# hammershock/SFM-Python

Hardware: AMD Instinct MI355X
Metric: BA iterations/sec (higher is better)
Workload: dtype f64

## Files before the change

sfm-python_amd/csrc/ba_kernels.hpp:

```cpp
#pragma once

#include <hip/hip_runtime.h>
#include <stdint.h>

#include "tr2d.hpp"

namespace sfmba {

constexpr int kCamTab = 17;
constexpr int kCamRow = 18;
#ifndef SFMBA_REC_LAYOUT
#define SFMBA_REC_LAYOUT 0
#endif
constexpr int kRecLayout = SFMBA_REC_LAYOUT;
constexpr int kRec = kRecLayout == 0 ? 6 : (kRecLayout == 1 ? 8 : 16);
constexpr int kVinvRow = kRecLayout == 0 ? 6 : (kRecLayout == 1 ? 8 : 16);
constexpr int kVinvInRec = kRecLayout == 2 ? 8 : -1;
constexpr int kRhsRec = 16;
constexpr int kSweepThreads = 1024;
constexpr int kWavesPerSweepBlock = kSweepThreads / 64;

struct KMat { double k[9]; };

constexpr int kJPlanes = 6;
// ... 68 lines not shown
        for (int q = 0; q < NQ; ++q) {
            double s = 0.0;
            for (int k = 0; k < nw; ++k) s += red[k * NQ + q];
            v[q] = s;
        }
    }
}

__device__ __forceinline__ double block_sum_all(double v, double* slots) {
    const int nw = (blockDim.x + 63) >> 6;
    v = wave_sum(v);
    if ((threadIdx.x & 63) == 0) slots[threadIdx.x >> 6] = v;
    __syncthreads();
    double s = 0.0;
    for (int k = 0; k < nw; ++k) s += slots[k];
    return s;
}

constexpr int kNQ = 9;

constexpr int kFinishCols = 10;
struct FinishJob { int row0[2], nrows[2], slot[2][kFinishCols]; };

__device__ __forceinline__ void finish_task(const double* __restrict__ part, const FinishJob& job, int y, int k,
                                            int nq, int first_sum, double* __restrict__ out) {
    const int lane = threadIdx.x & 63;
    const double* __restrict__ rows = part + (size_t)job.row0[y] * nq;
    const int nparts = job.nrows[y];
    double s = 0.0;
    if (k < first_sum) {
        for (int b = lane; b < nparts; b += 64) s = fmax(s, rows[(size_t)b * nq + k]);
        s = wave_max(s);
    } else {
        for (int b = lane; b < nparts; b += 64) s += rows[(size_t)b * nq + k];
        s = wave_sum(s);
    }
    const int dst = job.slot[y][k];
    if (lane == 0 && dst >= 0) out[dst] = s;
}

struct Piggyback {
    const double* __restrict__ part;
    double* __restrict__ out;
    FinishJob job;
    int ny, nq, first_sum;
};
__device__ __forceinline__ void finish_in_block(const Piggyback& pb) {
    const int w = threadIdx.x >> 6, nw = blockDim.x >> 6;
    for (int t = w; t < pb.ny * pb.nq; t += nw)
        finish_task(pb.part, pb.job, t / pb.nq, t % pb.nq, pb.nq, pb.first_sum, pb.out);
}

template <int NV>
__device__ __forceinline__ void seg_reduce_serial(double (&v)[NV], int key, int lane) {
    constexpr int kRowShl = 0x100;
    const int col = lane & 15, row = lane >> 4;
    const int n1 = dpp_int<kRowShl + 1>(key), n2 = dpp_int<kRowShl + 2>(key);
    const int n4 = dpp_int<kRowShl + 4>(key), n8 = dpp_int<kRowShl + 8>(key);
    const int f48 = __builtin_amdgcn_readlane(key, 48), f32 = __builtin_amdgcn_readlane(key, 32);
    const int f16 = __builtin_amdgcn_readlane(key, 16);
    const double m1 = ((col + 1 < 16) & (n1 == key)) ? 1.0 : 0.0, m2 = ((col + 2 < 16) & (n2 == key)) ? 1.0 : 0.0;
    const double m4 = ((col + 4 < 16) & (n4 == key)) ? 1.0 : 0.0, m8 = ((col + 8 < 16) & (n8 == key)) ? 1.0 : 0.0;
    const double r2 = ((row == 2) & (key == f48)) ? 1.0 : 0.0, r1 = ((row == 1) & (key == f32)) ? 1.0 : 0.0;
    const double r0 = ((row == 0) & (key == f16)) ? 1.0 : 0.0;
#pragma unroll
    for (int n = 0; n < NV; ++n) {
        double x = v[n];
        x = fma(dpp_double<kRowShl + 1>(x), m1, x);
        x = fma(dpp_double<kRowShl + 2>(x), m2, x);
        x = fma(dpp_double<kRowShl + 4>(x), m4, x);
        x = fma(dpp_double<kRowShl + 8>(x), m8, x);
        x = fma(readlane_double(x, 48), r2, x);
        x = fma(readlane_double(x, 32), r1, x);
        x = fma(readlane_double(x, 16), r0, x);
        v[n] = x;
        __builtin_amdgcn_sched_barrier(0);
    }
}

__device__ __forceinline__ int lane_below(int key, int lane) {
    int prev = dpp_int<0x111>(key);
    const int k15 = __builtin_amdgcn_readlane(key, 15), k31 = __builtin_amdgcn_readlane(key, 31);
    const int k47 = __builtin_amdgcn_readlane(key, 47);
    return lane == 16 ? k15 : (lane == 32 ? k31 : (lane == 48 ? k47 : prev));
}

__device__ __forceinline__ size_t jaddr_f32(int i, int m) {
    return ((size_t)(i >> 6) * 3 + m) * 64 + (i & 63);
}
__device__ __forceinline__ double2 load_pair(const double* __restrict__ base, int f32, int i) {
    if (f32) {
        const float2 v = reinterpret_cast<const float2*>(base)[i];
        return make_double2((double)v.x, (double)v.y);
    }
    return reinterpret_cast<const double2*>(base)[i];
}
__device__ __forceinline__ void store_pair(double* __restrict__ base, int f32, int i, double a, double b) {
    if (f32) reinterpret_cast<float2*>(base)[i] = make_float2((float)a, (float)b);
    else reinterpret_cast<double2*>(base)[i] = make_double2(a, b);
}

constexpr int kCamRT = 12, kCamWbc = 5;
__host__ __device__ constexpr size_t cam_rt_offset(int C) { return (size_t)C * kCamRow; }
__host__ __device__ constexpr size_t cam_wbc_offset(int C) { return cam_rt_offset(C) + (size_t)C * kCamRT; }
__host__ __device__ constexpr size_t cam_table_doubles(int C) { return cam_wbc_offset(C) + (size_t)C * kCamWbc; }
__device__ __forceinline__ void cam_row_values(const double* __restrict__ prm, double* __restrict__ t) {
    const double wx = prm[0], wy = prm[1], wz = prm[2];
    const double th2 = wx * wx + wy * wy + wz * wz;
    const double th = sqrt(th2);
    double a, b, cc;
    if (th < 1e-4) {
        a = 1.0 - th2 / 6.0 + th2 * th2 / 120.0;
        b = 0.5 - th2 / 24.0 + th2 * th2 / 720.0;
    } else {
        a = sin(th) / th;
        const double h = 0.5 * th;
        const double s = sin(h) / h;
        b = 0.5 * s * s;
    }
    if (th < 0.3) {
        cc = 1.0 / 6.0 - th2 / 120.0 + th2 * th2 / 5040.0 - th2 * th2 * th2 / 362880.0 +
             th2 * th2 * th2 * th2 / 39916800.0 - th2 * th2 * th2 * th2 * th2 / 6227020800.0;
    } else {
        cc = (th - sin(th)) / (th2 * th);
    }
    t[0] = 1.0 + b * (wx * wx - th2); t[1] = -a * wz + b * wx * wy;     t[2] = a * wy + b * wx * wz;
    t[3] = a * wz + b * wx * wy;      t[4] = 1.0 + b * (wy * wy - th2); t[5] = -a * wx + b * wy * wz;
    t[6] = -a * wy + b * wx * wz;     t[7] = a * wx + b * wy * wz;      t[8] = 1.0 + b * (wz * wz - th2);
    t[9] = prm[3]; t[10] = prm[4]; t[11] = prm[5];
    t[12] = wx; t[13] = wy; t[14] = wz;
    t[15] = b; t[16] = cc;
}
__device__ __forceinline__ void cam_table_row(const double* __restrict__ prm, double* __restrict__ tab, int C, int c) {
    double* __restrict__ t = tab + (size_t)c * kCamRow;
    t[kCamTab] = 0.0;
    cam_row_values(prm, t);
    double* __restrict__ rt = tab + cam_rt_offset(C) + (size_t)c * kCamRT;
#pragma unroll
    for (int k = 0; k < kCamRT; ++k) rt[k] = t[k];
    double* __restrict__ wbc = tab + cam_wbc_offset(C);
#pragma unroll
    for (int k = 0; k < kCamWbc; ++k) wbc[(size_t)k * C + c] = t[12 + k];
}

__global__ void k_cam_table(const double* __restrict__ xc, int C, double* __restrict__ tab) {
    const int c = blockIdx.x * blockDim.x + threadIdx.x;
    if (c >= C) return;
    double prm[6];
#pragma unroll
    for (int k = 0; k < 6; ++k) prm[k] = xc[6 * (size_t)c + k];
    cam_table_row(prm, tab, C, c);
}

__global__ void k_tr_step(double* __restrict__ sc, double Delta, const PcgCtrl* __restrict__ ctrl,
                          Piggyback pb) {
    if (pb.part != nullptr) {
        finish_in_block(pb);
        __syncthreads();
    }
    if (threadIdx.x != 0 || blockIdx.x != 0) return;
    if (ctrl != nullptr && ctrl->done == 0) { sc[30] = 1.0; return; }
    auto q = [&](int point_slot, int k) { return sc[point_slot] + sc[16 + k]; };
    const TrModel m = tr_build_model(sc[1], sc[2], sc[3], q(8, 1), q(4, 5), q(5, 6), q(11, 4), q(6, 7), q(7, 8));
    const TrStep st = tr_solve_step(m, Delta);
    sc[25] = st.c1; sc[26] = st.c2; sc[27] = st.predicted; sc[28] = st.step_h_norm; sc[29] = st.step_norm;
    sc[30] = 0.0; sc[31] = Delta;
}

__global__ __launch_bounds__(256) void k_step_table(const double* __restrict__ x,
                                                    const double* __restrict__ sg,
                                                    const double* __restrict__ p, double c1, double c2,
                                                    const double* __restrict__ coef,
                                                    int C, int64_t n, int bc, double* __restrict__ x_new,
                                                    double* __restrict__ tab, double* __restrict__ rec_new,
                                                    const double* __restrict__ skip) {
    if (skip != nullptr && *skip != 0.0) return;
    if (coef != nullptr) { c1 = coef[0]; c2 = coef[1]; }
    if ((int)blockIdx.x < bc) {
        const int c = blockIdx.x * blockDim.x + threadIdx.x;
        if (c >= C) return;
        double prm[6];
#pragma unroll
        for (int k = 0; k < 6; ++k) {
            const size_t e = 6 * (size_t)c + k;
            prm[k] = x[e] + c1 * sg[e] + c2 * p[e];
            x_new[e] = prm[k];
        }
        cam_table_row(prm, tab, C, c);
        return;
    }
    const int64_t n6 = 6 * (int64_t)C;
    const int nb = gridDim.x - bc;
    for (int64_t e = n6 + (blockIdx.x - bc) * (int64_t)blockDim.x + threadIdx.x; e < n; e += (int64_t)nb * blockDim.x) {
        const double v = x[e] + c1 * sg[e] + c2 * p[e];
        x_new[e] = v;
        const int q = (int)(e - n6), pt = q / 3;
        rec_new[(size_t)kRec * pt + (q - 3 * pt)] = v;
    }
}

__global__ void k_fill_rec(const double* __restrict__ pts, int P, double* __restrict__ rec) {
    const int q = blockIdx.x * blockDim.x + threadIdx.x;
    if (q >= 3 * P) return;
    const int p = q / 3;
    rec[(size_t)kRec * p + (q - 3 * p)] = pts[q];
}

template <bool JAC>
__device__ __forceinline__ void observe(const double* __restrict__ t, double X, double Y, double Z,
                                        double u, double v, const KMat& K, double& rx, double& ry,
                                        double* __restrict__ jc, double* __restrict__ jp) {
    const double vx = X - t[9], vy = Y - t[10], vz = Z - t[11];
    const double qx = t[0] * vx + t[1] * vy + t[2] * vz;
    const double qy = t[3] * vx + t[4] * vy + t[5] * vz;
    const double qz = t[6] * vx + t[7] * vy + t[8] * vz;
    const double px = K.k[0] * qx + K.k[1] * qy + K.k[2] * qz;
    const double py = K.k[3] * qx + K.k[4] * qy + K.k[5] * qz;
    const double pz = K.k[6] * qx + K.k[7] * qy + K.k[8] * qz;
    const double iz = 1.0 / pz;
    const double u0 = px * iz, u1 = py * iz;
    rx = u0 - u;
    ry = u1 - v;
    if (JAC) {
        const double wx = t[12], wy = t[13], wz = t[14], b = t[15], c = t[16];
#pragma unroll
        for (int k = 0; k < 2; ++k) {
            const double pk = k == 0 ? u0 : u1;
            const double a0 = (K.k[3 * k + 0] - pk * K.k[6]) * iz;
            const double a1 = (K.k[3 * k + 1] - pk * K.k[7]) * iz;
            const double a2 = (K.k[3 * k + 2] - pk * K.k[8]) * iz;
            const double j0 = a0 * t[0] + a1 * t[3] + a2 * t[6];
            const double j1 = a0 * t[1] + a1 * t[4] + a2 * t[7];
            const double j2 = a0 * t[2] + a1 * t[5] + a2 * t[8];
            jp[3 * k + 0] = j0; jp[3 * k + 1] = j1; jp[3 * k + 2] = j2;
            const double m0 = j1 * vz - j2 * vy, m1 = j2 * vx - j0 * vz, m2 = j0 * vy - j1 * vx;
            const double s0 = m1 * wz - m2 * wy, s1 = m2 * wx - m0 * wz, s2 = m0 * wy - m1 * wx;
            const double t0 = s1 * wz - s2 * wy, t1 = s2 * wx - s0 * wz, t2 = s0 * wy - s1 * wx;
            jc[6 * k + 0] = -(m0 - b * s0 + c * t0);
            jc[6 * k + 1] = -(m1 - b * s1 + c * t1);
            jc[6 * k + 2] = -(m2 - b * s2 + c * t2);
            jc[6 * k + 3] = -j0; jc[6 * k + 4] = -j1; jc[6 * k + 5] = -j2;
        }
    }
}

__device__ __forceinline__ void st16(double* __restrict__ p, double a, double b) {
    *reinterpret_cast<double2*>(p) = make_double2(a, b);
}

constexpr int kRowPieces = kCamRow / 2;
constexpr size_t kRowSlabDoubles = 64 * (size_t)kCamRow;
__device__ __forceinline__ void rows_request(const double* __restrict__ table, int cam, int lane, double* slab) {
#pragma unroll
    for (int k = 0; k < kRowPieces; ++k) {
        const int q = k * 64 + lane;
        const int row = q / kRowPieces, piece = q - kRowPieces * row;
        const int cr = __shfl(cam, row);
        __builtin_amdgcn_global_load_lds(table + (size_t)cr * kCamRow + 2 * piece,
                                         (__attribute__((address_space(3))) void*)(slab + 2 * 64 * k), 16, 0, 0);
        __builtin_amdgcn_sched_barrier(0);
    }
}
__device__ __forceinline__ void rows_wait() { asm volatile("s_waitcnt vmcnt(0)" ::: "memory"); }
__device__ __forceinline__ void rows_read_done() { asm volatile("s_waitcnt lgkmcnt(0)" ::: "memory"); }

constexpr int kEdgeRow = 10;
struct PointBlocksOut {
    double* __restrict__ V;
    double* __restrict__ gp;
    double* __restrict__ edge;
};

template <bool LDS_TAB, bool JAC, bool STORE_R, bool F32, bool BLOCKS = false, bool STORE_J = true>
__global__ __launch_bounds__(kSweepThreads) void k_resjac(
    const double* __restrict__ camtab, const double* __restrict__ pts, const int* __restrict__ cam_idx,
    const int* __restrict__ pt_idx, const double* __restrict__ uv, double* __restrict__ r,
    double* __restrict__ J, int N, int64_t ld, int C, KMat K,
    double* __restrict__ cost_part, const double* __restrict__ skip, PointBlocksOut pb) {
    extern __shared__ __align__(16) double smem[];
    __shared__ double red[kWavesPerSweepBlock];
    if (skip != nullptr && *skip != 0.0) return;
    const int stride = gridDim.x * blockDim.x;
    const int lane = threadIdx.x & 63;
    static_assert(JAC || !BLOCKS, "the point blocks are sums of Jacobian entries");
    constexpr bool blocks = BLOCKS;
    int i = blockIdx.x * blockDim.x + threadIdx.x;
    int c0 = 0, p0 = 0, c1 = 0, p1 = 0;
    double2 uv0 = make_double2(0.0, 0.0);
    double X0 = 0.0, Y0 = 0.0, Z0 = 0.0;
    if (i < N) { c0 = cam_idx[i]; p0 = pt_idx[i]; uv0 = load_pair(uv, F32, i); }
    if (i + stride < N) { c1 = cam_idx[i + stride]; p1 = pt_idx[i + stride]; }
    if (i < N) { const double* __restrict__ Xp = pts + 3 * (size_t)p0; X0 = Xp[0]; Y0 = Xp[1]; Z0 = Xp[2]; }
    if (LDS_TAB) {
        const int n2 = (C * kCamRow) >> 1;
        const double2* __restrict__ src = reinterpret_cast<const double2*>(camtab);
        double2* __restrict__ dst = reinterpret_cast<double2*>(smem);
        for (int k = threadIdx.x; k < n2; k += blockDim.x) dst[k] = src[k];
        __syncthreads();
    }
    double* const slab = smem + (size_t)(threadIdx.x >> 6) * kRowSlabDoubles;
    if (!LDS_TAB && i - lane < N) rows_request(camtab, c0, lane, slab);
    double acc = 0.0;
    while (i - lane < N) {
        const bool on = i < N;
        const int in = i + stride, in2 = in + stride;
        double tl[kCamRow];
        if (!LDS_TAB) rows_wait();
        {
            const double2* __restrict__ trow = reinterpret_cast<const double2*>(LDS_TAB ? smem + (size_t)c0 * kCamRow
                                                                                         : slab + (size_t)lane * kCamRow);
#pragma unroll
            for (int k = 0; k < kCamRow / 2; ++k) { const double2 q = trow[k]; tl[2 * k] = q.x; tl[2 * k + 1] = q.y; }
        }
        if (!LDS_TAB) {
            rows_read_done();
            if (in - lane < N) rows_request(camtab, c1, lane, slab);
        }
        int c2 = 0, p2 = 0;
        double2 uv1 = make_double2(0.0, 0.0);
        double X1 = 0.0, Y1 = 0.0, Z1 = 0.0;
        if (in2 < N) { c2 = cam_idx[in2]; p2 = pt_idx[in2]; }
        if (in < N) {
            uv1 = load_pair(uv, F32, in);
            const double* __restrict__ Xp = pts + 3 * (size_t)p1;
            X1 = Xp[0]; Y1 = Xp[1]; Z1 = Xp[2];
        }
        const int ib = i - lane;
        int pprev = -1, pnext = -2;
        if (blocks) {
            if (ib > 0) pprev = pt_idx[ib - 1];
            if (ib + 64 < N) pnext = pt_idx[ib + 64];
        }
        double jc[12], jp[6], rx, ry;
        observe<JAC>(tl, X0, Y0, Z0, uv0.x, uv0.y, K, rx, ry, jc, jp);
        if (on) {
            acc += rx * rx + ry * ry;
            if (STORE_R) {
                if (F32) store_pair(r, 1, i, rx, ry); else st16(r + 2 * (size_t)i, rx, ry);
            }
            if (JAC && STORE_J) {
                if (F32) {
                    float4* __restrict__ Jf = reinterpret_cast<float4*>(J);
                    Jf[jaddr_f32(i, 0)] = make_float4((float)jc[0], (float)jc[1], (float)jc[2], (float)jc[6]);
                    Jf[jaddr_f32(i, 1)] = make_float4((float)jc[7], (float)jc[8], (float)jp[0], (float)jp[1]);
                    Jf[jaddr_f32(i, 2)] = make_float4((float)jp[2], (float)jp[3], (float)jp[4], (float)jp[5]);
                } else {
                    st16(J + jaddr(ld, i, 0), jc[0], jc[1]);
                    st16(J + jaddr(ld, i, 1), jc[2], jc[6]);
                    st16(J + jaddr(ld, i, 2), jc[7], jc[8]);
#pragma unroll
                    for (int m = 0; m < 3; ++m) st16(J + jaddr(ld, i, 3 + m), jp[2 * m], jp[2 * m + 1]);
                }
            }
        }
        if (blocks) {
            double v[9];
            v[0] = jp[0] * jp[0] + jp[3] * jp[3]; v[1] = jp[0] * jp[1] + jp[3] * jp[4];
            v[2] = jp[0] * jp[2] + jp[3] * jp[5]; v[3] = jp[1] * jp[1] + jp[4] * jp[4];
// ... 377 lines not shown
                                  const double* __restrict__ uv, int f32, int N, int* __restrict__ cm_pt,
                                  double* __restrict__ cm_uv) {
    const int k = blockIdx.x * blockDim.x + threadIdx.x;
    if (k >= N) return;
    const int i = perm[k];
    cm_pt[k] = pt_idx[i];
    if (f32) reinterpret_cast<float2*>(cm_uv)[k] = reinterpret_cast<const float2*>(uv)[i];
    else reinterpret_cast<double2*>(cm_uv)[k] = reinterpret_cast<const double2*>(uv)[i];
}

__global__ __launch_bounds__(256) void k_unpack_obs(const unsigned short* __restrict__ ci16, const short2* __restrict__ uv16,
                                                    int from, int to, int f32, int* __restrict__ cam_idx, double* __restrict__ uv) {
    const int k = from + blockIdx.x * blockDim.x + threadIdx.x;
    if (k >= to) return;
    cam_idx[k] = (int)ci16[k];
    const short2 q = uv16[k];
    if (f32) reinterpret_cast<float2*>(uv)[k] = make_float2((float)q.x, (float)q.y);
    else reinterpret_cast<double2*>(uv)[k] = make_double2((double)q.x, (double)q.y);
}
__global__ __launch_bounds__(256) void k_expand_pt_idx(const int* __restrict__ pt_ptr, int P, int N, int ld, int* __restrict__ pt_idx) {
    const int p = blockIdx.x * blockDim.x + threadIdx.x;
    if (p < P) {
        const int b = pt_ptr[p], e = pt_ptr[p + 1];
        for (int k = b; k < e; ++k) pt_idx[k] = p;
    } else if (p == P) {
        for (int k = N; k < ld; ++k) pt_idx[k] = 0;
    }
}

constexpr int kSortSlices = 512;
__global__ __launch_bounds__(64) void k_cam_hist(const int* __restrict__ cam_idx, const unsigned char* __restrict__ fixed,
                                                 int N, int C, int per, int* __restrict__ hist) {
    extern __shared__ int cnt[];
    for (int c = threadIdx.x; c < C; c += 64) cnt[c] = 0;
    __syncthreads();
    const int b0 = blockIdx.x * per, b1 = min(N, b0 + per);
    for (int k0 = b0 + (int)threadIdx.x; k0 < b1; k0 += 64 * 8) {
        int c[8];
#pragma unroll
        for (int u = 0; u < 8; ++u) { const int k = k0 + 64 * u; c[u] = k < b1 ? cam_idx[k] : -1; }
#pragma unroll
        for (int u = 0; u < 8; ++u)
            if (c[u] >= 0 && (fixed == nullptr || fixed[c[u]] == 0)) atomicAdd(&cnt[c[u]], 1);
    }
    __syncthreads();
    for (int c = threadIdx.x; c < C; c += 64) hist[(size_t)blockIdx.x * C + c] = cnt[c];
}
__global__ __launch_bounds__(256) void k_cam_offsets(const int* __restrict__ hist, const int* __restrict__ cam_ptr, int B, int C,
                                                     int* __restrict__ off) {
    const int c = blockIdx.x * blockDim.x + threadIdx.x;
    if (c >= C) return;
    int run = cam_ptr[c];
    for (int b0 = 0; b0 < B; b0 += 16) {
        int n[16];
#pragma unroll
        for (int u = 0; u < 16; ++u) n[u] = b0 + u < B ? hist[(size_t)(b0 + u) * C + c] : 0;
#pragma unroll
        for (int u = 0; u < 16; ++u) {
            if (b0 + u < B) off[(size_t)(b0 + u) * C + c] = run;
            run += n[u];
        }
    }
}
__global__ __launch_bounds__(64) void k_cam_scatter(const int* __restrict__ cam_idx, const unsigned char* __restrict__ fixed,
                                                    const int* __restrict__ pt_idx, const double* __restrict__ uv, int f32,
                                                    int N, int C, int per, int key_bits, const int* __restrict__ off,
                                                    int* __restrict__ cm_pt, double* __restrict__ cm_uv) {
    extern __shared__ int cur[];
    for (int c = threadIdx.x; c < C; c += 64) cur[c] = off[(size_t)blockIdx.x * C + c];
    __syncthreads();
    const int lane = threadIdx.x;
    const unsigned long long lt = lane == 0 ? 0ull : (~0ull >> (64 - lane));
    const int b0 = blockIdx.x * per, b1 = min(N, b0 + per);
    auto fetch = [&](int k, int& c, int& p, double2& q) {
        c = -1; p = 0; q = make_double2(0.0, 0.0);
        if (k < b1) {
            c = cam_idx[k];
            p = pt_idx[k];
            if (f32) { const float2 t = reinterpret_cast<const float2*>(uv)[k]; q = make_double2((double)t.x, (double)t.y); }
            else q = reinterpret_cast<const double2*>(uv)[k];
        }
    };
    int cn, pn;
    double2 qn;
    fetch(b0 + lane, cn, pn, qn);
    for (int k0 = b0; k0 < b1; k0 += 64) {
        int c = cn;
        const int p = pn;
        const double2 q = qn;
        fetch(k0 + 64 + lane, cn, pn, qn);
        if (c >= 0 && fixed != nullptr && fixed[c] != 0) c = -1;
        const bool act = c >= 0;
        unsigned long long eq = __ballot(act);
        for (int bit = 0; bit < key_bits; ++bit) {
            const unsigned long long m = __ballot(act && ((c >> bit) & 1));
            eq &= ((c >> bit) & 1) ? m : ~m;
        }
        if (act) {
            const int dst = cur[c] + __popcll(eq & lt);
            cm_pt[dst] = p;
            if (f32) reinterpret_cast<float2*>(cm_uv)[dst] = make_float2((float)q.x, (float)q.y);
            else reinterpret_cast<double2*>(cm_uv)[dst] = q;
            if ((eq >> lane) == 1ull) cur[c] += __popcll(eq);
        }
        __builtin_amdgcn_wave_barrier();
    }
}
__global__ __launch_bounds__(256) void k_xcd_chunks(const int* __restrict__ cam_ptr, const int* __restrict__ cm_pt, int C, int P,
                                                    int4* __restrict__ chunks) {
    const int e = blockIdx.x * blockDim.x + threadIdx.x;
    const int groups = (C + 3) / 4;
    if (e >= groups * 32) return;
    const int j = e & 3, k = (e >> 2) & 7, g = e >> 5;
    const int c = 4 * g + j;
    if (c >= C) { chunks[e] = make_int4(-1, 0, 0, 8); return; }
    const int b = cam_ptr[c], en = cam_ptr[c + 1];
    auto bound = [&](int kk) {
        if (kk <= 0) return b;
        if (kk >= 8) return en;
        const int p_hi = (int)(((long long)P * kk) / 8);
        int lo = b, hi = en;
        while (lo < hi) { const int mid = (lo + hi) >> 1; if (cm_pt[mid] < p_hi) lo = mid + 1; else hi = mid; }
        return lo;
    };
    chunks[e] = make_int4(c, bound(k), bound(k + 1), 8);
}

struct StepTable {
    const int2* __restrict__ wsteps;
    const int2* __restrict__ steps;
    int n_waves;
};

__device__ __forceinline__ void write_partials(double (&q)[kNQ], double* __restrict__ part) {
    __shared__ double red[4 * kNQ];
    __shared__ double mred[4];
    const double m = wave_max(q[0]);
    q[0] = 0.0;
    if ((threadIdx.x & 63) == 0) mred[threadIdx.x >> 6] = m;
    block_sum<kNQ>(q, red);
    if (threadIdx.x == 0) {
        double mm = 0.0;
        for (int k = 0; k < (int)(blockDim.x >> 6); ++k) mm = fmax(mm, mred[k]);
        part[(size_t)blockIdx.x * kNQ + 0] = mm;
        for (int k = 1; k < kNQ; ++k) part[(size_t)blockIdx.x * kNQ + k] = q[k];
    }
}

template <int kScalePts>
__global__ __launch_bounds__(256) void k_update_scale(const double* __restrict__ Ugc,
                                                      const double* __restrict__ V,
                                                      const double* __restrict__ gp,
                                                      const double* __restrict__ x, int C, int P,
                                                      int first, int bc, double* __restrict__ si,
                                                      double* __restrict__ g, double* __restrict__ sg,
                                                      double* __restrict__ part) {
    const int n6 = 6 * C;
    double q[kNQ];
#pragma unroll
    for (int k = 0; k < kNQ; ++k) q[k] = 0.0;
    auto element = [&](double d, double ge, double s_old, double xe, double& s, double& sge) {
        s = sqrt(d);
        if (first) { if (s == 0.0) s = 1.0; } else { s = fmax(s, s_old); }
        sge = ge / (s * s);
        q[0] = fmax(q[0], fabs(ge));
        q[1] += (ge / s) * (ge / s);
        q[2] += (xe * s) * (xe * s);
        q[3] += xe * xe;
        q[4] += sge * sge;
    };
    if ((int)blockIdx.x < bc) {
        const int diagU[6] = {0, 6, 11, 15, 18, 20};
        for (int e = blockIdx.x * blockDim.x + threadIdx.x; e < n6; e += bc * blockDim.x) {
            const int c = e / 6, k = e - 6 * c;
            const double d = Ugc[(size_t)c * 27 + diagU[k]], ge = Ugc[(size_t)c * 27 + 21 + k];
            double s, sge;
            element(d, ge, first ? 0.0 : si[e], x[e], s, sge);
            si[e] = s; g[e] = ge; sg[e] = sge;
        }
    } else {
        const int nb = (int)gridDim.x - bc, b = (int)blockIdx.x - bc;
        const double* __restrict__ xp = x + n6;
        double* __restrict__ sip = si + n6;
        double* __restrict__ gpo = g + n6;
        double* __restrict__ sgp = sg + n6;
        for (int p0 = (b * kScalePts) * (int)blockDim.x + (int)threadIdx.x; p0 < P; p0 += nb * kScalePts * (int)blockDim.x) {
            double d[kScalePts][3], ge[kScalePts][3], so[kScalePts][3], xe[kScalePts][3];
#pragma unroll
            for (int u = 0; u < kScalePts; ++u) {
                const int p = p0 + u * (int)blockDim.x;
                const size_t pp = (size_t)(p < P ? p : 0);
                d[u][0] = V[pp * 6 + 0]; d[u][1] = V[pp * 6 + 3]; d[u][2] = V[pp * 6 + 5];
#pragma unroll
                for (int k = 0; k < 3; ++k) {
                    ge[u][k] = gp[pp * 3 + k];
                    xe[u][k] = xp[pp * 3 + k];
                    so[u][k] = first ? 0.0 : sip[pp * 3 + k];
                }
            }
#pragma unroll
            for (int u = 0; u < kScalePts; ++u) {
                const int p = p0 + u * (int)blockDim.x;
                if (p >= P) continue;
#pragma unroll
                for (int k = 0; k < 3; ++k) {
                    double s, sge;
                    element(d[u][k], ge[u][k], so[u][k], xe[u][k], s, sge);
                    sip[(size_t)p * 3 + k] = s; gpo[(size_t)p * 3 + k] = ge[u][k]; sgp[(size_t)p * 3 + k] = sge;
                }
            }
        }
    }
    write_partials(q, part);
}


__global__ void k_post(Mailbox mb) { post_mailbox(mb); }

__global__ void k_finish(const double* __restrict__ part, FinishJob job, int nq, int first_sum,
                         double* __restrict__ out, const double* __restrict__ skip, Mailbox mb) {
    if (skip != nullptr && *skip != 0.0) {
        if (mb.host != nullptr && blockIdx.x == 0 && threadIdx.x < 64) post_mailbox(mb);
        return;
    }
    const int k = threadIdx.x >> 6;
    if (k < nq) finish_task(part, job, (int)blockIdx.x, k, nq, first_sum, out);
    if (mb.host != nullptr) {
        __syncthreads();
        if (threadIdx.x < 64) post_mailbox(mb);
    }
}

struct Recompute {
    const double* __restrict__ camtab;
    const double* __restrict__ pts;
    KMat K;
};
__device__ __forceinline__ void stage_cam_table(const double* __restrict__ camtab, int C, double* __restrict__ smem) {
    const int n2 = (C * kCamRow) >> 1;
    const double2* __restrict__ src = reinterpret_cast<const double2*>(camtab);
    double2* __restrict__ dst = reinterpret_cast<double2*>(smem);
    for (int k = threadIdx.x; k < n2; k += blockDim.x) dst[k] = src[k];
    __syncthreads();
}
__device__ __forceinline__ void recompute_blocks(const Recompute& rc, const double* __restrict__ tab_lds, int c, int p,
                                                 double* jc, double* jp) {
    double tl[kCamRow];
    const double2* __restrict__ trow = reinterpret_cast<const double2*>(tab_lds + (size_t)c * kCamRow);
#pragma unroll
    for (int k = 0; k < kCamRow / 2; ++k) { const double2 q = trow[k]; tl[2 * k] = q.x; tl[2 * k + 1] = q.y; }
    const double* __restrict__ Xp = rc.pts + 3 * (size_t)p;
    double rx, ry;
    observe<true>(tl, Xp[0], Xp[1], Xp[2], 0.0, 0.0, rc.K, rx, ry, jc, jp);
}

template <bool LDS_VEC, bool JFREE = false>
__global__ __launch_bounds__(kSweepThreads) void k_jdot(ObsArrays o, const double* __restrict__ sgc,
                                                        const double* __restrict__ sgp, int N, int C,
                                                        double* __restrict__ t1,
                                                        double* __restrict__ part, Piggyback pb, Recompute rc) {
    static_assert(!(LDS_VEC && JFREE), "J-free: the LDS holds the camera table, the vector comes from L2");
    extern __shared__ __align__(16) double smem[];
    __shared__ double red[kWavesPerSweepBlock];
    const int nwork = pb.part != nullptr ? (int)gridDim.x - 1 : (int)gridDim.x;
    if ((int)blockIdx.x == nwork) { finish_in_block(pb); return; }
    if (LDS_VEC) {
        for (int i = threadIdx.x; i < 6 * C; i += blockDim.x) smem[i] = sgc[i];
        __syncthreads();
    }
    if (JFREE) stage_cam_table(rc.camtab, C, smem);
    const double* __restrict__ vc = LDS_VEC ? smem : sgc;
    double acc = 0.0;
    for (int i = blockIdx.x * blockDim.x + threadIdx.x; i < N; i += nwork * blockDim.x) {
        double jc[12], jp[6];
        if (JFREE) recompute_blocks(rc, smem, o.cam_idx[i], o.pt_idx[i], jc, jp);
        else load_blocks(o, i, jc, jp);
        const double2* a2 = reinterpret_cast<const double2*>(vc + 6 * o.cam_idx[i]);
        const double2 a01 = a2[0], a23 = a2[1], a45 = a2[2];
        const double a[6] = {a01.x, a01.y, a23.x, a23.y, a45.x, a45.y};
        const double* b = sgp + 3 * (size_t)o.pt_idx[i];
        double t0 = 0.0, t1v = 0.0;
#pragma unroll
        for (int k = 0; k < 6; ++k) { t0 += jc[k] * a[k]; t1v += jc[6 + k] * a[k]; }
#pragma unroll
        for (int k = 0; k < 3; ++k) { t0 += jp[k] * b[k]; t1v += jp[3 + k] * b[k]; }
        store_pair(t1, o.f32, i, t0, t1v);
        acc += t0 * t0 + t1v * t1v;
    }
    acc = wave_sum(acc);
    if ((threadIdx.x & 63) == 0) red[threadIdx.x >> 6] = acc;
    __syncthreads();
    if (threadIdx.x == 0) {
        double s = 0.0;
        for (int k = 0; k < (int)(blockDim.x >> 6); ++k) s += red[k];
        part[blockIdx.x] = s;
    }
}

__device__ __forceinline__ void chol3_inverse(const double* a , double* inv ) {
    const double l00 = sqrt(a[0]);
    const double l10 = a[1] / l00, l20 = a[2] / l00;
    const double l11 = sqrt(a[3] - l10 * l10);
    const double l21 = (a[4] - l20 * l10) / l11;
    const double l22 = sqrt(a[5] - l20 * l20 - l21 * l21);
    const double m00 = 1.0 / l00, m11 = 1.0 / l11, m22 = 1.0 / l22;
    const double m10 = -l10 * m00 * m11;
    const double m21 = -l21 * m11 * m22;
    const double m20 = -(l20 * m00 + l21 * m10) * m22;
    inv[0] = m00 * m00 + m10 * m10 + m20 * m20;
    inv[1] = m10 * m11 + m20 * m21;
    inv[2] = m20 * m22;
    inv[3] = m11 * m11 + m21 * m21;
    inv[4] = m21 * m22;
    inv[5] = m22 * m22;
}

__device__ __forceinline__ double reg_from_a11(double a11, double G11, double Delta, double reg_min) {
    const double a = 0.5 * G11, b = -a11;
    double reg = reg_min;
    if (a11 > 0.0) {
        const double to_tr = Delta / sqrt(a11);
        double best = 0.0;
        const double y_ub = to_tr * (a * to_tr + b);
        if (y_ub < best) best = y_ub;
        if (a != 0.0) {
            const double ext = -0.5 * b / a;
            if (ext > 0.0 && ext < to_tr) { const double y = ext * (a * ext + b); if (y < best) best = y; }
        }
        reg = fmax(-best / (Delta * Delta), reg_min);
    }
    return reg;
}
__device__ __forceinline__ double reg_from_scalars(const double* __restrict__ sc, double G11, double Delta,
                                                   double reg_min) {
    return reg_from_a11(sc[8] + sc[16 + 1], G11, Delta, reg_min);
}

__device__ __forceinline__ void point_prep_one(const double* __restrict__ V, const double* __restrict__ gp,
                                               const double* __restrict__ sip, const double* __restrict__ dp_extra,
                                               int p, double reg, double* __restrict__ Vinv,
                                               double* __restrict__ e, const double* __restrict__ pts = nullptr,
                                               double* __restrict__ rhsrec = nullptr) {
    double a[6], inv[6];
#pragma unroll
    for (int k = 0; k < 6; ++k) a[k] = V[(size_t)p * 6 + k];
    if (dp_extra) {
        a[0] += dp_extra[3 * (size_t)p]; a[3] += dp_extra[3 * (size_t)p + 1]; a[5] += dp_extra[3 * (size_t)p + 2];
    } else {
        const double s0 = sip[3 * (size_t)p], s1 = sip[3 * (size_t)p + 1], s2 = sip[3 * (size_t)p + 2];
        a[0] += reg * s0 * s0; a[3] += reg * s1 * s1; a[5] += reg * s2 * s2;
// ... 24 lines not shown
    float* __restrict__ rt32;
    float* __restrict__ rec32;
    double* __restrict__ rtd;
    Origin o;
};
__device__ __forceinline__ void mixed_prep_camera(const MixedPrep& mx, int C, int c) {
    const double* __restrict__ rt = mx.camtab + cam_rt_offset(C) + (size_t)kCamRT * c;
    float4* __restrict__ out = reinterpret_cast<float4*>(mx.rt32 + (size_t)kRt32 * c);
    out[0] = make_float4((float)rt[0], (float)rt[1], (float)rt[2], (float)rt[3]);
    out[1] = make_float4((float)rt[4], (float)rt[5], (float)rt[6], (float)rt[7]);
    out[2] = make_float4((float)rt[8], (float)(rt[9] - mx.o.x), (float)(rt[10] - mx.o.y), (float)(rt[11] - mx.o.z));
    double* __restrict__ d = mx.rtd + (size_t)kRt32 * c;
    const float4 a = out[0], b = out[1], e = out[2];
    d[0] = a.x; d[1] = a.y; d[2] = a.z; d[3] = a.w; d[4] = b.x; d[5] = b.y; d[6] = b.z; d[7] = b.w;
    d[8] = e.x; d[9] = e.y; d[10] = e.z; d[11] = e.w;
}
__device__ __forceinline__ void mixed_prep_point(const MixedPrep& mx, const double* __restrict__ pts, int p) {
    float4* __restrict__ out = reinterpret_cast<float4*>(mx.rec32 + (size_t)kRec32 * p);
    out[0] = make_float4((float)(pts[3 * (size_t)p] - mx.o.x), (float)(pts[3 * (size_t)p + 1] - mx.o.y),
                         (float)(pts[3 * (size_t)p + 2] - mx.o.z), 0.f);
}
__global__ void k_mixed_prep(MixedPrep mx, const double* __restrict__ pts, int C, int P, int bc) {
    if ((int)blockIdx.x < bc) {
        const int c = blockIdx.x * blockDim.x + threadIdx.x;
        if (c < C) mixed_prep_camera(mx, C, c);
        return;
    }
    const int p = (blockIdx.x - bc) * blockDim.x + threadIdx.x;
    if (p < P) mixed_prep_point(mx, pts, p);
}

__global__ void k_point_prep(const double* __restrict__ V, const double* __restrict__ gp,
                             const double* __restrict__ sip, const double* __restrict__ dp_extra,
                             int P, double reg, double* __restrict__ Vinv, double* __restrict__ e,
                             const double* __restrict__ pts, double* __restrict__ rhsrec) {
    const int p = blockIdx.x * blockDim.x + threadIdx.x;
    if (p >= P) return;
    point_prep_one(V, gp, sip, dp_extra, p, reg, Vinv, e, pts, rhsrec);
}

__device__ __forceinline__ void spd6_inverse(const double (&A)[6][6], double (&out)[21]) {
    double Lm[6][6];
#pragma unroll
    for (int j = 0; j < 6; ++j) {
        double sj = A[j][j];
#pragma unroll
        for (int k = 0; k < j; ++k) sj -= Lm[j][k] * Lm[j][k];
        const double ljj = sqrt(sj);
        Lm[j][j] = ljj;
        const double inv = 1.0 / ljj;
#pragma unroll
        for (int i = j + 1; i < 6; ++i) {
            double t = A[i][j];
#pragma unroll
            for (int k = 0; k < j; ++k) t -= Lm[i][k] * Lm[j][k];
            Lm[i][j] = t * inv;
        }
    }
    double M[6][6];
#pragma unroll
    for (int j = 0; j < 6; ++j) {
        M[j][j] = 1.0 / Lm[j][j];
#pragma unroll
        for (int i = j + 1; i < 6; ++i) {
            double t = 0.0;
#pragma unroll
            for (int k = j; k < i; ++k) t -= Lm[i][k] * M[k][j];
            M[i][j] = t / Lm[i][i];
        }
    }
    int n = 0;
#pragma unroll
    for (int a = 0; a < 6; ++a)
#pragma unroll
        for (int b = a; b < 6; ++b) {
            double t = 0.0;
#pragma unroll
            for (int k = b; k < 6; ++k) t += M[k][a] * M[k][b];
            out[n++] = t;
        }
}

__device__ __forceinline__ void cam_prep_regs(const double* __restrict__ Ugc, const double* __restrict__ sic,
                                              const double* __restrict__ dc_extra, int C, int c, double reg,
                                              double* __restrict__ Dc, double* __restrict__ Minv,
                                              const double* __restrict__ sd, double (&out)[21]) {
    double A[6][6];
    {
        int n = 0;
#pragma unroll
        for (int a = 0; a < 6; ++a)
#pragma unroll
            for (int b = a; b < 6; ++b) {
                A[a][b] = Ugc[(size_t)c * 27 + n] - (sd ? sd[(size_t)n * C + c] : 0.0);
                A[b][a] = A[a][b];
                ++n;
            }
    }
#pragma unroll
    for (int a = 0; a < 6; ++a) {
        double d;
        if (sd) d = Dc[(size_t)a * C + c];
        else {
            d = dc_extra ? dc_extra[6 * (size_t)c + a] : reg * sic[6 * (size_t)c + a] * sic[6 * (size_t)c + a];
            Dc[(size_t)a * C + c] = d;
        }
        A[a][a] += d;
    }
    spd6_inverse(A, out);
#pragma unroll
    for (int n = 0; n < 21; ++n) Minv[(size_t)n * C + c] = out[n];
}
__device__ __forceinline__ void cam_prep_one(const double* __restrict__ Ugc, const double* __restrict__ sic,
                                             const double* __restrict__ dc_extra, int C, int c, double reg,
                                             double* __restrict__ Dc, double* __restrict__ Minv,
                                             const double* __restrict__ sd = nullptr) {
    double out[21];
    cam_prep_regs(Ugc, sic, dc_extra, C, c, reg, Dc, Minv, sd, out);
}

__global__ void k_cam_prep(const double* __restrict__ Ugc, const double* __restrict__ sic,
                           const double* __restrict__ dc_extra, int C, double reg,
                           double* __restrict__ Dc, double* __restrict__ Minv) {
    const int c = blockIdx.x * blockDim.x + threadIdx.x;
    if (c >= C) return;
    cam_prep_one(Ugc, sic, dc_extra, C, c, reg, Dc, Minv);
}

__global__ __launch_bounds__(64) void k_cam_prep_schur(const double* __restrict__ Ugc, const double* __restrict__ sd, int C,
                                                       double* __restrict__ Dc, double* __restrict__ Minv) {
    const int c = blockIdx.x * blockDim.x + threadIdx.x;
    if (c >= C) return;
    cam_prep_one(Ugc, nullptr, nullptr, C, c, 0.0, Dc, Minv, sd);
}

__global__ __launch_bounds__(64) void k_prep(double* __restrict__ sc, double Delta, double reg_min,
                                             const double* __restrict__ Ugc, const double* __restrict__ V,
                                             const double* __restrict__ gp, const double* __restrict__ si,
                                             int C, int P, int bc, double* __restrict__ Dc,
                                             double* __restrict__ Minv,
                                             double* __restrict__ Vinv, double* __restrict__ e,
                                             const double* __restrict__ jd_part, int jd_n, double eta_min, double eta_max,
                                             const double* __restrict__ pts, double* __restrict__ rhsrec, MixedPrep mx) {
    double G11;
    if (jd_part != nullptr) {
        double s = 0.0;
        for (int b = threadIdx.x; b < jd_n; b += 64) s += jd_part[b];
        G11 = wave_sum(s);
        G11 = __shfl(G11, 0);
        if (blockIdx.x == 0 && threadIdx.x == 0) sc[1] = G11;
    } else {
        G11 = sc[1];
    }
    const double reg = reg_from_scalars(sc, G11, Delta, reg_min);
    if (blockIdx.x == 0 && threadIdx.x == 0) {
        sc[13] = reg;
        const double a11 = sc[8] + sc[16 + 1], prev = sc[14];
        double eta = eta_max;
        if (prev > 0.0 && a11 >= 0.0) eta = fmin(eta_max, fmax(eta_min, sqrt(a11 / prev)));
        sc[15] = eta;
        sc[14] = a11;
    }
    if ((int)blockIdx.x < bc) {
        const int c = blockIdx.x * blockDim.x + threadIdx.x;
        if (c >= C) return;
        if (mx.rt32 != nullptr) mixed_prep_camera(mx, C, c);
        if (Minv != nullptr) { cam_prep_one(Ugc, si, nullptr, C, c, reg, Dc, Minv); return; }
#pragma unroll
        for (int a = 0; a < 6; ++a) Dc[(size_t)a * C + c] = reg * si[6 * (size_t)c + a] * si[6 * (size_t)c + a];
        return;
    }
    const int p = (blockIdx.x - bc) * blockDim.x + threadIdx.x;
    if (p >= P) return;
    if (mx.rt32 != nullptr) mixed_prep_point(mx, pts, p);
    point_prep_one(V, gp, si + 6 * (size_t)C, nullptr, p, reg, Vinv, e, pts, rhsrec);
}

__device__ __forceinline__ double minv_row(const double* m, const double* r, int k) {
    double z = 0.0;
#pragma unroll
    for (int j = 0; j < 6; ++j) {
        const int a = k < j ? k : j, b = k < j ? j : k;
        z += m[a * 6 - a * (a - 1) / 2 + (b - a)] * r[j];
    }
    return z;
}

struct PcgFused {
    const double* __restrict__ Dc;
    const double* __restrict__ Minv;
    const double* __restrict__ Ugc;
    double* __restrict__ vecs;
    PcgCtrl* __restrict__ ctrl2;
    double tol;
    int max_iters;
    const double* __restrict__ tol_dev;
    double* __restrict__ part;
};
constexpr int kPcgM = kPcgUcm;

__device__ __forceinline__ double pcg_local_step(const double* __restrict__ part, int C, const PcgCtrl& ci, PcgCtrl& co) {
    __shared__ double red4[16][4];
    const int cam = threadIdx.x;
    double q4[4] = {0.0, 0.0, 0.0, 0.0};
    if (cam < C) {
#pragma unroll
        for (int k = 0; k < 4; ++k) q4[k] = part[(size_t)k * C + cam];
    }
#pragma unroll
    for (int k = 0; k < 4; ++k) q4[k] = wave_sum(q4[k]);
    if ((threadIdx.x & 63) == 0) {
#pragma unroll
        for (int k = 0; k < 4; ++k) red4[threadIdx.x >> 6][k] = q4[k];
    }
    __syncthreads();
    double tot[4] = {0.0, 0.0, 0.0, 0.0};
    for (int w = 0; w < (int)(blockDim.x >> 6); ++w) {
#pragma unroll
        for (int k = 0; k < 4; ++k) tot[k] += red4[w][k];
    }
    const double delta = tot[0], su = tot[1], sm = tot[2], gamma = tot[3];
    const double beta = ci.iters == 0 ? 0.0 : ci.rz / ci.rz_prev;
    const double den = delta - (ci.iters == 0 ? 0.0 : beta * gamma / ci.alpha_prev);
    const double alpha = gamma / den;
    co = ci;
    if (!(den > 0.0) || !isfinite(alpha)) { co.done = 3; return 0.0; }
    const double rz = gamma - 2.0 * alpha * su + alpha * alpha * sm;
    int done = 0;
    if (!(rz > ci.tol2 * ci.rz0)) done = 1;
    else if (ci.iters + 1 >= ci.max_iters) done = 2;
    co.rz_prev = gamma; co.alpha_prev = alpha; co.rz = rz; co.iters = ci.iters + 1; co.done = done;
    return alpha;
}

__device__ __forceinline__ bool pcg_fused_update(const PcgFused& pf, const double* __restrict__ acc, int C, int L,
                                                 double (&uu)[6]) {
    __shared__ double red_a[16];
    __shared__ double red_b[16];
    const int n6 = 6 * C;
    PcgCtrl* __restrict__ cout = pf.ctrl2 + ((L + 1) & 1);
    const bool writer = blockIdx.x == 0 && threadIdx.x == 0;
    const int cam = threadIdx.x;
    const bool has = cam < C;
    const int slice = (C + (int)gridDim.x - 1) / (int)gridDim.x;
    const bool own = has && cam >= (int)blockIdx.x * slice && cam < ((int)blockIdx.x + 1) * slice;
    const int set = L == 0 ? 0 : (L - 1) & 1;
    const double* __restrict__ vold = pf.vecs + (size_t)set * kPcgVecs * n6;
    double* __restrict__ vnew = pf.vecs + (size_t)(L == 0 ? 0 : set ^ 1) * kPcgVecs * n6;
#pragma unroll
    for (int k = 0; k < 6; ++k) uu[k] = 0.0;
    double m[21];
    PcgCtrl ci;
    if (L != 0) {
        ci = pf.ctrl2[L & 1];
        if (ci.done != 0) {
            if (writer) *cout = ci;
            return false;
        }
    }
    if (pf.part != nullptr && L != 0) {
        double ue[6] = {0.0, 0.0, 0.0, 0.0, 0.0, 0.0}, me[6] = {0.0, 0.0, 0.0, 0.0, 0.0, 0.0};
        if (has) {
#pragma unroll
            for (int k = 0; k < 6; ++k) {
                const size_t e = (size_t)k * C + cam;
                ue[k] = vold[kPcgU * n6 + e];
                me[k] = pf.vecs[kPcgM * n6 + e];
            }
        }
        PcgCtrl co;
        const double alpha = pcg_local_step(pf.part, C, ci, co);
        if (writer) *cout = co;
        if (co.done == 3) return false;
        const int done = co.done;
        if (has) {
#pragma unroll
            for (int k = 0; k < 6; ++k) uu[k] = ue[k] - alpha * me[k];
            if (own) {
#pragma unroll
                for (int k = 0; k < 6; ++k) {
                    const size_t e = (size_t)k * C + cam;
                    vnew[kPcgU * n6 + e] = uu[k];
                    if (done != 0) {
                        const double xk = pf.vecs[kPcgX * n6 + e] + alpha * pf.vecs[kPcgP * n6 + e];
                        pf.vecs[kPcgX * n6 + e] = xk;
                        pf.vecs[(size_t)kPcgVecs * n6 + kPcgX * n6 + e] = xk;
                    }
                }
            }
        }
        return done == 0;
    }
    if (has) {
#pragma unroll
        for (int n = 0; n < 21; ++n) m[n] = pf.Minv[(size_t)n * C + cam];
    }
    if (L == 0) {
        double rr[6];
        double t = 0.0;
        if (has) {
#pragma unroll
            for (int k = 0; k < 6; ++k) rr[k] = -pf.Ugc[(size_t)cam * 27 + 21 + k] - acc[(size_t)k * C + cam];
#pragma unroll
            for (int k = 0; k < 6; ++k) {
                uu[k] = minv_row(m, rr, k);
                t += uu[k] * rr[k];
            }
// ... 1980 lines not shown
```

sfm-python_amd/csrc/sfmba.hip:

```cpp
#include "../../include/sfmba.h"

#include <hip/hip_runtime.h>
#include <hip/hip_ext.h>
#include <rccl/rccl.h>
#include <dlfcn.h>

#include <algorithm>
#include <atomic>
#include <chrono>
#include <cmath>
#include <cstdarg>
#include <cstdio>
#include <cstdlib>
#include <cstring>
#include <condition_variable>
#include <functional>
#include <mutex>
#include <numeric>
#include <string>
#include <thread>
#include <vector>

#include "ba_kernels.hpp"
#include "tr2d.hpp"
// ... 54 lines not shown
        if (p && keep) memcpy(q, p, std::min(keep, bytes));
        if (p) (void)hipHostFree(p);
        p = q; bytes = cap;
        return hipSuccess;
    }
    template <class T> T* as() const { return static_cast<T*>(p); }
};

class HostPool {
public:
    static constexpr int kMax = 16;
    ~HostPool() {
        { std::lock_guard<std::mutex> lk(m_); stop_ = true; ++gen_; }
        cv_.notify_all();
        for (auto& t : th_) t.join();
    }
    int parts_for(int64_t n) const {
        const int hw = (int)std::thread::hardware_concurrency();
        return (int)std::max<int64_t>(1, std::min<int64_t>(std::min(kMax, hw > 0 ? hw : 1), n / 65536));
    }
    template <class Fn>
    void run(int parts, Fn fn) {
        if (parts <= 1) { fn(0); return; }
        while ((int)th_.size() < parts - 1) {
            const int id = (int)th_.size() + 1;
            th_.emplace_back([this, id] { worker(id); });
        }
        std::function<void(int)> f = fn;
        {
            std::lock_guard<std::mutex> lk(m_);
            job_ = &f; job_parts_ = parts; pending_ = parts - 1; ++gen_;
        }
        cv_.notify_all();
        fn(0);
        std::unique_lock<std::mutex> lk(m_);
        done_.wait(lk, [this] { return pending_ == 0; });
        job_ = nullptr;
    }
private:
    void worker(int id) {
        unsigned long long seen = 0;
        for (;;) {
            std::function<void(int)>* f = nullptr;
            {
                std::unique_lock<std::mutex> lk(m_);
                cv_.wait(lk, [&] { return gen_ != seen; });
                seen = gen_;
                if (stop_) return;
                if (id >= job_parts_ || job_ == nullptr) continue;
                f = job_;
            }
            (*f)(id);
            {
                std::lock_guard<std::mutex> lk(m_);
                if (--pending_ == 0) done_.notify_one();
            }
        }
    }
    std::vector<std::thread> th_;
    std::mutex m_;
    std::condition_variable cv_, done_;
    std::function<void(int)>* job_ = nullptr;
    int job_parts_ = 0, pending_ = 0;
    unsigned long long gen_ = 0;
    bool stop_ = false;
};

struct RcclApi {
    void* lib = nullptr;
    ncclResult_t (*GetUniqueId)(ncclUniqueId*) = nullptr;
    ncclResult_t (*CommInitRank)(ncclComm_t*, int, ncclUniqueId, int) = nullptr;
    ncclResult_t (*AllReduce)(const void*, void*, size_t, ncclDataType_t, ncclRedOp_t, ncclComm_t, hipStream_t) = nullptr;
    ncclResult_t (*CommDestroy)(ncclComm_t) = nullptr;
    const char* (*GetErrorString)(ncclResult_t) = nullptr;
};
RcclApi* rccl_api() {
    static RcclApi api;
    static bool tried = false;
    if (!tried) {
        tried = true;
        void* lib = dlopen("librccl.so.1", RTLD_NOW | RTLD_GLOBAL);
        if (!lib) lib = dlopen("librccl.so", RTLD_NOW | RTLD_GLOBAL);
        if (!lib) lib = dlopen("/opt/rocm/lib/librccl.so.1", RTLD_NOW | RTLD_GLOBAL);
        if (lib) {
            api.GetUniqueId = (decltype(api.GetUniqueId))dlsym(lib, "ncclGetUniqueId");
            api.CommInitRank = (decltype(api.CommInitRank))dlsym(lib, "ncclCommInitRank");
            api.AllReduce = (decltype(api.AllReduce))dlsym(lib, "ncclAllReduce");
            api.CommDestroy = (decltype(api.CommDestroy))dlsym(lib, "ncclCommDestroy");
            api.GetErrorString = (decltype(api.GetErrorString))dlsym(lib, "ncclGetErrorString");
            if (api.GetUniqueId && api.CommInitRank && api.AllReduce && api.CommDestroy && api.GetErrorString)
                api.lib = lib;
        }
    }
    return api.lib ? &api : nullptr;
}

double now_s() {
    return std::chrono::duration<double>(std::chrono::steady_clock::now().time_since_epoch()).count();
}

}

struct sfmba_handle {
    int device = 0;
    hipStream_t stream = nullptr;
    bool own_stream = false;
    std::string err;
    int n_cu = 256;

    bool have_problem = false;
    int64_t C = 0, P = 0, N = 0, ld = 0, n = 0;
    int64_t N_total = 0;
    KMat K{};
    bool permuted = false;
    std::vector<int64_t> order;
    int n_ranges = 0;
    bool f32 = false;
    bool f32_next = false;
    std::vector<int64_t> fixed_next;
    int64_t n_fixed = 0;
    bool lds_tab = true, lds_vec = true;
    bool sweep_rc = false;
    bool sweep_rc_g = false;
    DevBuf rctab;
    bool jfree = false;
    bool mixed = false;
    bool mixed_b = false;
    DevBuf rt32, rec32, rctab32, rtd;
    Origin origin{0.0, 0.0, 0.0};
    bool dense = false;
    DevView cov_ptr, cov_pt, blk_ab;
    DevBuf Sblk;
    DevBuf tables;
    int n_blk = 0;
    struct Debug {
        int pcg_fused = -1;
        int tab_lds = -1, vec_lds = -1;
        int sweep_rc = -1;
        int dense = -1;
        int precond = -1;
        int pcg_local = -1;
        int xcd_chunks = -1;
        int rhsrec = -1;
        int cost_rider = -1;
        int packed_upload = -1;
        int jfree = -1;
        int cm_device = -1;
        int pcg_inline = -1;
        int xcd_cam = -1;
        int pcg_skip_last = -1;
        int pcg_mixed_b = -1;
        int pcg_mixed = -1;
        int pcg_split = -1;
        int cam_chunk = 0;
        int pcg_guess_bias = 0;
        int trace_pcg = 0, trace_stalls = 0, trace_timing = 0;
        int wait_deadline_s = 120;
        int p2p_delay_ms = 0;
        int p2p_timeout_ms = 0;
    } dbg;

    DevBuf cam_idx, pt_idx, pt_ptr, uv;
    DevView ranges, wsteps, steps;
    int n_steps = 0;
    DevBuf cm_perm, cm_pt, cm_uv, cam_partial;
    DevBuf sort_hist, fixed_dev;
    DevView cam_ptr_dev;
    DevView cam_chunks, cam_chunk_ptr;
    int n_chunks = 0;
    DevView cam_chunks_b, cam_chunk_ptr_b;
    int n_chunks_b = 0;
    bool xcd_b = false;
    std::vector<int4> host_chunks_b;
    std::vector<int> host_chunk_ptr_b;
    bool cam_multi = false;
    DevBuf xa, xb, tabA, tabB, r, J, t1;
    DevBuf rhsrec;
    DevBuf V, Vinv, gp, e, recA, recB;
    DevBuf edge;
    DevBuf g, si, sg, p;
    DevBuf Dc, Minv, vecs, vtmp, vcm;
    DevBuf part, ctrl;
    DevBuf arena_own;
    double* arena = nullptr;
    int64_t arena_doubles = 0;
    sfmba_allreduce_fn ar_fn = nullptr;
    void* ar_ctx = nullptr;
    sfmba_print_fn print_fn = nullptr;
    void* print_ctx = nullptr;
    ncclComm_t comm = nullptr;
    int64_t n_collectives = 0, n_launches = 0;
    struct P2p {
        bool ready = false;
        int rank = 0, world = 0;
        int64_t stride = 0;
        void* own = nullptr;
        void* opened[kP2pMaxRanks] = {};
        double* data[kP2pMaxRanks] = {};
        unsigned long long* flags[kP2pMaxRanks] = {};
        double* camdata[kP2pMaxRanks] = {};
        unsigned* words = nullptr;
        int64_t calls = 0;
        bool first_in_solve = true;
        int shared_device = 1;
        bool any_multi = false;
    } p2p;
    double* h_scal = nullptr;
    struct Stage { PinnedBuf uv, ci, pi, perm, ptr, uvf, tables, ci16, uv16; } stage;
    DevBuf ci16_dev, uv16_dev;
    struct Prev { bool valid = false; bool f32 = false; bool packed = false; int64_t N = 0, P = 0; } prev;
    std::vector<int2> host_ranges, host_wsteps, host_steps;
    std::vector<int4> host_chunks;
    std::vector<int> host_chunk_ptr;
    HostPool pool;
    int64_t obs_reused = 0, obs_uploaded = 0;
    double* mbox = nullptr;
    double* mbox_dev = nullptr;
    unsigned long long mbox_seq = 0;
    Mailbox post{};
    double* h_x = nullptr;
    size_t h_x_doubles = 0;
    hipStream_t copy_stream = nullptr;
    hipEvent_t ev_written = nullptr, ev_copied[2] = {nullptr, nullptr};
    PinnedBuf mirror[2];
    unsigned long long mirror_tag[2] = {0, 0}, copy_count = 0, x_tag = 0;
    bool mirror_on = false;
    const double* skip = nullptr;
    double pcg_tol = 0.0; int pcg_cap = 0;
    bool pcg_fused = false;
    bool pcg_local = false;
    bool pcg_local2 = false;
    bool pcg_b_owed = false;
    bool pcg_a_owed = false;
    bool pcg_inline = false;
    bool pcg_split = false;
    DevBuf pcg_part;
    int pcg_hint = 0;
    std::vector<int> pcg_hist;
    int64_t hist_C = 0, hist_P = 0, hist_N = 0;
    unsigned long long hist_sig = 0;
    unsigned long long problem_gen = 0;
    bool use_rhsrec = false;
    bool solved = false;
    bool transport_dropped = false;
    std::vector<const void*> lds_ready;
    int last_pcg_iters = 0;

    double* x = nullptr;
    double* x_new = nullptr;
    double* tab = nullptr;
    double* tab_new = nullptr;
    double* rec = nullptr;
    double* rec_new = nullptr;

    double* acc() const { return arena; }
    double* sd() const { return arena + 6 * C; }
    double* Ugc() const { return arena + 27 * C; }
    double* scal() const { return arena + 54 * C; }
    int pcg_L = 0;
    int red_bc = 1, red_grid = 2;
    int scale_pts = 1;
    double* partB() const { return part.as<double>() + (size_t)kPartRows * kNQ; }
    bool pending_scale_sums = false;
};

namespace {

int fail(sfmba_handle* h, int code, const char* fmt, ...) {
    char buf[512];
    va_list ap;
    va_start(ap, fmt);
    vsnprintf(buf, sizeof buf, fmt, ap);
    va_end(ap);
    if (h) h->err = buf;
    return code;
}

#define HIPCHK(h, call)                                                                         \
    do {                                                                                        \
        hipError_t e_ = (call);                                                                 \
        if (e_ != hipSuccess)                                                                   \
            return fail(h, e_ == hipErrorOutOfMemory ? -4 : -3, "%s failed: %s (%s:%d)", #call,  \
                        hipGetErrorString(e_), __FILE__, __LINE__);                             \
    } while (0)

#define LAUNCHED(h)                            \
    do {                                       \
        ++(h)->n_launches;                     \
        HIPCHK(h, hipGetLastError());          \
    } while (0)

#define CHK(expr)                  \
    do {                           \
        int rc_ = (expr);          \
        if (rc_ != 0) return rc_;  \
    } while (0)

int enter(sfmba_handle* h) {
    if (!h) return -1;
    h->err.clear();
    HIPCHK(h, hipSetDevice(h->device));
    return 0;
}

void p2p_release(sfmba_handle* h);
void p2p_close_peers(sfmba_handle* h);
bool multi_rank(const sfmba_handle* h) { return h->p2p.ready || h->comm != nullptr || h->ar_fn != nullptr; }
const unsigned* p2p_error_word(const sfmba_handle* h) { return h->p2p.ready ? h->p2p.words + 1 : nullptr; }

constexpr long long kP2pFirstTicks = 6000000000ll, kP2pSteadyTicks = 3000000000ll;
constexpr size_t kP2pFlagBytes = sizeof(unsigned long long) * 2 * kP2pMaxRanks * kP2pFlagStride;

void p2p_fill_args(sfmba_handle* h, P2pArgs& a) {
    auto& p = h->p2p;
    for (int q = 0; q < p.world; ++q) { a.data[q] = p.data[q]; a.flags[q] = p.flags[q]; }
    a.rank = p.rank; a.world = p.world; a.stride = p.stride;
    a.seq = reinterpret_cast<unsigned long long*>(p.words + 2);
    a.ticket = p.words; a.error = p.words + 1;
    a.timeout = p.first_in_solve ? kP2pFirstTicks : kP2pSteadyTicks;
    if (h->dbg.p2p_timeout_ms > 0) a.timeout = 100000ll * h->dbg.p2p_timeout_ms;
    p.first_in_solve = false;
}

constexpr int64_t kSharedDeviceCams = 128;
bool p2p_inline_ok(const sfmba_handle* h) {
    const auto& p = h->p2p;
    return p.ready && !p.any_multi && !(p.shared_device > 1 && h->C * (p.shared_device - 1) > kSharedDeviceCams);
}
bool xcd_cam(const sfmba_handle* h) { return h->xcd_b && h->dbg.xcd_cam != 0; }
bool cam_inline(const sfmba_handle* h) { return p2p_inline_ok(h) && !h->cam_multi && !xcd_cam(h) && h->dbg.pcg_inline != 0; }

CamExchange cam_exchange(sfmba_handle* h) {
    CamExchange cx{};
    auto& p = h->p2p;
    for (int q = 0; q < p.world; ++q) cx.data[q] = p.camdata[q];
    cx.rank = p.rank; cx.world = p.world; cx.C = (int)h->C; cx.error = p.words + 1;
    cx.timeout = p.first_in_solve ? kP2pFirstTicks : kP2pSteadyTicks;
    if (h->dbg.p2p_timeout_ms > 0) cx.timeout = 100000ll * h->dbg.p2p_timeout_ms;
    p.first_in_solve = false;
    return cx;
}

int p2p_allreduce(sfmba_handle* h, double* ptr, int64_t count, int op, const int* cancel,
                  unsigned long long max_mask = 0, const Piggyback* rider = nullptr, const Mailbox* post = nullptr,
                  const double* skip = nullptr) {
    auto& p = h->p2p;
    P2pArgs a{};
    p2p_fill_args(h, a);
    a.cancel = cancel;
    a.max_mask = max_mask;
    if (rider) a.rider = *rider;
    if (post) a.post = *post;
    a.skip = skip;
    if ((rider || post) && count > 512) return fail(h, -1, "rider / post need a single-workgroup collective");
    const int grid = (int)std::min<int64_t>(kP2pMaxBlocks, std::max<int64_t>(1, (count + 511) / 512));
    hipLaunchKernelGGL(k_p2p_allreduce, dim3(grid), dim3(256), 0, h->stream, ptr, (int)count, op, a);
    LAUNCHED(h);
    ++p.calls;
    return 0;
}

int exchange(sfmba_handle* h, double* ptr, int64_t count, int op, const int* cancel = nullptr) {
    if (h->p2p.ready && count <= h->p2p.stride) {
        CHK(p2p_allreduce(h, ptr, count, op, cancel));
        ++h->n_collectives;
        return 0;
    }
    if (h->comm) {
        RcclApi* api = rccl_api();
        const ncclResult_t rc = api->AllReduce(ptr, ptr, (size_t)count, ncclDouble, op == 0 ? ncclSum : ncclMax,
                                               h->comm, h->stream);
        if (rc != ncclSuccess) return fail(h, -5, "ncclAllReduce failed: %s", api->GetErrorString(rc));
        ++h->n_collectives;
        return 0;
    }
    if (!h->ar_fn) return 0;
    if (h->ar_fn(h->ar_ctx, ptr, count, op) != 0) return fail(h, -5, "all-reduce callback failed");
    ++h->n_collectives;
    return 0;
}

template <class Kern>
int set_lds(sfmba_handle* h, Kern k, size_t bytes) {
    if (bytes <= 64 * 1024) return 0;
    const void* fn = reinterpret_cast<const void*>(k);
    if (std::find(h->lds_ready.begin(), h->lds_ready.end(), fn) != h->lds_ready.end()) return 0;
    HIPCHK(h, hipFuncSetAttribute(fn, hipFuncAttributeMaxDynamicSharedMemorySize, (int)kLdsDynMax));
    h->lds_ready.push_back(fn);
    return 0;
}

double* vinv_ptr(const sfmba_handle* h) { return kVinvInRec < 0 ? h->Vinv.as<double>() : h->rec + kVinvInRec; }

MixedPrep mixed_prep(const sfmba_handle* h, const double* tab) {
    if (!h->mixed) return MixedPrep{nullptr, nullptr, nullptr, nullptr, Origin{0.0, 0.0, 0.0}};
    return MixedPrep{tab, h->rt32.as<float>(), h->rec32.as<float>(), h->rtd.as<double>(), h->origin};
}
int launch_mixed_prep(sfmba_handle* h, const double* x, const double* tab) {
    if (!h->mixed) return 0;
    const int bc = (int)((h->C + 255) / 256), bp = (int)((h->P + 255) / 256);
    hipLaunchKernelGGL(k_mixed_prep, dim3(bc + bp), dim3(256), 0, h->stream, mixed_prep(h, tab), x + 6 * h->C, (int)h->C, (int)h->P, bc);
    LAUNCHED(h);
    return 0;
}

ObsArrays obs_arrays(const sfmba_handle* h) {
    return ObsArrays{h->cam_idx.as<int>(), h->pt_idx.as<int>(), h->pt_ptr.as<int>(),
                     h->J.as<double>(), h->ld, h->f32 ? 1 : 0};
}

StepTable step_table(const sfmba_handle* h) {
    return StepTable{h->wsteps.as<int2>(), h->steps.as<int2>(), h->n_ranges};
}

int grid_1d(int64_t n, int block, int cap) {
    int64_t g = (n + block - 1) / block;
    if (g < 1) g = 1;
    if (g > cap) g = cap;
    return (int)g;
}

void report_stall(const sfmba_handle* h, const char* where, double seconds) {
    if (h->dbg.trace_stalls && seconds > 2e-3) fprintf(stderr, "sfmba: waited %.2f ms in %s\n", 1e3 * seconds, where);
}

int wait_stream(sfmba_handle* h) {
    const double t0 = now_s();
    for (;;) {
        const hipError_t e = hipStreamQuery(h->stream);
        if (e == hipSuccess) { report_stall(h, "wait_stream", now_s() - t0); return 0; }
        if (e != hipErrorNotReady) return fail(h, -3, "hipStreamQuery failed: %s", hipGetErrorString(e));
        if (now_s() - t0 > 0.05) break;
    }
    HIPCHK(h, hipStreamSynchronize(h->stream));
    report_stall(h, "wait_stream (blocking)", now_s() - t0);
    return 0;
}

int p2p_timed_out(sfmba_handle* h, unsigned code);
int mailbox_arrived(sfmba_handle* h, const char* where, double t0) {
    report_stall(h, where, now_s() - t0);
    if (h->mbox[kMboxErr] != 0.0)
        return p2p_timed_out(h, (unsigned)h->mbox[kMboxErr]);
    return 0;
}

int p2p_timed_out(sfmba_handle* h, unsigned code) {
    if ((code & 0x80000000u) == 0u) return fail(h, -5, "a direct all-reduce timed out waiting for a peer rank");
    static const char* const kinds[8] = {"?", "?", "Schur product (pass B)", "camera blocks (K3)", "reduced right-hand side", "?", "?", "?"};
    return fail(h, -5, "a direct all-reduce timed out waiting for a peer rank: the per-camera exchange of the %s, value %u of "
                       "camera %u", kinds[(code >> 28) & 7u], (code >> 23) & 31u, code & 0x7FFFFFu);
}

int wait_mailbox(sfmba_handle* h, unsigned long long seq) {
    unsigned long long* word = reinterpret_cast<unsigned long long*>(h->mbox + kMboxSeq);
    const double t0 = now_s();
    double t_check = t0 + 5e-3;
    for (int spin = 0;; ++spin) {
        if (__atomic_load_n(word, __ATOMIC_ACQUIRE) == seq) return mailbox_arrived(h, "wait_mailbox", t0);
        __builtin_ia32_pause();
        if ((spin & 15) != 15) continue;
        const double t = now_s();
        if (t < t_check) continue;
        const hipError_t e = hipStreamQuery(h->stream);
        if (e == hipSuccess) {
            if (__atomic_load_n(word, __ATOMIC_ACQUIRE) == seq) return mailbox_arrived(h, "wait_mailbox (stream idle)", t0);
            return fail(h, -3, "hand-off mailbox was not written");
        }
        if (e != hipErrorNotReady) return fail(h, -3, "hipStreamQuery failed: %s", hipGetErrorString(e));
        if (t - t0 > h->dbg.wait_deadline_s)
            return fail(h, -3, "hand-off not posted within %d s: the device queue is stuck", h->dbg.wait_deadline_s);
        t_check = t + 1e-3;
    }
}


int launch_cam_table(sfmba_handle* h, const double* x, double* tab, double* rec) {
    hipLaunchKernelGGL(k_cam_table, dim3((h->C + 255) / 256), dim3(256), 0, h->stream, x, (int)h->C, tab);
    LAUNCHED(h);
    hipLaunchKernelGGL(k_fill_rec, dim3((unsigned)((3 * h->P + 255) / 256)), dim3(256), 0, h->stream, x + 6 * h->C, (int)h->P, rec);
    LAUNCHED(h);
    return 0;
}

PointBlocksOut point_blocks_out(sfmba_handle* h) {
    return PointBlocksOut{h->V.as<double>(), h->gp.as<double>(), h->edge.as<double>()};
}

template <bool LDS, bool JAC, bool STORE_R, bool F32, bool BLOCKS>
int launch_resjac_b(sfmba_handle* h, const double* x, const double* tab, int grid, size_t lds,
                    hipEvent_t ev0, hipEvent_t ev1) {
    const double* pts = x + 6 * h->C;
    const PointBlocksOut pb = BLOCKS ? point_blocks_out(h) : PointBlocksOut{nullptr, nullptr, nullptr};
    auto kern = k_resjac<LDS, JAC, STORE_R, F32, BLOCKS>;
    if constexpr (JAC && BLOCKS && LDS && STORE_R) {
        if (h->jfree) kern = k_resjac<LDS, JAC, STORE_R, F32, BLOCKS, false>;
    }
    CHK(set_lds(h, kern, lds));
    if (ev0) {
        hipExtLaunchKernelGGL(kern, dim3(grid), dim3(kSweepThreads), (uint32_t)lds, h->stream, ev0, ev1, 0u, tab, pts,
                              (const int*)h->cam_idx.as<int>(), (const int*)h->pt_idx.as<int>(),
                              (const double*)h->uv.as<double>(), h->r.as<double>(), h->J.as<double>(),
                              (int)h->N, h->ld, (int)h->C, h->K, h->part.as<double>(), h->skip, pb);
    } else {
        hipLaunchKernelGGL(kern, dim3(grid), dim3(kSweepThreads), lds, h->stream, tab, pts,
                           h->cam_idx.as<int>(), h->pt_idx.as<int>(), h->uv.as<double>(),
                           h->r.as<double>(), h->J.as<double>(), (int)h->N,
                           h->ld, (int)h->C, h->K, h->part.as<double>(), h->skip, pb);
    }
    LAUNCHED(h);
    return 0;
}
template <bool LDS, bool JAC, bool STORE_R, bool F32>
int launch_resjac_v(sfmba_handle* h, const double* x, const double* tab, int grid, size_t lds,
                    hipEvent_t ev0, hipEvent_t ev1, bool blocks) {
    if constexpr (JAC) {
        if (blocks) return launch_resjac_b<LDS, JAC, STORE_R, F32, true>(h, x, tab, grid, lds, ev0, ev1);
    }
    return launch_resjac_b<LDS, JAC, STORE_R, F32, false>(h, x, tab, grid, lds, ev0, ev1);
}

template <bool JAC, bool STORE_R>
int launch_resjac(sfmba_handle* h, const double* x, const double* tab, int* nparts,
                  hipEvent_t ev0 = nullptr, hipEvent_t ev1 = nullptr, bool blocks = JAC) {
    const int grid = grid_1d(h->N, kSweepThreads, h->n_cu);
    *nparts = grid;
    const size_t lds = (size_t)h->C * kCamRow * sizeof(double);
    if (h->lds_tab)
        return h->f32 ? launch_resjac_v<true, JAC, STORE_R, true>(h, x, tab, grid, lds, ev0, ev1, blocks)
                      : launch_resjac_v<true, JAC, STORE_R, false>(h, x, tab, grid, lds, ev0, ev1, blocks);
    const size_t slabs = sizeof(double) * kRowSlabDoubles * kWavesPerSweepBlock;
    return h->f32 ? launch_resjac_v<false, JAC, STORE_R, true>(h, x, tab, grid, slabs, ev0, ev1, blocks)
                  : launch_resjac_v<false, JAC, STORE_R, false>(h, x, tab, grid, slabs, ev0, ev1, blocks);
}

int launch_finish(sfmba_handle* h, const double* part, int nparts, int nq, int slot) {
    FinishJob job{};
    job.row0[0] = 0; job.nrows[0] = nparts;
    for (int k = 0; k < kFinishCols; ++k) { job.slot[0][k] = slot + k; job.slot[1][k] = -1; }
    hipLaunchKernelGGL(k_finish, dim3(1), dim3(64 * nq), 0, h->stream, part, job, nq, 0, h->scal(), h->skip,
                       h->post);
    LAUNCHED(h);
    return 0;
}

FinishJob slices_job(const sfmba_handle* h, int q_lo, int q_hi) {
    FinishJob job{};
    job.row0[0] = 0;         job.nrows[0] = h->red_bc;
    job.row0[1] = h->red_bc; job.nrows[1] = h->red_grid - h->red_bc;
    for (int k = 0; k < kFinishCols; ++k) { job.slot[0][k] = -1; job.slot[1][k] = -1; }
    for (int k = 0; k < kNQ; ++k) {
        job.slot[0][k] = kCamSlot + k;
        job.slot[1][k] = (k >= q_lo && k <= q_hi) ? kPointSlot[k] : -1;
    }
    return job;
}
Piggyback slices_rider(sfmba_handle* h, int q_lo, int q_hi) {
    return Piggyback{h->part.as<double>(), h->scal(), slices_job(h, q_lo, q_hi), 2, kNQ, 1};
}

int launch_finish_slices(sfmba_handle* h, int q_lo, int q_hi) {
    const FinishJob job = slices_job(h, q_lo, q_hi);
    hipLaunchKernelGGL(k_finish, dim3(2), dim3(64 * kNQ), 0, h->stream, h->part.as<double>(), job, kNQ, 1, h->scal(),
                       (const double*)nullptr, Mailbox{});
    LAUNCHED(h);
    return 0;
}

CamMajor cam_major(const sfmba_handle* h) {
    return CamMajor{h->cam_chunks.as<int4>(), h->cm_pt.as<int>(), h->cm_uv.as<double>()};
}

int launch_cam_combine(sfmba_handle* h, int ncols, double* out, int cs, int ks, const double* skip, const int* done,
                       bool table_b = false) {
    if (!(table_b ? h->xcd_b : h->cam_multi)) return 0;
    hipLaunchKernelGGL(k_cam_combine, dim3((int)((h->C * ncols + 255) / 256)), dim3(256), 0, h->stream,
                       (table_b ? h->cam_chunk_ptr_b : h->cam_chunk_ptr).as<int>(), h->cam_partial.as<double>(), (int)h->C, ncols,
                       out, cs, ks, skip, done);
    LAUNCHED(h);
    return 0;
}

template <bool F32>
int launch_normal_blocks_v(sfmba_handle* h, const double* x, const double* tab, const double* rec, int cost_parts,
                           const Mailbox& mb) {
    (void)x;
    const int tiles = (int)((h->N + 63) / 64);
    const int riders = (tiles + kCamThreads - 1) / kCamThreads;
    CamExchange cx{};
    if (cam_inline(h)) { cx = cam_exchange(h); ++h->p2p.calls; ++h->n_collectives; }
    Piggyback fin{};
    if (cost_parts > 0) {
        fin = Piggyback{h->part.as<double>(), h->scal(), FinishJob{}, 1, 1, 0};
        fin.job.row0[0] = 0; fin.job.nrows[0] = cost_parts;
        for (int k = 0; k < kFinishCols; ++k) { fin.job.slot[0][k] = k; fin.job.slot[1][k] = -1; }
    }
    if (xcd_cam(h)) {
        const CamMajor cmb{h->cam_chunks_b.as<int4>(), h->cm_pt.as<int>(), h->cm_uv.as<double>()};
        const int wgrid = h->n_chunks_b / kWaveChunkCams;
        hipLaunchKernelGGL((k_cam_blocks_w<F32>), dim3(wgrid + riders + (cost_parts > 0 ? 1 : 0)), dim3(kCamThreads), 0, h->stream,
                           cmb, tab, rec, h->K, h->cam_partial.as<double>(), h->skip, wgrid,
                           (const int*)h->pt_idx.as<int>(), (int)h->N, point_blocks_out(h), fin, mb);
        LAUNCHED(h);
        hipLaunchKernelGGL(k_cam_combine_w<27>, dim3((unsigned)((27 * h->C + 255) / 256)), dim3(256), 0, h->stream,
                           (const double*)h->cam_partial.as<double>(), (int)h->C, h->Ugc(), 27, 1, (const int*)nullptr,
                           (const double*)h->skip);
        LAUNCHED(h);
        return exchange(h, h->Ugc(), 27 * h->C, 0);
    }
    hipLaunchKernelGGL((k_cam_blocks<F32>), dim3(h->n_chunks + riders + (cost_parts > 0 ? 1 : 0)), dim3(kCamThreads), 0, h->stream,
                       cam_major(h), tab, rec, h->K, h->Ugc(), h->cam_partial.as<double>(), h->skip, (int)h->n_chunks,
                       (const int*)h->pt_idx.as<int>(), (int)h->N, point_blocks_out(h), fin, mb, cx);
    LAUNCHED(h);
    CHK(launch_cam_combine(h, 27, h->Ugc(), 27, 1, h->skip, nullptr));
    if (cx.world > 1 || cam_inline(h)) return 0;
    return exchange(h, h->Ugc(), 27 * h->C, 0);
}
int launch_normal_blocks(sfmba_handle* h, const double* x, const double* tab, const double* rec, int cost_parts = 0,
                         const Mailbox& mb = Mailbox{}) {
    return h->f32 ? launch_normal_blocks_v<true>(h, x, tab, rec, cost_parts, mb)
                  : launch_normal_blocks_v<false>(h, x, tab, rec, cost_parts, mb);
}

int launch_point_sweep(sfmba_handle* h, const double* vin, const PcgCtrl* ctrl2, int L) {
    const int grid = (h->n_ranges + kWavesPerSweepBlock - 1) / kWavesPerSweepBlock;
    if (h->mixed && h->sweep_rc) {
        const size_t lds = sizeof(float) * kRc32Row * (size_t)h->C;
        auto kern = h->mixed_b ? k_point_sweep_rc32<false, false, false> : k_point_sweep_rc32<false, false, true>;
        CHK(set_lds(h, kern, lds));
        hipLaunchKernelGGL(kern, dim3(grid), dim3(kSweepThreads), lds, h->stream, step_table(h), (const int*)h->cam_idx.as<int>(),
// ... 79 lines not shown
        auto kern_rc = k_point_sweep_rc<true>;
        CHK(set_lds(h, kern_rc, lds_rc));
        hipLaunchKernelGGL(kern_rc, dim3(grid), dim3(kSweepThreads), lds_rc, h->stream, step_table(h),
                           (const int*)h->cam_idx.as<int>(), (const int*)h->pt_idx.as<int>(), (const double*)h->tab,
                           (const double*)(h->x + 6 * h->C), h->K, (const double*)h->vecs.as<double>(),
                           (const double*)vinv_ptr(h), h->rec, (const double*)h->acc(), (int)h->C,
                           (const PcgCtrl*)h->ctrl.as<PcgCtrl>(), L, pf, (const double*)nullptr);
        LAUNCHED(h);
        return 0;
    }
    const size_t lds = sizeof(double) * 6 * (size_t)h->C;
    auto kern = k_point_sweep<true, true>;
    CHK(set_lds(h, kern, lds));
    hipLaunchKernelGGL(kern, dim3(grid), dim3(kSweepThreads), lds, h->stream, step_table(h), obs_arrays(h),
                       (const double*)h->vecs.as<double>(), vinv_ptr(h), h->rec,
                       (const double*)h->acc(), (int)h->C, (const PcgCtrl*)h->ctrl.as<PcgCtrl>(), L, pf);
    LAUNCHED(h);
    return 0;
}

template <int MODE>
int launch_cam_schur(sfmba_handle* h, const double* vin, const PcgCtrl* ctrl_done, int set, bool local = false,
                     bool inline_exchange = false) {
    const PcgLocal pl{h->Dc.as<double>(), h->Minv.as<double>(), h->vecs.as<double>(),
                      local ? h->pcg_part.as<double>() : (double*)nullptr};
    CamExchange cx{};
    if (MODE == 0 && inline_exchange) { cx = cam_exchange(h); ++h->p2p.calls; ++h->n_collectives; }
    const bool tb = MODE == 0 && h->xcd_b;
    const CamMajor cm = tb ? CamMajor{h->cam_chunks_b.as<int4>(), h->cm_pt.as<int>(), h->cm_uv.as<double>()} : cam_major(h);
    const int grid = tb ? h->n_chunks_b : h->n_chunks;
    const MixedB mxb{h->rtd.as<double>()};
    if (tb) {
        const bool round = h->f32 && !h->sweep_rc && !h->sweep_rc_g;
        if (round) return fail(h, -1, "XCD-aware chunks need the recomputing form of pass A");
        const int wgrid = h->n_chunks_b / kWaveChunkCams;
        if (h->mixed_b)
            hipLaunchKernelGGL((k_cam_schur_w<true>), dim3(wgrid), dim3(kCamThreads), 0, h->stream, cm, (const double*)h->tab,
                               reinterpret_cast<const double*>(h->rec32.as<float>()), h->K, vin, (int)h->C,
                               h->cam_partial.as<double>(), ctrl_done, set, mxb);
        else
            hipLaunchKernelGGL((k_cam_schur_w<false>), dim3(wgrid), dim3(kCamThreads), 0, h->stream, cm, (const double*)h->tab,
                               (const double*)h->rec, h->K, vin, (int)h->C, h->cam_partial.as<double>(), ctrl_done, set, mxb);
        LAUNCHED(h);
        hipLaunchKernelGGL(k_cam_combine_w<6>, dim3((unsigned)((6 * h->C + 255) / 256)), dim3(256), 0, h->stream,
                           (const double*)h->cam_partial.as<double>(), (int)h->C, h->acc(), 1, (int)h->C,
                           ctrl_done ? &ctrl_done->done : (const int*)nullptr, (const double*)nullptr);
        LAUNCHED(h);
        return 0;
    }
    if (h->f32 && !h->sweep_rc && !h->sweep_rc_g)
        hipLaunchKernelGGL((k_cam_schur<MODE, true>), dim3(grid), dim3(kCamThreads), 0, h->stream, cm,
                           (const double*)h->tab, (const double*)h->rec, h->K, vin, (int)h->C, h->acc(),
                           h->cam_partial.as<double>(), ctrl_done, set, pl, mxb, cx);
    else if (MODE == 0 && h->mixed_b)
        hipLaunchKernelGGL((k_cam_schur<0, false, true>), dim3(grid), dim3(kCamThreads), 0, h->stream, cm,
                           (const double*)h->tab, reinterpret_cast<const double*>(h->rec32.as<float>()), h->K, vin, (int)h->C,
                           h->acc(), h->cam_partial.as<double>(), ctrl_done, set, pl, mxb, cx);
    else
        hipLaunchKernelGGL((k_cam_schur<MODE, false>), dim3(grid), dim3(kCamThreads), 0, h->stream, cm,
                           (const double*)h->tab, (const double*)h->rec, h->K, vin, (int)h->C, h->acc(),
                           h->cam_partial.as<double>(), ctrl_done, set, pl, mxb, cx);
    LAUNCHED(h);
    return launch_cam_combine(h, 6, h->acc(), 1, (int)h->C, nullptr, ctrl_done ? &ctrl_done->done : nullptr, tb);
}

bool pcg_split_mode(const sfmba_handle* h) {
    if (h->dbg.pcg_local == 0 || h->dbg.precond == 0) return false;
    if (!(h->pcg_fused || h->sweep_rc_g)) return false;
    return (multi_rank(h) || h->cam_multi || h->xcd_b) ? h->dbg.pcg_split != 0 : h->dbg.pcg_split == 1;
}

int launch_rhs_and_preconditioner(sfmba_handle* h) {
    const int64_t C = h->C;
    if (h->dbg.precond == 0) {
        CHK(launch_cam_schur<1>(h, nullptr, nullptr, 0));
        return exchange(h, h->acc(), 6 * C, 0);
    }
    CamExchange cx{};
    if (cam_inline(h)) { cx = cam_exchange(h); ++h->p2p.calls; ++h->n_collectives; }
    if (xcd_cam(h)) {
        const CamMajor cmb{h->cam_chunks_b.as<int4>(), h->cm_pt.as<int>(), h->cm_uv.as<double>()};
        const int wgrid = h->n_chunks_b / kWaveChunkCams;
        const double* rr = h->use_rhsrec ? (const double*)h->rhsrec.as<double>() : (const double*)nullptr;
        if (h->f32 && !h->sweep_rc && !h->sweep_rc_g)
            hipLaunchKernelGGL((k_cam_rhs_diag_w<true>), dim3(wgrid), dim3(kCamThreads), 0, h->stream, cmb, (const double*)h->tab,
                               (const double*)h->rec, (const double*)vinv_ptr(h), h->K, h->cam_partial.as<double>(), rr);
        else
            hipLaunchKernelGGL((k_cam_rhs_diag_w<false>), dim3(wgrid), dim3(kCamThreads), 0, h->stream, cmb, (const double*)h->tab,
                               (const double*)h->rec, (const double*)vinv_ptr(h), h->K, h->cam_partial.as<double>(), rr);
        LAUNCHED(h);
        hipLaunchKernelGGL(k_cam_combine_w<27>, dim3((unsigned)((27 * C + 255) / 256)), dim3(256), 0, h->stream,
                           (const double*)h->cam_partial.as<double>(), (int)C, h->acc(), 1, (int)C, (const int*)nullptr,
                           (const double*)nullptr);
        LAUNCHED(h);
        CHK(exchange(h, h->acc(), 27 * C, 0));
        hipLaunchKernelGGL(k_cam_prep_schur, dim3((unsigned)((C + 63) / 64)), dim3(64), 0, h->stream, (const double*)h->Ugc(),
                           (const double*)h->sd(), (int)C, h->Dc.as<double>(), h->Minv.as<double>());
        LAUNCHED(h);
        return 0;
    }
    const bool own_inverse = !h->cam_multi && (!multi_rank(h) || cam_inline(h));
    const RhsPrecond mp = own_inverse ? RhsPrecond{h->Ugc(), h->Dc.as<double>(), h->Minv.as<double>()} : RhsPrecond{nullptr, nullptr, nullptr};
    if (h->f32 && !h->sweep_rc && !h->sweep_rc_g)
        hipLaunchKernelGGL((k_cam_rhs_diag<true>), dim3(h->n_chunks), dim3(kRhsThreads), 0, h->stream, cam_major(h),
                           (const double*)h->tab, (const double*)h->rec, (const double*)vinv_ptr(h), h->K, (int)C,
                           h->acc(), h->cam_partial.as<double>(), mp, h->use_rhsrec ? (const double*)h->rhsrec.as<double>() : (const double*)nullptr, cx);
    else
        hipLaunchKernelGGL((k_cam_rhs_diag<false>), dim3(h->n_chunks), dim3(kRhsThreads), 0, h->stream, cam_major(h),
                           (const double*)h->tab, (const double*)h->rec, (const double*)vinv_ptr(h), h->K, (int)C,
                           h->acc(), h->cam_partial.as<double>(), mp, h->use_rhsrec ? (const double*)h->rhsrec.as<double>() : (const double*)nullptr, cx);
    LAUNCHED(h);
    if (own_inverse) return 0;
    CHK(launch_cam_combine(h, 27, h->acc(), 1, (int)C, nullptr, nullptr));
    CHK(exchange(h, h->acc(), 27 * C, 0));
    hipLaunchKernelGGL(k_cam_prep_schur, dim3((unsigned)((C + 63) / 64)), dim3(64), 0, h->stream, (const double*)h->Ugc(),
                       (const double*)h->sd(), (int)C, h->Dc.as<double>(), h->Minv.as<double>());
    LAUNCHED(h);
    return 0;
}

constexpr double kDenseTolFactor = 0.1;
int launch_dense_solve(sfmba_handle* h, double tol, int max_iters, bool rhs) {
    hipLaunchKernelGGL(k_schur_blocks, dim3(h->n_blk), dim3(kCamThreads), 0, h->stream, (const int*)h->cov_ptr.as<int>(),
                       (const int*)h->cov_pt.as<int>(), (const int2*)h->blk_ab.as<int2>(), (const double*)h->tab,
                       (const double*)h->rec, (const double*)vinv_ptr(h), h->K, (int)h->C,
                       h->Sblk.as<double>(), rhs ? h->acc() : (double*)nullptr);
    LAUNCHED(h);
    const int n = 6 * (int)h->C;
    const size_t lds = sizeof(double) * ((size_t)n * (size_t)(n | 1) + 2 * kDenseMaxN + ((21 * kDenseMaxN / 6 + 1) & ~1) +
                                         4 * (kDenseThreads / 64));
    CHK(set_lds(h, k_dense_pcg, lds));
    hipLaunchKernelGGL(k_dense_pcg, dim3(1), dim3(kDenseThreads), lds, h->stream, (const double*)h->Sblk.as<double>(),
                       (const double*)h->Ugc(), (const double*)h->Dc.as<double>(),
                       (const double*)h->acc(), (int)h->C, tol, max_iters, h->vecs.as<double>(), h->ctrl.as<PcgCtrl>());
    LAUNCHED(h);
    h->pcg_L = 0;
    return 0;
}

int schur_product_standalone(sfmba_handle* h, const double* v_planes) {
    const double* va = v_planes;
    if (!h->lds_vec && !h->sweep_rc && !h->sweep_rc_g) {
        hipLaunchKernelGGL(k_transpose, dim3((unsigned)((6 * h->C + 255) / 256)), dim3(256), 0, h->stream, v_planes,
                           6, (int)h->C, h->vcm.as<double>(), (const PcgCtrl*)nullptr, 0);
        LAUNCHED(h);
        va = h->vcm.as<double>();
    }
    CHK(launch_point_sweep(h, va, nullptr, 0));
    return launch_cam_schur<0>(h, v_planes, nullptr, 0);
}

int launch_jdot(sfmba_handle* h, int* nparts) {
    const int grid = grid_1d(h->N, kSweepThreads, h->n_cu);
    const double* sgc = h->sg.as<double>();
    const double* sgp = sgc + 6 * h->C;
    Piggyback pb{};
    if (h->pending_scale_sums) pb = slices_rider(h, 0, 4);
    const int launch_grid = grid + (pb.part != nullptr ? 1 : 0);
    const Recompute rc{h->tab, h->x + 6 * h->C, h->K};
    if (h->jfree) {
        const size_t lds = sizeof(double) * kCamRow * (size_t)h->C;
        auto kern = k_jdot<false, true>;
        CHK(set_lds(h, kern, lds));
        hipLaunchKernelGGL(kern, dim3(launch_grid), dim3(kSweepThreads), lds, h->stream, obs_arrays(h), sgc, sgp,
                           (int)h->N, (int)h->C, h->t1.as<double>(), h->partB(), pb, rc);
    } else if (h->lds_vec) {
        const size_t lds = sizeof(double) * 6 * h->C;
        auto kern = k_jdot<true>;
        CHK(set_lds(h, kern, lds));
        hipLaunchKernelGGL(kern, dim3(launch_grid), dim3(kSweepThreads), lds, h->stream, obs_arrays(h), sgc, sgp,
                           (int)h->N, (int)h->C, h->t1.as<double>(), h->partB(), pb, rc);
    } else {
        hipLaunchKernelGGL(k_jdot<false>, dim3(launch_grid), dim3(kSweepThreads), 0, h->stream, obs_arrays(h),
                           sgc, sgp, (int)h->N, (int)h->C, h->t1.as<double>(), h->partB(), pb, rc);
    }
    LAUNCHED(h);
    h->pending_scale_sums = false;
    *nparts = grid;
    return 0;
}

int launch_backsub(sfmba_handle* h, int* nparts) {
    const int grid = (h->n_ranges + kWavesPerSweepBlock - 1) / kWavesPerSweepBlock;
    double* dc = h->p.as<double>();
    double* dp = dc + 6 * h->C;
    const PcgCtrl* ctrl2 = h->ctrl.as<PcgCtrl>();
    const Recompute rc{h->tab, h->x + 6 * h->C, h->K};
    if (h->jfree) {
        hipLaunchKernelGGL(k_transpose, dim3((6 * h->C + 255) / 256), dim3(256), 0, h->stream,
                           (const double*)h->vecs.as<double>(), 6, (int)h->C, dc, ctrl2, h->pcg_L);
        LAUNCHED(h);
        const size_t lds = sizeof(double) * kCamRow * (size_t)h->C;
        auto kern = k_backsub<false, true>;
        CHK(set_lds(h, kern, lds));
        hipLaunchKernelGGL(kern, dim3(grid), dim3(kSweepThreads), lds, h->stream, h->ranges.as<int2>(), h->n_ranges, obs_arrays(h),
                           h->vecs.as<double>(), dc, vinv_ptr(h), h->gp.as<double>(), h->t1.as<double>(), dp, h->partB(),
                           (int)h->C, (const PcgCtrl*)nullptr, 0, h->g.as<double>(), h->si.as<double>(), h->sg.as<double>(), rc, FinalUpdate{});
    } else if (h->lds_vec) {
        const size_t lds = sizeof(double) * 6 * h->C;
        auto kern = k_backsub<true>;
        CHK(set_lds(h, kern, lds));
        hipLaunchKernelGGL(kern, dim3(grid), dim3(kSweepThreads), lds, h->stream, h->ranges.as<int2>(),
                           h->n_ranges, obs_arrays(h), h->vecs.as<double>(), dc, vinv_ptr(h),
                           h->gp.as<double>(), h->t1.as<double>(), dp, h->partB(), (int)h->C,
                           ctrl2, h->pcg_L, h->g.as<double>(), h->si.as<double>(), h->sg.as<double>(), rc,
                           h->pcg_a_owed ? FinalUpdate{h->pcg_part.as<double>(), h->vecs.as<double>(), h->ctrl.as<PcgCtrl>(), h->pcg_L - 1}
                                         : FinalUpdate{});
    } else {
        hipLaunchKernelGGL(k_transpose, dim3((6 * h->C + 255) / 256), dim3(256), 0, h->stream,
                           (const double*)h->vecs.as<double>(), 6, (int)h->C, dc, ctrl2, h->pcg_L);
        LAUNCHED(h);
        hipLaunchKernelGGL(k_backsub<false>, dim3(grid), dim3(kSweepThreads), 0, h->stream,
                           h->ranges.as<int2>(), h->n_ranges, obs_arrays(h), h->vecs.as<double>(), dc,
                           vinv_ptr(h), h->gp.as<double>(), h->t1.as<double>(), dp,
                           h->partB(), (int)h->C, (const PcgCtrl*)nullptr, 0, h->g.as<double>(),
                           h->si.as<double>(), h->sg.as<double>(), rc, FinalUpdate{});
    }
    LAUNCHED(h);
    *nparts = grid;
    return 0;
}

int launch_update_scale(sfmba_handle* h, int first, bool defer = false) {
    if (h->scale_pts == 2)
        hipLaunchKernelGGL(k_update_scale<2>, dim3(h->red_grid), dim3(256), 0, h->stream, h->Ugc(), h->V.as<double>(),
                           h->gp.as<double>(), h->x, (int)h->C, (int)h->P, first, h->red_bc, h->si.as<double>(),
                           h->g.as<double>(), h->sg.as<double>(), h->part.as<double>());
    else
        hipLaunchKernelGGL(k_update_scale<1>, dim3(h->red_grid), dim3(256), 0, h->stream, h->Ugc(), h->V.as<double>(),
                           h->gp.as<double>(), h->x, (int)h->C, (int)h->P, first, h->red_bc, h->si.as<double>(),
                           h->g.as<double>(), h->sg.as<double>(), h->part.as<double>());
    LAUNCHED(h);
    if (defer) { h->pending_scale_sums = true; return 0; }
    return launch_finish_slices(h, 0, 4);
}

Piggyback backsub_rider(sfmba_handle* h, int nparts) {
    Piggyback pb{h->partB(), h->scal(), FinishJob{}, 1, kBacksubCols, 0};
    pb.job.row0[0] = 0; pb.job.nrows[0] = nparts;
    for (int k = 0; k < kFinishCols; ++k) { pb.job.slot[0][k] = -1; pb.job.slot[1][k] = -1; }
    for (int k = 0; k < 6; ++k) pb.job.slot[0][k] = 2 + k;
    for (int k = 0; k < 4; ++k) pb.job.slot[0][6 + k] = kCamSlot + 5 + k;
    return pb;
}
int launch_finish_backsub(sfmba_handle* h, int nparts) {
    const Piggyback pb = backsub_rider(h, nparts);
    hipLaunchKernelGGL(k_finish, dim3(1), dim3(64 * kBacksubCols), 0, h->stream, pb.part, pb.job, kBacksubCols, 0,
                       h->scal(), (const double*)nullptr, Mailbox{});
    LAUNCHED(h);
    return 0;
}

int flush_scale_sums(sfmba_handle* h) {
    if (!h->pending_scale_sums) return 0;
    h->pending_scale_sums = false;
    return launch_finish_slices(h, 0, 4);
}
int exchange_linearise(sfmba_handle* h) {
    CHK(exchange(h, h->scal() + 8, 4, 0));
    CHK(exchange(h, h->scal() + kMaxSlot, 1, 1));
    return 0;
}
int exchange_tail(sfmba_handle* h) {
    return exchange(h, h->scal() + 2, 6, 0);
}

int fetch_scalars(sfmba_handle* h) {
    const Mailbox mb{h->mbox_dev, h->scal(), nullptr, ++h->mbox_seq, p2p_error_word(h)};
    hipLaunchKernelGGL(k_post, dim3(1), dim3(64), 0, h->stream, mb);
    LAUNCHED(h);
    CHK(wait_mailbox(h, h->mbox_seq));
    memcpy(h->h_scal, h->mbox, sizeof(double) * kScalSlots);
    return 0;
}

double qsum(const sfmba_handle* h, int q) { return h->h_scal[kPointSlot[q]] + h->h_scal[kCamSlot + q]; }

int ensure_h_x(sfmba_handle* h) {
    const size_t need = (size_t)std::max<int64_t>(h->n, 2 * h->N);
    if (h->h_x && h->h_x_doubles >= need) return 0;
    if (h->h_x) { (void)hipHostFree(h->h_x); h->h_x = nullptr; h->h_x_doubles = 0; }
    HIPCHK(h, hipHostMalloc((void**)&h->h_x, sizeof(double) * need, hipHostMallocDefault));
    h->h_x_doubles = need;
    return 0;
}

template <class Fn>
void staging_copy(sfmba_handle* h, void* dst, const void* src, size_t bytes, Fn chunk_done) {
    const int parts = (int)std::min<size_t>(4, bytes >> 19);
    if (parts <= 1) { memcpy(dst, src, bytes); chunk_done(0, (size_t)0, bytes); return; }
    const size_t per = ((bytes + parts - 1) / parts + 63) & ~(size_t)63;
    std::atomic<int> done[8];
    for (auto& d : done) d.store(0, std::memory_order_relaxed);
    h->pool.run(parts, [&](int t) {
        const size_t b = std::min(bytes, (size_t)t * per), e = std::min(bytes, b + per);
        if (e > b) memcpy(static_cast<char*>(dst) + b, static_cast<const char*>(src) + b, e - b);
        if (t != 0) { done[t].store(1, std::memory_order_release); return; }
        chunk_done(0, b, e - b);
        for (int k = 1; k < parts; ++k) {
            while (done[k].load(std::memory_order_acquire) == 0) { }
            const size_t bk = std::min(bytes, (size_t)k * per), ek = std::min(bytes, bk + per);
            chunk_done(k, bk, ek - bk);
        }
    });
}
void staging_copy(sfmba_handle* h, void* dst, const void* src, size_t bytes) {
    staging_copy(h, dst, src, bytes, [](int, size_t, size_t) {});
}

int upload_x(sfmba_handle* h, const double* x_host) {
    CHK(ensure_h_x(h));
    if (h->mixed) {
        const double* pts = x_host + 6 * h->C;
        const int64_t stride = std::max<int64_t>(1, h->P / 1024);
        double sx = 0.0, sy = 0.0, sz = 0.0;
        int64_t cnt = 0;
        for (int64_t q = 0; q < h->P; q += stride, ++cnt) { sx += pts[3 * q]; sy += pts[3 * q + 1]; sz += pts[3 * q + 2]; }
        h->origin = Origin{sx / (double)cnt, sy / (double)cnt, sz / (double)cnt};
        if (!std::isfinite(h->origin.x + h->origin.y + h->origin.z)) h->origin = Origin{0.0, 0.0, 0.0};
    }
    HIPCHK(h, hipStreamSynchronize(h->stream));
    const double t0 = now_s();
    hipError_t err = hipSuccess;
    staging_copy(h, h->h_x, x_host, sizeof(double) * h->n, [&](int, size_t off, size_t bytes) {
        if (bytes == 0 || err != hipSuccess) return;
        err = hipMemcpyAsync(reinterpret_cast<char*>(h->x) + off, reinterpret_cast<const char*>(h->h_x) + off, bytes,
                             hipMemcpyHostToDevice, h->stream);
    });
    HIPCHK(h, err);
    if (h->dbg.trace_timing) fprintf(stderr, "sfmba: upload_x  staging copy + enqueue %.1f us\n", 1e6 * (now_s() - t0));
    return 0;
}

int download_residuals(sfmba_handle* h, double* r_out) {
    CHK(ensure_h_x(h));
    HIPCHK(h, hipStreamSynchronize(h->stream));
    const size_t bytes = (h->f32 ? sizeof(float) : sizeof(double)) * 2 * (size_t)h->N;
    HIPCHK(h, hipMemcpyAsync(h->h_x, h->r.p, bytes, hipMemcpyDeviceToHost, h->stream));
    CHK(wait_stream(h));
    if (!h->f32 && !h->permuted) { memcpy(r_out, h->h_x, bytes); return 0; }
    const float* sf = reinterpret_cast<const float*>(h->h_x);
    for (int64_t k = 0; k < h->N; ++k) {
        const int64_t d = h->permuted ? h->order[k] : k;
        r_out[2 * d] = h->f32 ? (double)sf[2 * k] : h->h_x[2 * k];
        r_out[2 * d + 1] = h->f32 ? (double)sf[2 * k + 1] : h->h_x[2 * k + 1];
    }
    return 0;
}

int check_ready(sfmba_handle* h, const void* x) {
    if (!h->have_problem) return fail(h, -1, "sfmba_set_problem has not been called");
    if (h->transport_dropped)
        return fail(h, -1, "sfmba_set_problem removed this handle's multi-rank transport (direct link / RCCL communicator / "
                           "callback): set it up again for the new problem, or call sfmba_set_exchange(h, NULL, 0, NULL, NULL, 0) "
                           "to solve the shard on its own");
    if (!x) return fail(h, -1, "x is NULL");
    return 0;
}

int pcg_max_iters(const sfmba_handle* h, const sfmba_options& opt) {
    return opt.pcg_max_iter > 0 ? opt.pcg_max_iter : (int)std::max<int64_t>(20, 2 * 6 * h->C);
}

int pcg_start(sfmba_handle* h, const sfmba_options& opt) {
    h->pcg_L = 0;
    h->pcg_b_owed = false;
    h->pcg_a_owed = false;
    h->pcg_inline = p2p_inline_ok(h) && !h->cam_multi && !h->xcd_b && h->dbg.pcg_inline != 0 && h->dbg.pcg_local != 0 &&
                    h->dbg.precond != 0 && h->dbg.pcg_split != 1 && (h->pcg_fused || h->sweep_rc_g);
    h->pcg_split = !h->pcg_inline && pcg_split_mode(h);
    const bool own_cameras = (!multi_rank(h) && !h->cam_multi && !h->xcd_b) || h->pcg_split || h->pcg_inline;
    h->pcg_local = h->pcg_fused && h->dbg.pcg_local != 0 && own_cameras;
    h->pcg_local2 = !h->pcg_fused && h->sweep_rc_g && h->dbg.pcg_local != 0 && own_cameras;
    if (h->pcg_fused) {
        h->pcg_tol = opt.pcg_tol;
        h->pcg_cap = pcg_max_iters(h, opt);
        return 0;
    }
    if (h->pcg_local2)
        hipLaunchKernelGGL(k_pcg_init_local, dim3((unsigned)((h->C + 63) / 64)), dim3(64), 0, h->stream, (const double*)h->Ugc(),
                           (const double*)h->acc(), (const double*)h->Minv.as<double>(), (int)h->C, h->vecs.as<double>(),
                           (const double*)(h->scal() + kEtaSlot), pcg_max_iters(h, opt), h->ctrl.as<PcgCtrl>());
    else
        hipLaunchKernelGGL(k_pcg_init, dim3(1), dim3(1024), 0, h->stream, h->Ugc(), (const double*)h->acc(),
                           h->Minv.as<double>(), (int)h->C, h->vecs.as<double>(), (const double*)(h->scal() + kEtaSlot),
                           pcg_max_iters(h, opt), h->ctrl.as<PcgCtrl>());
    LAUNCHED(h);
    return 0;
}

int launch_reduce_and_tail(sfmba_handle* h, const PcgCtrl* cd, int set) {
    const int C = (int)h->C;
    const PcgLocal pl{h->Dc.as<double>(), h->Minv.as<double>(), h->vecs.as<double>(), h->pcg_part.as<double>()};
    const int grid = std::max((C + kP2pPcgThreads - 1) / kP2pPcgThreads, std::min(kP2pMaxBlocks, (C + 63) / 64));
    if (h->p2p.ready && 6 * h->C <= h->p2p.stride && grid <= kP2pMaxBlocks) {
        P2pArgs a{};
        p2p_fill_args(h, a);
        hipLaunchKernelGGL(k_p2p_pcg, dim3(grid), dim3(kP2pPcgThreads), 0, h->stream, h->acc(), (const double*)h->vecs.as<double>(),
                           C, cd, set, pl, a);
        LAUNCHED(h);
        ++h->p2p.calls;
        ++h->n_collectives;
        return 0;
    }
    CHK(exchange(h, h->acc(), 6 * h->C, 0, &cd->done));
    hipLaunchKernelGGL(k_pcg_tail, dim3((unsigned)((C + 63) / 64)), dim3(64), 0, h->stream, (const double*)h->acc(),
                       (const double*)h->vecs.as<double>(), C, cd, set, pl);
    LAUNCHED(h);
    return 0;
}

int pcg_pass_b(sfmba_handle* h, int L) {
    const PcgCtrl* cd = h->ctrl.as<PcgCtrl>() + ((L + 1) & 1);
    CHK(launch_cam_schur<0>(h, h->vecs.as<double>(), cd, L & 1, h->pcg_local && !h->pcg_split, h->pcg_inline));
    if (h->pcg_split) CHK(launch_reduce_and_tail(h, cd, L & 1));
    else if (!h->pcg_inline) CHK(exchange(h, h->acc(), 6 * h->C, 0, &cd->done));
    return 0;
}

int pcg_enqueue(sfmba_handle* h, int count, bool speculative = false) {
    PcgCtrl* ctrl2 = h->ctrl.as<PcgCtrl>();
    if (h->pcg_a_owed) {
        h->pcg_a_owed = false;
        h->pcg_b_owed = true;
        CHK(launch_pcg_fused(h, h->pcg_L - 1));
    }
    if (h->pcg_b_owed) {
        h->pcg_b_owed = false;
        CHK(pcg_pass_b(h, h->pcg_L - 1));
    }
    for (int k = 0; k < count; ++k) {
        const int L = h->pcg_L;
        if (h->pcg_fused) {
            const bool last = speculative && k == count - 1 && (!multi_rank(h) || h->pcg_inline) && h->dbg.pcg_skip_last != 0;
            if (last && L > 0 && h->pcg_local && h->lds_vec && !h->jfree && h->dbg.pcg_skip_last != 2) {
                h->pcg_L = L + 1;
                h->pcg_a_owed = true;
                break;
            }
            CHK(launch_pcg_fused(h, L));
            h->pcg_L = L + 1;
            if (last) { h->pcg_b_owed = true; break; }
            CHK(pcg_pass_b(h, L));
            continue;
        }
        const PcgCtrl* cd = ctrl2 + (L & 1);
        CHK(launch_point_sweep(h, h->vecs.as<double>(), ctrl2, L));
        CHK(launch_cam_schur<0>(h, h->vecs.as<double>(), cd, -1, h->pcg_local2 && !h->pcg_split, h->pcg_inline));
        if (h->pcg_local2 && h->pcg_split) CHK(launch_reduce_and_tail(h, cd, -1));
        if (h->pcg_local2) {
            hipLaunchKernelGGL(k_pcg_update_local, dim3((unsigned)((h->C + 1023) / 1024)), dim3(1024), 0, h->stream,
                               h->vecs.as<double>(), (const double*)h->pcg_part.as<double>(), ctrl2, L, (int)h->C);
            LAUNCHED(h);
            h->pcg_L = L + 1;
            continue;
        }
        CHK(exchange(h, h->acc(), 6 * h->C, 0, &cd->done));
        hipLaunchKernelGGL(k_pcg_update, dim3(kPcgUpdateBlocks), dim3(1024), 0, h->stream, (const double*)h->acc(),
                           h->Dc.as<double>(), h->Minv.as<double>(), (int)h->C, h->vecs.as<double>(), ctrl2, L);
        LAUNCHED(h);
        h->pcg_L = L + 1;
    }
    return 0;
}

int pcg_read(sfmba_handle* h, PcgCtrl* hc) {
    static_assert(sizeof(PcgCtrl) <= 24 * sizeof(double), "PcgCtrl fits the pinned tail");
    HIPCHK(h, hipMemcpyAsync(h->h_scal + 40, h->ctrl.as<PcgCtrl>() + (h->pcg_L & 1), sizeof *hc,
                             hipMemcpyDeviceToHost, h->stream));
    CHK(wait_stream(h));
    memcpy(hc, h->h_scal + 40, sizeof *hc);
    return 0;
}

int pcg_finish_polling(sfmba_handle* h, const sfmba_options& opt, PcgCtrl* hc) {
    const int every = std::max(1, opt.pcg_check_every);
    const int cap = pcg_max_iters(h, opt) + every + 1;
    int launched = 0;
    for (;;) {
        CHK(pcg_enqueue(h, every));
        launched += every;
        CHK(pcg_read(h, hc));
        if (hc->done != 0 || launched > cap) return 0;
    }
}

void append_center(std::string& line, const char* s) {
    const int w = 15, len = (int)strlen(s);
    const int left = (w - len) / 2 > 0 ? (w - len) / 2 : 0;
    const int right = w - len - left > 0 ? w - len - left : 0;
    line.append((size_t)left, ' ').append(s).append((size_t)right, ' ');
}
void emit_line(sfmba_handle* h, const std::string& line) {
    if (h->print_fn) { h->print_fn(h->print_ctx, line.c_str()); return; }
    fputs(line.c_str(), stdout);
    fputc('\n', stdout);
    fflush(stdout);
}

void print_header(sfmba_handle* h) {
    const char* cols[6] = {"Iteration", "Total nfev", "Cost", "Cost reduction", "Step norm", "Optimality"};
    std::string line;
    for (auto c : cols) append_center(line, c);
    emit_line(h, line);
}
void print_iter(sfmba_handle* h, int64_t it, int64_t nfev, double cost, bool have, double red, double step, double opt) {
    char b[64];
    std::string line;
    snprintf(b, sizeof b, "%lld", (long long)it); append_center(line, b);
    snprintf(b, sizeof b, "%lld", (long long)nfev); append_center(line, b);
    snprintf(b, sizeof b, "%.4e", cost); append_center(line, b);
    if (have) { snprintf(b, sizeof b, "%.2e", red); append_center(line, b); snprintf(b, sizeof b, "%.2e", step); append_center(line, b); }
    else { append_center(line, ""); append_center(line, ""); }
    snprintf(b, sizeof b, "%.2e", opt); append_center(line, b);
    emit_line(h, line);
}

}


extern "C" {

void sfmba_default_options(sfmba_options* o) {
    if (!o) return;
    memset(o, 0, sizeof *o);
    o->ftol = 1e-8; o->xtol = 1e-8; o->gtol = 1e-8;
    o->max_nfev = 0; o->verbose = 0; o->max_iter = 0;
    o->pcg_tol = 1e-2; o->pcg_max_iter = 0; o->pcg_check_every = 2;
    o->reg_min = 1e-6; o->profile = 0; o->reserved = 0; o->pcg_tol_max = 0.1;
}

int sfmba_create(sfmba_handle** out, int device_id) {
    if (!out) return -1;
    *out = nullptr;
    int ndev = 0;
    hipError_t e = hipGetDeviceCount(&ndev);
    if (e != hipSuccess || ndev <= 0) return -3;
    if (device_id < 0 || device_id >= ndev) return -1;
    auto* h = new sfmba_handle();
    h->device = device_id;
    if (hipSetDevice(device_id) != hipSuccess) { delete h; return -3; }
    hipDeviceProp_t prop;
    if (hipGetDeviceProperties(&prop, device_id) == hipSuccess) h->n_cu = prop.multiProcessorCount;
    if (hipStreamCreateWithFlags(&h->stream, hipStreamNonBlocking) != hipSuccess) { delete h; return -3; }
    h->own_stream = true;
    if (hipHostMalloc((void**)&h->h_scal, sizeof(double) * 64, hipHostMallocDefault) != hipSuccess ||
        hipHostMalloc((void**)&h->mbox, sizeof(double) * 64, hipHostMallocCoherent | hipHostMallocMapped) != hipSuccess ||
        hipHostGetDevicePointer((void**)&h->mbox_dev, h->mbox, 0) != hipSuccess) {
        (void)hipStreamDestroy(h->stream); delete h; return -4;
    }
    memset(h->mbox, 0, sizeof(double) * 64);
    {
        int prio_low = 0, prio_high = 0;
        if (hipDeviceGetStreamPriorityRange(&prio_low, &prio_high) != hipSuccess) prio_low = 0;
        if (hipStreamCreateWithPriority(&h->copy_stream, hipStreamNonBlocking, prio_low) != hipSuccess) h->copy_stream = nullptr;
    }
    if (h->copy_stream &&
        (hipEventCreateWithFlags(&h->ev_written, hipEventDisableTiming) != hipSuccess ||
         hipEventCreateWithFlags(&h->ev_copied[0], hipEventDisableTiming) != hipSuccess ||
         hipEventCreateWithFlags(&h->ev_copied[1], hipEventDisableTiming) != hipSuccess)) {
        (void)hipStreamDestroy(h->copy_stream);
        h->copy_stream = nullptr;
    }
    *out = h;
    return 0;
}

void sfmba_destroy(sfmba_handle* h) {
    if (!h) return;
    (void)hipSetDevice(h->device);
    if (h->stream) (void)hipStreamSynchronize(h->stream);
    if (h->comm) { if (RcclApi* api = rccl_api()) (void)api->CommDestroy(h->comm); h->comm = nullptr; }
    p2p_release(h);
    if (h->copy_stream) { (void)hipStreamSynchronize(h->copy_stream); (void)hipStreamDestroy(h->copy_stream); }
    if (h->ev_written) (void)hipEventDestroy(h->ev_written);
    for (auto& ev : h->ev_copied) if (ev) (void)hipEventDestroy(ev);
    if (h->own_stream && h->stream) (void)hipStreamDestroy(h->stream);
    if (h->h_scal) (void)hipHostFree(h->h_scal);
    if (h->mbox) (void)hipHostFree(h->mbox);
    if (h->h_x) (void)hipHostFree(h->h_x);
    delete h;
}

const char* sfmba_last_error(const sfmba_handle* h) { return h ? h->err.c_str() : "null handle"; }

int sfmba_set_stream(sfmba_handle* h, void* hip_stream) {
    CHK(enter(h));
    if (h->stream) HIPCHK(h, hipStreamSynchronize(h->stream));
    if (h->own_stream && h->stream) (void)hipStreamDestroy(h->stream);
    h->stream = static_cast<hipStream_t>(hip_stream);
    h->own_stream = false;
    return 0;
}

int sfmba_set_print(sfmba_handle* h, sfmba_print_fn fn, void* ctx) {
    CHK(enter(h));
    h->print_fn = fn;
    h->print_ctx = ctx;
    return 0;
}

int sfmba_debug_option(sfmba_handle* h, const char* name, int64_t value) {
    CHK(enter(h));
    if (!name) return fail(h, -1, "option name is NULL");
    const std::string n(name);
    const int v = (int)value;
    if (n == "pcg_fused") h->dbg.pcg_fused = v;
    else if (n == "sweep_rc") h->dbg.sweep_rc = v;
    else if (n == "dense") h->dbg.dense = v;
    else if (n == "precond") h->dbg.precond = v;
    else if (n == "pcg_local") h->dbg.pcg_local = v;
    else if (n == "pcg_split") h->dbg.pcg_split = v;
    else if (n == "pcg_mixed") h->dbg.pcg_mixed = v;
    else if (n == "pcg_inline") h->dbg.pcg_inline = v;
    else if (n == "pcg_skip_last") h->dbg.pcg_skip_last = v;
    else if (n == "xcd_cam") h->dbg.xcd_cam = v;
    else if (n == "cm_device") h->dbg.cm_device = v;
    else if (n == "jfree") h->dbg.jfree = v;
    else if (n == "packed_upload") h->dbg.packed_upload = v;
    else if (n == "pcg_mixed_b") h->dbg.pcg_mixed_b = v;
    else if (n == "cost_rider") h->dbg.cost_rider = v;
    else if (n == "rhsrec") h->dbg.rhsrec = v;
    else if (n == "xcd_chunks") h->dbg.xcd_chunks = v;
    else if (n == "tab_lds") h->dbg.tab_lds = v;
    else if (n == "vec_lds") h->dbg.vec_lds = v;
    else if (n == "cam_chunk") h->dbg.cam_chunk = v;
    else if (n == "pcg_guess_bias") h->dbg.pcg_guess_bias = v;
    else if (n == "trace_pcg") h->dbg.trace_pcg = v;
    else if (n == "trace_stalls") h->dbg.trace_stalls = v;
    else if (n == "trace_timing") h->dbg.trace_timing = v;
    else if (n == "wait_deadline_s") h->dbg.wait_deadline_s = v;
    else if (n == "p2p_delay_ms") h->dbg.p2p_delay_ms = v;
    else if (n == "p2p_timeout_ms") h->dbg.p2p_timeout_ms = v;
    else return fail(h, -1, "unknown debug option '%s'", name);
    return 0;
}

int sfmba_set_precision(sfmba_handle* h, int32_t storage_bits) {
    CHK(enter(h));
    if (storage_bits != 64 && storage_bits != 32) return fail(h, -1, "storage_bits must be 64 or 32");
    h->f32_next = storage_bits == 32;
    return 0;
}

int sfmba_set_fixed_cameras(sfmba_handle* h, const int64_t* camera_indices, int64_t n_fixed) {
    CHK(enter(h));
    if (n_fixed < 0 || (n_fixed > 0 && !camera_indices)) return fail(h, -1, "bad fixed-camera list");
    h->fixed_next.assign(camera_indices, camera_indices + n_fixed);
    return 0;
}

int64_t sfmba_exchange_doubles(int64_t n_cameras) { return 54 * n_cameras + kScalSlots; }

int sfmba_set_exchange(sfmba_handle* h, void* arena, int64_t arena_doubles, sfmba_allreduce_fn fn,
                       void* ctx, int64_t n_obs_total) {
    CHK(enter(h));
    if (!h->have_problem) return fail(h, -1, "call sfmba_set_problem before sfmba_set_exchange");
    h->transport_dropped = false;
    if (!fn) {
        h->ar_fn = nullptr; h->ar_ctx = nullptr;
        h->arena = h->arena_own.as<double>();
        h->N_total = h->N;
        return 0;
    }
    if (!arena || arena_doubles < sfmba_exchange_doubles(h->C))
        return fail(h, -1, "exchange arena too small: need %lld doubles", (long long)sfmba_exchange_doubles(h->C));
    if (n_obs_total < h->N) return fail(h, -1, "n_obs_total is smaller than the local shard");
    h->arena = static_cast<double*>(arena);
    h->arena_doubles = arena_doubles;
    h->ar_fn = fn; h->ar_ctx = ctx;
    h->N_total = n_obs_total;
    return 0;
}

int sfmba_comm_get_unique_id(void* id128_out) {
    RcclApi* api = rccl_api();
    if (!api || !id128_out) return -5;
    ncclUniqueId id;
    if (api->GetUniqueId(&id) != ncclSuccess) return -5;
    static_assert(sizeof(ncclUniqueId) == 128, "ncclUniqueId is 128 bytes");
    memcpy(id128_out, &id, sizeof id);
    return 0;
}

int sfmba_comm_init(sfmba_handle* h, const void* id128, int32_t rank, int32_t world, int64_t n_obs_total) {
    CHK(enter(h));
    if (!h->have_problem) return fail(h, -1, "call sfmba_set_problem before sfmba_comm_init");
    if (!id128 || world < 1 || rank < 0 || rank >= world) return fail(h, -1, "bad communicator arguments");
    if (n_obs_total < h->N) return fail(h, -1, "n_obs_total is smaller than the local shard");
    RcclApi* api = rccl_api();
    if (!api) return fail(h, -5, "librccl.so.1 could not be loaded: %s", dlerror());
    if (h->comm) { (void)api->CommDestroy(h->comm); h->comm = nullptr; }
    ncclUniqueId id;
    memcpy(&id, id128, sizeof id);
    const ncclResult_t rc = api->CommInitRank(&h->comm, world, id, rank);
    if (rc != ncclSuccess) { h->comm = nullptr; return fail(h, -5, "ncclCommInitRank failed: %s", api->GetErrorString(rc)); }
    h->ar_fn = nullptr; h->ar_ctx = nullptr;
    h->arena = h->arena_own.as<double>();
    h->N_total = n_obs_total;
    h->transport_dropped = false;
    return 0;
}

int sfmba_comm_destroy(sfmba_handle* h) {
    CHK(enter(h));
    h->transport_dropped = false;
    if (h->comm) {
        if (h->stream) HIPCHK(h, hipStreamSynchronize(h->stream));
        if (RcclApi* api = rccl_api()) (void)api->CommDestroy(h->comm);
        h->comm = nullptr;
    }
    h->N_total = h->N;
    return 0;
}

namespace {
void p2p_close_peers(sfmba_handle* h) {
    auto& p = h->p2p;
    if (h->stream) (void)hipStreamSynchronize(h->stream);
    for (int q = 0; q < kP2pMaxRanks; ++q) {
        if (p.opened[q]) (void)hipIpcCloseMemHandle(p.opened[q]);
        p.opened[q] = nullptr; p.data[q] = nullptr; p.flags[q] = nullptr; p.camdata[q] = nullptr;
    }
    p.ready = false;
}
void p2p_release(sfmba_handle* h) {
    auto& p = h->p2p;
    p2p_close_peers(h);
    if (p.own) (void)hipFree(p.own);
    if (p.words) (void)hipFree(p.words);
    p.own = nullptr; p.words = nullptr; p.ready = false; p.world = 0; p.stride = 0;
    p.shared_device = 1; p.any_multi = false;
}
}

int sfmba_p2p_export(sfmba_handle* h, int32_t world, void* handle64_out) {
    CHK(enter(h));
    if (!h->have_problem) return fail(h, -1, "call sfmba_set_problem before sfmba_p2p_export");
    if (!handle64_out || world < 1 || world > kP2pMaxRanks) return fail(h, -1, "bad arguments (1 <= world <= %d)", kP2pMaxRanks);
    p2p_release(h);
    auto& p = h->p2p;
    p.world = world;
    p.stride = (27 * h->C + 15) / 16 * 16;
    const size_t bytes = kP2pFlagBytes + sizeof(double) * 2 * (size_t)world * (size_t)p.stride +
                         sizeof(double) * cam_slots_total(world, (int)h->C);
    if (hipExtMallocWithFlags(&p.own, bytes, hipDeviceMallocUncached) != hipSuccess) {
        p.own = nullptr; (void)hipGetLastError();
        return fail(h, -5, "hipExtMallocWithFlags(uncached, %zu bytes) failed", bytes);
    }
    HIPCHK(h, hipMalloc((void**)&p.words, 4 * sizeof(unsigned)));
    HIPCHK(h, hipMemset(p.own, 0, bytes));
    {
        const size_t cam_off = kP2pFlagBytes + sizeof(double) * 2 * (size_t)world * (size_t)p.stride;
        HIPCHK(h, hipMemsetD32((hipDeviceptr_t)(static_cast<char*>(p.own) + cam_off), (int)0xFFF8A5A5u, (bytes - cam_off) / 4));
    }
    HIPCHK(h, hipMemset(p.words, 0, 4 * sizeof(unsigned)));
    HIPCHK(h, hipDeviceSynchronize());
    hipIpcMemHandle_t mh;
    if (hipIpcGetMemHandle(&mh, p.own) != hipSuccess) {
        (void)hipGetLastError(); p2p_release(h);
        return fail(h, -5, "hipIpcGetMemHandle failed");
    }
    static_assert(sizeof mh == 64, "hipIpcMemHandle_t is 64 bytes");
    memcpy(handle64_out, &mh, sizeof mh);
    return 0;
}

int sfmba_p2p_attach(sfmba_handle* h, const void* handles, int32_t rank, int32_t world) {
    CHK(enter(h));
    auto& p = h->p2p;
    if (!p.own || world != p.world) return fail(h, -1, "sfmba_p2p_export(world) must precede sfmba_p2p_attach");
    if (!handles || rank < 0 || rank >= world) return fail(h, -1, "bad arguments");
    p.rank = rank;
    for (int q = 0; q < world; ++q) {
// ... 323 lines not shown
        if (h->dbg.cam_chunk > 0) chunk_len = h->dbg.cam_chunk;
        h->cam_multi = false;
        for (int64_t c = 0; c < C; ++c) {
            chunk_ptr[c] = (int)chunks.size();
            const int b = cam_ptr[c], e = cam_ptr[c + 1];
            const int nch = std::max<int>(1, (int)((e - b + chunk_len - 1) / chunk_len));
            if (nch > 1) h->cam_multi = true;
            for (int j = 0; j < nch; ++j)
                chunks.push_back(make_int4((int)c, (int)std::min<int64_t>(e, b + j * chunk_len),
                                           (int)std::min<int64_t>(e, b + (j + 1) * chunk_len), nch));
        }
        chunk_ptr[C] = (int)chunks.size();
        h->n_chunks = (int)chunks.size();
        std::vector<int4>& chunks_b = h->host_chunks_b;
        std::vector<int>& chunk_ptr_b = h->host_chunk_ptr_b;
        chunks_b.clear();
        chunk_ptr_b.clear();
        h->xcd_b = h->dbg.xcd_chunks == 1 || (h->dbg.xcd_chunks != 0 && P >= 250000);
        if (h->xcd_b) {
            constexpr int kX = kWaveChunkRanges, kG = kWaveChunkCams;
            static_assert(kX == 8, "one range per XCD");
            const int64_t groups = (C + kG - 1) / kG;
            chunks_b.assign((size_t)(groups * kX * kG), make_int4(-1, 0, 0, kX));
            for (int64_t c = 0; c < C && !cm_device; ++c) {
                const int b = cam_ptr[c], e = cam_ptr[c + 1];
                int prev = b;
                for (int k = 0; k < kX; ++k) {
                    int bound = e;
                    if (k + 1 < kX) {
                        const int64_t p_hi = P * (int64_t)(k + 1) / kX;
                        int lo = prev, hi = e;
                        while (lo < hi) { const int mid = (lo + hi) >> 1; if (pi[perm[mid]] < p_hi) lo = mid + 1; else hi = mid; }
                        bound = lo;
                    }
                    chunks_b[(size_t)(((c / kG) * kX + k) * kG + c % kG)] = make_int4((int)c, prev, bound, kX);
                    prev = bound;
                }
            }
        }
        h->n_chunks_b = (int)chunks_b.size();
    }
    h->dense = 6 * C <= kDenseMaxN && h->dbg.dense != 0;
    std::vector<int> cov_ptr, cov_pt;
    std::vector<int2> blk_ab;
    if (h->dense) {
        const int nblk = (int)(C * (C + 1) / 2);
        cov_ptr.assign((size_t)nblk + 1, 0);
        const int pp = P >= 32768 ? 4 : 1;
        std::vector<int> cnt((size_t)pp * (size_t)nblk, 0);
        const int64_t pper = (P + pp - 1) / pp;
        auto each_pair = [&](int t, auto&& visit) {
            const int64_t p0 = std::min<int64_t>(P, t * pper), p1 = std::min<int64_t>(P, p0 + pper);
            for (int64_t p = p0; p < p1; ++p)
                for (int i = ptr[p]; i < ptr[p + 1]; ++i)
                    for (int j = i; j < ptr[p + 1]; ++j) {
                        const int a = std::min(ci[i], ci[j]), b = std::max(ci[i], ci[j]);
                        if (fixed[(size_t)a] || fixed[(size_t)b]) continue;
                        visit((int)p, dense_block_index(a, b, (int)C), i == j, a == b);
                    }
        };
        h->pool.run(pp, [&](int t) {
            int* ct = cnt.data() + (size_t)t * (size_t)nblk;
            each_pair(t, [&](int, int blk, bool self, bool same_cam) { ct[blk] += (self || !same_cam) ? 1 : 2; });
        });
        int64_t total = 0;
        for (int blk = 0; blk < nblk; ++blk) {
            cov_ptr[(size_t)blk] = (int)std::min<int64_t>(total, INT32_MAX);
            for (int t = 0; t < pp; ++t) { int& v = cnt[(size_t)t * (size_t)nblk + blk]; const int n_e = v; v = (int)std::min<int64_t>(total, INT32_MAX); total += n_e; }
        }
        cov_ptr[(size_t)nblk] = (int)std::min<int64_t>(total, INT32_MAX);
        if (total > ((int64_t)1 << 26)) h->dense = false;
        else {
            cov_pt.resize((size_t)std::max<int64_t>(1, total));
            h->pool.run(pp, [&](int t) {
                int* fill = cnt.data() + (size_t)t * (size_t)nblk;
                each_pair(t, [&](int p, int blk, bool self, bool same_cam) {
                    int& f = fill[blk];
                    cov_pt[(size_t)f++] = self ? ~p : p;
                    if (!self && same_cam) cov_pt[(size_t)f++] = p;
                });
            });
            blk_ab.resize((size_t)nblk);
            for (int a = 0; a < (int)C; ++a)
                for (int b = a; b < (int)C; ++b) blk_ab[(size_t)dense_block_index(a, b, (int)C)] = make_int2(a, b);
            h->n_blk = nblk;
        }
    }
    tp2 = now_s();
    h->lds_tab = (size_t)C * kCamRow * sizeof(double) <= kLdsDynMax;
    h->lds_vec = (size_t)C * 6 * sizeof(double) <= kLdsDynMax;
    if (h->dbg.tab_lds == 0) h->lds_tab = false;
    if (h->dbg.vec_lds == 0) h->lds_vec = false;
    h->sweep_rc = C <= kRcMaxCams && (size_t)C * kRcRow * sizeof(double) <= kLdsDynMax && h->dbg.sweep_rc != 0 &&
                  h->dbg.sweep_rc != 2;
    h->sweep_rc_g = !h->sweep_rc && h->dbg.sweep_rc != 0;
    h->pcg_fused = (h->lds_vec || h->sweep_rc) && C <= kSweepThreads;
    if (h->dbg.pcg_fused == 0) h->pcg_fused = false;
    h->mixed = (h->sweep_rc || h->sweep_rc_g) && (h->dbg.pcg_mixed == 1 || (h->dbg.pcg_mixed != 0 && f32));
    h->mixed_b = h->mixed && h->dbg.pcg_mixed_b != 0;
    h->jfree = h->dbg.jfree == 1 && h->lds_tab;

    const size_t esz = f32 ? sizeof(float) : sizeof(double);
    const size_t keep = (size_t)fdiff;
    HIPCHK(h, h->cam_idx.ensure_keep(sizeof(int) * ldz, sizeof(int) * keep));
    HIPCHK(h, h->pt_idx.ensure_keep(sizeof(int) * ldz, sizeof(int) * keep));
    HIPCHK(h, h->uv.ensure_keep(esz * 2 * ldz, esz * 2 * keep));
    const int64_t p_keep = keep == 0 ? 0 : std::min<int64_t>(std::min<int64_t>(prev.P, P), (int64_t)pi[fdiff - 1] + 1);
    HIPCHK(h, h->pt_ptr.ensure_keep(sizeof(int) * ((size_t)P + 1), sizeof(int) * (size_t)p_keep));
    struct Piece { const void* src; size_t bytes; DevView* view; size_t off; };
    Piece pieces[11] = {
        {cam_ptr.data(), sizeof(int) * cam_ptr.size(), &h->cam_ptr_dev, 0},
        {ranges.data(), sizeof(int2) * ranges.size(), &h->ranges, 0}, {wsteps.data(), sizeof(int2) * wsteps.size(), &h->wsteps, 0},
        {steps.data(), sizeof(int2) * steps.size(), &h->steps, 0}, {chunks.data(), sizeof(int4) * chunks.size(), &h->cam_chunks, 0},
        {chunk_ptr.data(), sizeof(int) * chunk_ptr.size(), &h->cam_chunk_ptr, 0},
        {cov_ptr.data(), h->dense ? sizeof(int) * cov_ptr.size() : 0, &h->cov_ptr, 0},
        {cov_pt.data(), h->dense ? sizeof(int) * cov_pt.size() : 0, &h->cov_pt, 0},
        {blk_ab.data(), h->dense ? sizeof(int2) * blk_ab.size() : 0, &h->blk_ab, 0},
        {h->host_chunks_b.data(), sizeof(int4) * h->host_chunks_b.size(), &h->cam_chunks_b, 0},
        {h->host_chunk_ptr_b.data(), sizeof(int) * h->host_chunk_ptr_b.size(), &h->cam_chunk_ptr_b, 0}};
    size_t tables_bytes = 0;
    for (auto& pc : pieces) { pc.off = tables_bytes; tables_bytes += (pc.bytes + 255) / 256 * 256; }
    HIPCHK(h, h->tables.ensure(tables_bytes + 256));
    HIPCHK(h, sg.tables.ensure(tables_bytes + 256, 0));
    for (auto& pc : pieces) {
        if (pc.bytes) memcpy(sg.tables.as<char>() + pc.off, pc.src, pc.bytes);
        pc.view->p = h->tables.as<char>() + pc.off;
    }
    HIPCHK(h, h->xa.ensure(sizeof(double) * h->n));
    HIPCHK(h, h->xb.ensure(sizeof(double) * h->n));
    HIPCHK(h, h->tabA.ensure(sizeof(double) * cam_table_doubles((int)C)));
    HIPCHK(h, h->tabB.ensure(sizeof(double) * cam_table_doubles((int)C)));
    HIPCHK(h, h->r.ensure(esz * 2 * ldz));
    HIPCHK(h, h->J.ensure(esz * 12 * ldz));
    HIPCHK(h, h->cm_perm.ensure(sizeof(int) * ldz));
    HIPCHK(h, h->cm_pt.ensure(sizeof(int) * ldz));
    HIPCHK(h, h->cm_uv.ensure(esz * 2 * ldz));
    HIPCHK(h, h->cam_partial.ensure(sizeof(double) * std::max<size_t>(27 * chunks.size(), 27 * h->host_chunks_b.size())));
    HIPCHK(h, h->recA.ensure(sizeof(double) * kRec * P));
    HIPCHK(h, h->recB.ensure(sizeof(double) * kRec * P));
    h->use_rhsrec = h->dbg.rhsrec == 1 || (h->dbg.rhsrec != 0 && P >= 250000);
    if (h->use_rhsrec) HIPCHK(h, h->rhsrec.ensure(sizeof(double) * kRhsRec * P));
    if (h->dense) {
        HIPCHK(h, h->Sblk.ensure(sizeof(double) * 36 * blk_ab.size()));
    }
    HIPCHK(h, h->t1.ensure(esz * 2 * ldz));
    HIPCHK(h, h->V.ensure(sizeof(double) * 6 * P));
    HIPCHK(h, h->Vinv.ensure(sizeof(double) * (kVinvInRec < 0 ? kVinvRow * P : 8)));
    HIPCHK(h, h->gp.ensure(sizeof(double) * 3 * P + 16));
    HIPCHK(h, h->edge.ensure(sizeof(double) * 2 * kEdgeRow * (size_t)((N + 63) / 64)));
    HIPCHK(h, h->e.ensure(sizeof(double) * 3 * P));
    HIPCHK(h, h->g.ensure(sizeof(double) * h->n));
    HIPCHK(h, h->si.ensure(sizeof(double) * h->n));
    HIPCHK(h, h->sg.ensure(sizeof(double) * h->n));
    HIPCHK(h, h->p.ensure(sizeof(double) * h->n + 16));
    HIPCHK(h, h->Dc.ensure(sizeof(double) * 6 * C));
    HIPCHK(h, h->Minv.ensure(sizeof(double) * 21 * C));
    HIPCHK(h, h->vecs.ensure(sizeof(double) * 2 * kPcgVecs * 6 * C));
    HIPCHK(h, h->vtmp.ensure(sizeof(double) * 6 * C));
    HIPCHK(h, h->vcm.ensure(sizeof(double) * 6 * C));
    if (h->sweep_rc_g) HIPCHK(h, h->rctab.ensure(sizeof(double) * kRcRow * (size_t)C));
    if (h->mixed) {
        HIPCHK(h, h->rt32.ensure(sizeof(float) * kRt32 * (size_t)C));
        HIPCHK(h, h->rtd.ensure(sizeof(double) * kRt32 * (size_t)C));
        HIPCHK(h, h->rec32.ensure(sizeof(float) * kRec32 * (size_t)P));
        if (h->sweep_rc_g) HIPCHK(h, h->rctab32.ensure(sizeof(float) * kRc32Row * (size_t)C));
    }
    h->scale_pts = P >= 65536 ? 2 : 1;
    h->red_bc = grid_1d(6 * C, 256, 32);
    h->red_grid = h->red_bc + grid_1d(P, 256 * h->scale_pts, 992);
    HIPCHK(h, h->part.ensure(sizeof(double) * (size_t)(2 * kPartRows * kNQ)));
    HIPCHK(h, h->ctrl.ensure(2 * sizeof(PcgCtrl)));
    HIPCHK(h, h->pcg_part.ensure(sizeof(double) * 4 * C));
    HIPCHK(h, h->arena_own.ensure(sizeof(double) * (size_t)sfmba_exchange_doubles(C)));
    h->arena = h->arena_own.as<double>();
    h->ar_fn = nullptr; h->ar_ctx = nullptr;
    h->x = h->xa.as<double>(); h->x_new = h->xb.as<double>();
    h->tab = h->tabA.as<double>(); h->tab_new = h->tabB.as<double>();
    h->rec = h->recA.as<double>(); h->rec_new = h->recB.as<double>();

    auto up = [&](void* dst, const void* src, size_t elem, size_t from, size_t to) -> hipError_t {
        if (to <= from) return hipSuccess;
        return hipMemcpyAsync(static_cast<char*>(dst) + elem * from, static_cast<const char*>(src) + elem * from,
                              elem * (to - from), hipMemcpyHostToDevice, h->stream);
    };
    if (packed) {
        HIPCHK(h, h->ci16_dev.ensure(sizeof(unsigned short) * ldz));
        HIPCHK(h, h->uv16_dev.ensure(sizeof(short) * 2 * ldz));
        HIPCHK(h, up(h->ci16_dev.p, ci16, sizeof(unsigned short), keep, ldz));
        HIPCHK(h, up(h->uv16_dev.p, uv16, 2 * sizeof(short), keep, ldz));
    } else {
        HIPCHK(h, up(h->cam_idx.p, ci, sizeof(int), keep, ldz));
        HIPCHK(h, up(h->pt_idx.p, pi, sizeof(int), keep, ldz));
        HIPCHK(h, up(h->uv.p, f32 ? (const void*)uvf : (const void*)uvs, 2 * esz, keep, ldz));
    }
    HIPCHK(h, up(h->pt_ptr.p, ptr, sizeof(int), (size_t)p_keep, (size_t)P + 1));
    if (packed) {
        if (keep < ldz) {
            hipLaunchKernelGGL(k_unpack_obs, dim3((unsigned)((ldz - keep + 255) / 256)), dim3(256), 0, h->stream,
                               (const unsigned short*)h->ci16_dev.as<unsigned short>(), (const short2*)h->uv16_dev.as<short2>(),
                               (int)keep, (int)ldz, f32 ? 1 : 0, h->cam_idx.as<int>(), h->uv.as<double>());
            LAUNCHED(h);
            hipLaunchKernelGGL(k_expand_pt_idx, dim3((unsigned)((P + 1 + 255) / 256)), dim3(256), 0, h->stream,
                               (const int*)h->pt_ptr.as<int>(), (int)P, (int)N, (int)ld, h->pt_idx.as<int>());
            LAUNCHED(h);
        }
    }
    h->obs_reused = fdiff;
    h->obs_uploaded = ld - fdiff;
    if (!(fdiff == N && n_cmp == N && prev.N == N && prev.P == P && h->C == C)) ++h->problem_gen;
    HIPCHK(h, hipMemcpyAsync(h->tables.p, sg.tables.p, tables_bytes, hipMemcpyHostToDevice, h->stream));
    {
        ZeroJob z{};
        auto put = [&](int k, void* ptr_, size_t bytes) { z.p[k] = ptr_; z.n16[k] = (int64_t)(bytes / 16); };
        put(0, h->arena, sizeof(double) * (size_t)sfmba_exchange_doubles(C));
        put(1, h->V.p, sizeof(double) * 6 * P);
        put(2, h->gp.p, (sizeof(double) * 3 * P + 15) / 16 * 16);
        put(3, h->p.p, (sizeof(double) * h->n + 15) / 16 * 16);
        put(4, h->r.p, esz * 2 * ldz);
        put(5, h->recA.p, sizeof(double) * kRec * P);
        put(6, h->recB.p, sizeof(double) * kRec * P);
        int64_t most = 0;
        for (int k = 0; k < 7; ++k) most = std::max(most, z.n16[k]);
        hipLaunchKernelGGL(k_zero_many, dim3((unsigned)grid_1d(most, 256 * 4, 2048), 7), dim3(256), 0, h->stream, z);
        LAUNCHED(h);
    }
    if (cm_device) {
        const int B = (int)std::min<int64_t>(kSortSlices, (N + 63) / 64);
        const int per_slice = (int)(((N + B - 1) / B + 63) / 64 * 64);
        int key_bits = 0;
        while (((int64_t)1 << key_bits) < C) ++key_bits;
        HIPCHK(h, h->sort_hist.ensure(sizeof(int) * 2 * (size_t)B * (size_t)C));
        int* sort_off = h->sort_hist.as<int>() + (size_t)B * (size_t)C;
        const unsigned char* fixed_dev = nullptr;
        if (h->n_fixed > 0) {
            HIPCHK(h, h->fixed_dev.ensure((size_t)C));
            HIPCHK(h, hipMemcpyAsync(h->fixed_dev.p, fixed.data(), (size_t)C, hipMemcpyHostToDevice, h->stream));
            fixed_dev = h->fixed_dev.as<unsigned char>();
        }
        const size_t lds = sizeof(int) * (size_t)C;
        CHK(set_lds(h, k_cam_hist, lds));
        CHK(set_lds(h, k_cam_scatter, lds));
        hipLaunchKernelGGL(k_cam_hist, dim3(B), dim3(64), lds, h->stream, (const int*)h->cam_idx.as<int>(), fixed_dev, (int)N, (int)C,
                           per_slice, h->sort_hist.as<int>());
        LAUNCHED(h);
        hipLaunchKernelGGL(k_cam_offsets, dim3((unsigned)((C + 255) / 256)), dim3(256), 0, h->stream, (const int*)h->sort_hist.as<int>(),
                           (const int*)h->cam_ptr_dev.as<int>(), B, (int)C, sort_off);
        LAUNCHED(h);
        hipLaunchKernelGGL(k_cam_scatter, dim3(B), dim3(64), lds, h->stream, (const int*)h->cam_idx.as<int>(), fixed_dev,
                           (const int*)h->pt_idx.as<int>(), (const double*)h->uv.as<double>(), f32 ? 1 : 0, (int)N, (int)C, per_slice,
                           key_bits, (const int*)sort_off, h->cm_pt.as<int>(), h->cm_uv.as<double>());
        LAUNCHED(h);
        if (h->xcd_b) {
            hipLaunchKernelGGL(k_xcd_chunks, dim3((unsigned)((h->n_chunks_b + 255) / 256)), dim3(256), 0, h->stream,
                               (const int*)h->cam_ptr_dev.as<int>(), (const int*)h->cm_pt.as<int>(), (int)C, (int)P,
                               h->cam_chunks_b.as<int4>());
            LAUNCHED(h);
        }
    } else {
        HIPCHK(h, hipMemcpyAsync(h->cm_perm.p, perm, sizeof(int) * ldz, hipMemcpyHostToDevice, h->stream));
        hipLaunchKernelGGL(k_build_cam_major, dim3((unsigned)((N + 255) / 256)), dim3(256), 0, h->stream, h->cm_perm.as<int>(),
                           h->pt_idx.as<int>(), h->uv.as<double>(), f32 ? 1 : 0, (int)N, h->cm_pt.as<int>(),
                           h->cm_uv.as<double>());
        LAUNCHED(h);
    }
    tp3 = now_s();
    HIPCHK(h, hipStreamSynchronize(h->stream));
    if (timing)
        fprintf(stderr, "sfmba: set_problem  structure = run offsets + camera-major permutation %.2f ms, wave ranges %.2f ms, step table %.2f ms, "
                        "chunks + pair lists %.2f ms\n", 1e3 * (ts1 - tp1), 1e3 * (ts2 - ts1), 1e3 * (ts3 - ts2), 1e3 * (tp2 - ts3));
    if (timing)
        fprintf(stderr, "sfmba: set_problem  convert+compare %.2f ms  structure %.2f ms  allocate+enqueue %.2f ms  upload wait %.2f ms"
                        "  (%lld of %lld observations re-used)\n",
                1e3 * (tp1 - tp0), 1e3 * (tp2 - tp1), 1e3 * (tp3 - tp2), 1e3 * (now_s() - tp3), (long long)fdiff, (long long)N);
    if (sorted) { prev.valid = true; prev.f32 = f32; prev.N = N; prev.P = P; }
    prev.packed = sorted && packed;
    h->have_problem = true;
    return 0;
}

int sfmba_residuals(sfmba_handle* h, const double* x, double* r_out) {
    CHK(enter(h));
    CHK(check_ready(h, x));
    if (!r_out) return fail(h, -1, "r_out is NULL");
    CHK(upload_x(h, x));
    CHK(launch_cam_table(h, h->x, h->tab, h->rec));
    int np = 0;
    CHK((launch_resjac<false, true>(h, h->x, h->tab, &np)));
    return download_residuals(h, r_out);
}

int sfmba_residual_jacobian(sfmba_handle* h, const double* x, double* r_out, double* Jc_out, double* Jp_out) {
    CHK(enter(h));
    CHK(check_ready(h, x));
    if (!r_out || !Jc_out || !Jp_out) return fail(h, -1, "NULL output");
    CHK(upload_x(h, x));
    CHK(launch_cam_table(h, h->x, h->tab, h->rec));
    int np = 0;
    CHK((launch_resjac<true, true>(h, h->x, h->tab, &np, nullptr, nullptr, false)));
    DevBuf jc_rm, jp_rm;
    HIPCHK(h, jc_rm.ensure(sizeof(double) * 12 * h->N));
    HIPCHK(h, jp_rm.ensure(sizeof(double) * 6 * h->N));
    hipLaunchKernelGGL(k_unpack_jac, dim3((h->N + 255) / 256), dim3(256), 0, h->stream, h->J.as<double>(),
                       (int)h->N, h->ld, h->f32 ? 1 : 0, jc_rm.as<double>(), jp_rm.as<double>());
    LAUNCHED(h);
    std::vector<double> tc(12 * h->N), tp(6 * h->N);
    CHK(download_residuals(h, r_out));
    HIPCHK(h, hipMemcpyAsync(tc.data(), jc_rm.p, sizeof(double) * 12 * h->N, hipMemcpyDeviceToHost, h->stream));
    HIPCHK(h, hipMemcpyAsync(tp.data(), jp_rm.p, sizeof(double) * 6 * h->N, hipMemcpyDeviceToHost, h->stream));
    HIPCHK(h, hipStreamSynchronize(h->stream));
    for (int64_t k = 0; k < h->N; ++k) {
        const int64_t d = h->permuted ? h->order[k] : k;
        memcpy(Jc_out + 12 * d, tc.data() + 12 * k, sizeof(double) * 12);
        memcpy(Jp_out + 6 * d, tp.data() + 6 * k, sizeof(double) * 6);
    }
    return 0;
}

int sfmba_normal_blocks(sfmba_handle* h, const double* x, double* U, double* V, double* gc, double* gp) {
    CHK(enter(h));
    CHK(check_ready(h, x));
    CHK(upload_x(h, x));
    CHK(launch_cam_table(h, h->x, h->tab, h->rec));
    int np = 0;
    CHK((launch_resjac<true, true>(h, h->x, h->tab, &np)));
    CHK(launch_normal_blocks(h, h->x, h->tab, h->rec));
    std::vector<double> ugc(27 * h->C);
    HIPCHK(h, hipMemcpyAsync(ugc.data(), h->Ugc(), sizeof(double) * 27 * h->C, hipMemcpyDeviceToHost, h->stream));
    if (V) HIPCHK(h, hipMemcpyAsync(V, h->V.p, sizeof(double) * 6 * h->P, hipMemcpyDeviceToHost, h->stream));
    if (gp) HIPCHK(h, hipMemcpyAsync(gp, h->gp.p, sizeof(double) * 3 * h->P, hipMemcpyDeviceToHost, h->stream));
    HIPCHK(h, hipStreamSynchronize(h->stream));
    for (int64_t c = 0; c < h->C; ++c) {
        if (U) memcpy(U + 21 * c, ugc.data() + 27 * c, sizeof(double) * 21);
        if (gc) memcpy(gc + 6 * c, ugc.data() + 27 * c + 21, sizeof(double) * 6);
    }
    return 0;
}

int sfmba_schur_matvec(sfmba_handle* h, const double* x, const double* dc, const double* dp, const double* v, double* y) {
    CHK(enter(h));
    CHK(check_ready(h, x));
    if (!dc || !dp || !v || !y) return fail(h, -1, "NULL argument");
    CHK(upload_x(h, x));
    CHK(launch_cam_table(h, h->x, h->tab, h->rec));
    int np = 0;
    CHK((launch_resjac<true, true>(h, h->x, h->tab, &np)));
    CHK(launch_normal_blocks(h, h->x, h->tab, h->rec));
    const int64_t C = h->C;
    std::vector<double> vp(6 * C);
    for (int64_t c = 0; c < C; ++c)
        for (int k = 0; k < 6; ++k) vp[k * C + c] = v[6 * c + k];
    HIPCHK(h, hipMemcpyAsync(h->e.p, dp, sizeof(double) * 3 * h->P, hipMemcpyHostToDevice, h->stream));
    HIPCHK(h, hipMemcpyAsync(h->vtmp.p, vp.data(), sizeof(double) * 6 * C, hipMemcpyHostToDevice, h->stream));
    hipLaunchKernelGGL(k_point_prep, dim3((h->P + 255) / 256), dim3(256), 0, h->stream, h->V.as<double>(),
                       h->gp.as<double>(), (const double*)nullptr, h->e.as<double>(), (int)h->P, 0.0,
                       vinv_ptr(h), (double*)nullptr, (const double*)nullptr, (double*)nullptr);
    LAUNCHED(h);
    CHK(launch_mixed_prep(h, h->x, h->tab));
    CHK(schur_product_standalone(h, h->vtmp.as<double>()));
    CHK(exchange(h, h->acc(), 6 * C, 0));
    std::vector<double> a(6 * C);
    HIPCHK(h, hipMemcpyAsync(a.data(), h->acc(), sizeof(double) * 6 * C, hipMemcpyDeviceToHost, h->stream));
    HIPCHK(h, hipStreamSynchronize(h->stream));
    for (int64_t c = 0; c < C; ++c)
        for (int k = 0; k < 6; ++k) y[6 * c + k] = a[k * C + c] + dc[6 * c + k] * v[6 * c + k];
    HIPCHK(h, hipMemsetAsync(h->acc(), 0, sizeof(double) * 6 * C, h->stream));
    return 0;
}

int sfmba_dense_schur(sfmba_handle* h, const double* x, const double* dc, const double* dp, const double* rhs,
                      double* S_out, double* sol_out) {
    CHK(enter(h));
    CHK(check_ready(h, x));
    if (!dc || !dp || !rhs || !sol_out) return fail(h, -1, "NULL argument");
    if (!h->dense) return fail(h, -1, "the dense reduced-camera path needs 6 * n_cameras <= %d", kDenseMaxN);
    const int64_t C = h->C;
    CHK(upload_x(h, x));
    CHK(launch_cam_table(h, h->x, h->tab, h->rec));
    int np = 0;
    CHK((launch_resjac<true, true>(h, h->x, h->tab, &np)));
    CHK(launch_normal_blocks(h, h->x, h->tab, h->rec));
    std::vector<double> ugc(27 * C), planes(6 * C), accp(6 * C);
    HIPCHK(h, hipMemcpyAsync(ugc.data(), h->Ugc(), sizeof(double) * 27 * C, hipMemcpyDeviceToHost, h->stream));
    HIPCHK(h, hipStreamSynchronize(h->stream));
    for (int64_t c = 0; c < C; ++c)
        for (int k = 0; k < 6; ++k) {
            planes[k * C + c] = dc[6 * c + k];
            accp[k * C + c] = -ugc[27 * c + 21 + k] - rhs[6 * c + k];
        }
    HIPCHK(h, hipMemcpyAsync(h->e.p, dp, sizeof(double) * 3 * h->P, hipMemcpyHostToDevice, h->stream));
    HIPCHK(h, hipMemcpyAsync(h->Dc.p, planes.data(), sizeof(double) * 6 * C, hipMemcpyHostToDevice, h->stream));
    HIPCHK(h, hipMemcpyAsync(h->acc(), accp.data(), sizeof(double) * 6 * C, hipMemcpyHostToDevice, h->stream));
    hipLaunchKernelGGL(k_point_prep, dim3((h->P + 255) / 256), dim3(256), 0, h->stream, h->V.as<double>(),
                       h->gp.as<double>(), (const double*)nullptr, h->e.as<double>(), (int)h->P, 0.0,
                       vinv_ptr(h), (double*)nullptr, (const double*)nullptr, (double*)nullptr);
    LAUNCHED(h);
    CHK(launch_dense_solve(h, 1e-14, 40 * 6 * (int)C, false));
    std::vector<double> blk(36 * (size_t)h->n_blk), sol(6 * C);
    HIPCHK(h, hipMemcpyAsync(blk.data(), h->Sblk.p, sizeof(double) * blk.size(), hipMemcpyDeviceToHost, h->stream));
    HIPCHK(h, hipMemcpyAsync(sol.data(), h->vecs.p, sizeof(double) * 6 * C, hipMemcpyDeviceToHost, h->stream));
    HIPCHK(h, hipStreamSynchronize(h->stream));
    for (int64_t c = 0; c < C; ++c)
        for (int k = 0; k < 6; ++k) sol_out[6 * c + k] = sol[k * C + c];
    if (S_out) {
        const int64_t n = 6 * C;
        for (int64_t a = 0; a < C; ++a)
            for (int64_t b = a; b < C; ++b) {
                const double* B = blk.data() + 36 * (size_t)dense_block_index((int)a, (int)b, (int)C);
                for (int u = 0; u < 6; ++u)
                    for (int v = 0; v < 6; ++v) {
                        double val = -B[6 * u + v];
                        if (a == b) {
                            const int lo = std::min(u, v), hi = std::max(u, v);
                            val += ugc[27 * a + (lo * 6 - lo * (lo - 1) / 2 + (hi - lo))];
                            if (u == v) val += dc[6 * a + u];
                        }
                        S_out[(6 * a + u) * n + 6 * b + v] = val;
                        if (a != b) S_out[(6 * b + v) * n + 6 * a + u] = val;
                    }
            }
    }
    return 0;
}

int sfmba_time_kernel(sfmba_handle* h, const double* x, int32_t which, int32_t reps, double* avg_us) {
    CHK(enter(h));
    CHK(check_ready(h, x));
    if (!avg_us || reps <= 0) return fail(h, -1, "bad reps / avg_us");
    CHK(upload_x(h, x));
    CHK(launch_cam_table(h, h->x, h->tab, h->rec));
    int np = 0;
    CHK((launch_resjac<true, true>(h, h->x, h->tab, &np)));
    if (which >= 2) {
        CHK(launch_normal_blocks(h, h->x, h->tab, h->rec));
        CHK(launch_update_scale(h, 1));
        hipLaunchKernelGGL(k_point_prep, dim3((h->P + 255) / 256), dim3(256), 0, h->stream, h->V.as<double>(),
                           h->gp.as<double>(), h->si.as<double>() + 6 * h->C, (const double*)nullptr, (int)h->P,
                           1e-6, vinv_ptr(h), h->rec + 3, (const double*)(h->x + 6 * h->C),
                           h->use_rhsrec ? h->rhsrec.as<double>() : (double*)nullptr);
        LAUNCHED(h);
        CHK(launch_mixed_prep(h, h->x, h->tab));
        hipLaunchKernelGGL(k_transpose, dim3((unsigned)((6 * h->C + 255) / 256)), dim3(256), 0, h->stream,
                           (const double*)h->g.as<double>(), (int)h->C, 6, h->vtmp.as<double>(), (const PcgCtrl*)nullptr, 0);
        HIPCHK(h, hipMemcpyAsync(h->vcm.p, h->g.p, sizeof(double) * 6 * h->C, hipMemcpyDeviceToDevice, h->stream));
        CHK(schur_product_standalone(h, h->vtmp.as<double>()));
    }
    struct EventPair {
        hipEvent_t a = nullptr, b = nullptr;
        ~EventPair() { if (a) (void)hipEventDestroy(a); if (b) (void)hipEventDestroy(b); }
    } ev;
    HIPCHK(h, hipEventCreate(&ev.a));
    HIPCHK(h, hipEventCreate(&ev.b));
    HIPCHK(h, hipStreamSynchronize(h->stream));
    HIPCHK(h, hipEventRecord(ev.a, h->stream));
    for (int k = 0; k < reps; ++k) {
        switch (which) {
            case 0: CHK((launch_resjac<true, true>(h, h->x, h->tab, &np))); break;
            case 1: CHK((launch_resjac<false, false>(h, h->x, h->tab, &np))); break;
            case 2: CHK(launch_normal_blocks(h, h->x, h->tab, h->rec)); break;
            case 3: CHK(schur_product_standalone(h, h->vtmp.as<double>())); break;
            case 4: CHK(launch_point_sweep(h, (h->lds_vec || h->sweep_rc || h->sweep_rc_g) ? h->vtmp.as<double>() : h->vcm.as<double>(), nullptr, 0)); break;
            case 5: CHK(launch_cam_schur<0>(h, h->vtmp.as<double>(), nullptr, 0)); break;
            case 6: CHK(launch_cam_schur<1>(h, nullptr, nullptr, 0)); break;
            case 7: CHK((launch_resjac<true, true>(h, h->x, h->tab, &np, nullptr, nullptr, false))); break;
            case 8:
                if (xcd_cam(h)) { CHK(launch_rhs_and_preconditioner(h)); break; }
                hipLaunchKernelGGL((k_cam_rhs_diag<false>), dim3(h->n_chunks), dim3(kRhsThreads), 0, h->stream, cam_major(h),
                                   (const double*)h->tab, (const double*)h->rec, (const double*)vinv_ptr(h), h->K, (int)h->C,
                                   h->acc(), h->cam_partial.as<double>(), RhsPrecond{nullptr, nullptr, nullptr},
                                   h->use_rhsrec ? (const double*)h->rhsrec.as<double>() : (const double*)nullptr, CamExchange{});
                LAUNCHED(h);
                break;
            case 10:
                hipLaunchKernelGGL(k_fill16, dim3(h->n_cu * 2), dim3(1024), 0, h->stream, h->J.as<double>(),
                                   (int64_t)((h->f32 ? 3 : 6) * h->ld), 1.0);
                break;
            default: return fail(h, -1, "unknown kernel id %d", which);
        }
    }
    HIPCHK(h, hipEventRecord(ev.b, h->stream));
    HIPCHK(h, hipEventSynchronize(ev.b));
    float ms = 0.f;
    HIPCHK(h, hipEventElapsedTime(&ms, ev.a, ev.b));
    *avg_us = 1e3 * (double)ms / reps;
    HIPCHK(h, hipStreamSynchronize(h->stream));
    return 0;
}

static int solve_impl(sfmba_handle* h, const double* x_start, double* x_inout, const sfmba_options* opt_in, sfmba_result* out);

int sfmba_solve(sfmba_handle* h, double* x_inout, const sfmba_options* opt_in, sfmba_result* out) {
    return sfmba_solve_from(h, x_inout, x_inout, opt_in, out);
}

int sfmba_solve_from(sfmba_handle* h, const double* x0, double* x_out, const sfmba_options* opt_in, sfmba_result* out) {
    const int rc = solve_impl(h, x0, x_out, opt_in, out);
    if (rc != 0 && h) {
        const std::string msg = h->err;
        h->skip = nullptr; h->post = Mailbox{};
        if (h->stream) (void)hipStreamSynchronize(h->stream);
        if (h->copy_stream) (void)hipStreamSynchronize(h->copy_stream);
        if (rc == -5 && h->p2p.ready) {
            p2p_close_peers(h);
            if (h->p2p.words) (void)hipMemset(h->p2p.words, 0, 4 * sizeof(unsigned));
        }
        h->err = msg;
    }
    return rc;
}

static int solve_impl(sfmba_handle* h, const double* x_start, double* x_inout, const sfmba_options* opt_in, sfmba_result* out) {
    CHK(enter(h));
    CHK(check_ready(h, x_start));
    if (!x_inout) return fail(h, -1, "x_out is NULL");
    if (!out) return fail(h, -1, "result is NULL");
    sfmba_options opt;
    if (opt_in) opt = *opt_in; else sfmba_default_options(&opt);
    memset(out, 0, sizeof *out);
    h->solved = false;
    h->skip = nullptr; h->post = Mailbox{};
    h->pending_scale_sums = false;
    h->p2p.first_in_solve = true;
    if (h->dbg.p2p_delay_ms > 0) std::this_thread::sleep_for(std::chrono::milliseconds(h->dbg.p2p_delay_ms));
    const double t_begin = now_s();
    const int64_t C = h->C, P = h->P, n = h->n;
    const int64_t max_nfev = opt.max_nfev > 0 ? opt.max_nfev : 100 * (6 * C + 3 * P);
    const double m_total = 2.0 * (double)h->N_total;
    double* sc = h->scal();

    h->x = h->xa.as<double>(); h->x_new = h->xb.as<double>();
    h->tab = h->tabA.as<double>(); h->tab_new = h->tabB.as<double>();
    h->rec = h->recA.as<double>(); h->rec_new = h->recB.as<double>();
    CHK(upload_x(h, x_start));
    h->mirror_on = h->copy_stream != nullptr && n >= 2000000;
    h->x_tag = 0; h->mirror_tag[0] = h->mirror_tag[1] = 0;
    if (h->mirror_on) {
        HIPCHK(h, h->mirror[0].ensure(sizeof(double) * n, 0));
        HIPCHK(h, h->mirror[1].ensure(sizeof(double) * n, 0));
    }
    HIPCHK(h, hipMemsetAsync(h->scal() + kGhPrevSlot, 0, 2 * sizeof(double), h->stream));
    const double t_dev0 = now_s();
    report_stall(h, "upload_x", t_dev0 - t_begin);

    struct EventList : std::vector<std::pair<hipEvent_t, hipEvent_t>> {
        ~EventList() { for (auto& pr : *this) { (void)hipEventDestroy(pr.first); (void)hipEventDestroy(pr.second); } }
    } evs;
    int np_cost = 0;
    auto eval_jac = [&](const double* x, double* tab, bool table_ready, bool finish = true) -> int {
        if (!table_ready) CHK(launch_cam_table(h, x, tab, h->rec));
        int& np = np_cost;
        if (opt.profile) {
            hipEvent_t a, b;
            HIPCHK(h, hipEventCreateWithFlags(&a, hipEventDisableSystemFence));
            if (hipEventCreateWithFlags(&b, hipEventDisableSystemFence) != hipSuccess) {
                (void)hipEventDestroy(a);
                return fail(h, -3, "hipEventCreateWithFlags failed");
            }
            evs.emplace_back(a, b);
            CHK((launch_resjac<true, true>(h, x, tab, &np, a, b)));
        } else {
            CHK((launch_resjac<true, true>(h, x, tab, &np)));
        }
        if (finish) CHK(launch_finish(h, h->part.as<double>(), np, 1, 0));
        return 0;
    };
    auto linearise = [&](int first) -> int {
        CHK(launch_normal_blocks(h, h->x, h->tab, h->rec));
        CHK(launch_update_scale(h, first));
        CHK(exchange_linearise(h));
        return 0;
    };

    CHK(eval_jac(h->x, h->tab, false));
    CHK(exchange(h, sc, 1, 0));
    CHK(linearise(1));
    CHK(fetch_scalars(h));
    double cost = 0.5 * h->h_scal[0];
    if (!std::isfinite(cost)) return fail(h, -2, "Residuals are not finite in the initial point.");
    out->cost0 = cost;
    out->rmse0 = std::sqrt(2.0 * cost / m_total);
    int64_t nfev = 1, njev = 1, iteration = 0, pcg_total = 0;
    double Delta = std::sqrt(qsum(h, 2));
    if (Delta == 0.0) Delta = 1.0;
    int status = -1;
    double step_norm = 0.0, actual_reduction = 0.0, g_norm = 0.0, reg_term = 0.0;
    bool have_red = false;
    int pcg_guess = h->pcg_hint;
    std::vector<int> pcg_hist_new;
    bool guess_exact = false;
    unsigned long long sig = h->problem_gen * 0x9E3779B97F4A7C15ull;
    {
        const int64_t stride = std::max<int64_t>(1, n / 509);
        for (int64_t k = 0; k < n; k += stride) {
            unsigned long long bits;
            memcpy(&bits, x_start + k, sizeof bits);
            sig = (sig ^ bits) * 0x100000001B3ull;
        }
    }
    const bool hist_same = h->hist_C == C && h->hist_P == P && h->hist_N == h->N && h->hist_sig == sig;
    const bool hist_near = hist_same || (h->hist_N > 0 && std::llabs(h->hist_C - C) <= 1 && 2 * h->N >= h->hist_N && h->N <= 2 * h->hist_N);
    if (!hist_near) { h->pcg_hist.clear(); h->pcg_hint = 0; pcg_guess = 0; }
    if (!h->pcg_hist.empty() && h->pcg_hist[0] > 0) { pcg_guess = h->pcg_hist[0]; guess_exact = hist_same; }
    int64_t pcg_breakdowns = 0;
    bool nb_valid = true;
    const bool pcg_debug = h->dbg.trace_pcg != 0;
    const int pcg_bias = h->dbg.pcg_guess_bias;
    if (opt.verbose >= 2) print_header(h);

    for (;;) {
        if (!nb_valid) {
            CHK(eval_jac(h->x, h->tab, true));
            CHK(launch_normal_blocks(h, h->x, h->tab, h->rec));
            nb_valid = true;
        }
        const bool one_rank = !multi_rank(h);
        int np = 0;
        const bool scale_sums_rode = h->pending_scale_sums;
        CHK(launch_jdot(h, &np));
        if (!one_rank && h->p2p.ready) {
            Piggyback pb{h->partB(), sc, FinishJob{}, 1, 1, 0};
            pb.job.row0[0] = 0; pb.job.nrows[0] = np;
            for (int k = 0; k < kNQ; ++k) { pb.job.slot[0][k] = 1 + k; pb.job.slot[1][k] = -1; }
            static_assert(kMaxSlot == 12, "mask below assumes the maximum sits at the end of the run");
            CHK(p2p_allreduce(h, sc + 1, scale_sums_rode ? kMaxSlot : 1, 0, nullptr,
                              scale_sums_rode ? 1ull << (kMaxSlot - 1) : 0ull, &pb));
            ++h->n_collectives;
        } else if (!one_rank) {
            CHK(launch_finish(h, h->partB(), np, 1, 1));
            if (scale_sums_rode) CHK(exchange_linearise(h));
            CHK(exchange(h, sc + 1, 1, 0));
        }
        {
            const int bc = (int)((C + 63) / 64), bp = (int)((P + 63) / 64);
            hipLaunchKernelGGL(k_prep, dim3(bc + bp), dim3(64), 0, h->stream, sc, Delta, opt.reg_min, h->Ugc(),
                               h->V.as<double>(), h->gp.as<double>(), h->si.as<double>(), (int)C, (int)P, bc,
                               h->Dc.as<double>(), (h->dbg.precond == 0 ? h->Minv.as<double>() : (double*)nullptr),
                               vinv_ptr(h), h->rec + 3,
                               one_rank ? (const double*)h->partB() : (const double*)nullptr, np, opt.pcg_tol,
                               std::max(opt.pcg_tol, opt.pcg_tol_max), (const double*)(h->x + 6 * C),
                               (h->use_rhsrec && !(h->dense && one_rank)) ? h->rhsrec.as<double>() : (double*)nullptr,
                               (h->dense && one_rank) ? MixedPrep{nullptr, nullptr, nullptr, nullptr, Origin{0.0, 0.0, 0.0}} : mixed_prep(h, h->tab));
            LAUNCHED(h);
        }
        const bool dense = h->dense && one_rank;
        if (!dense) CHK(launch_rhs_and_preconditioner(h));
        if (!dense) CHK(pcg_start(h, opt));
        PcgCtrl hc{};
        if (dense) {
            CHK(launch_dense_solve(h, kDenseTolFactor * opt.pcg_tol, pcg_max_iters(h, opt), true));
        } else if (pcg_guess > 0) {
            CHK(pcg_enqueue(h, pcg_guess + (h->pcg_fused ? 1 : 0) + (guess_exact ? 0 : 1), true));
        } else {
            CHK(pcg_finish_polling(h, opt, &hc));
        }
        int np_tail = 0;
        auto tail = [&](bool for_device_step) -> int {
            CHK(launch_backsub(h, &np));
            np_tail = np;
            if (!one_rank && h->p2p.ready) {
                const Piggyback pb = backsub_rider(h, np);
                CHK(p2p_allreduce(h, sc + 2, 6, 0, nullptr, 0, &pb));
                ++h->n_collectives;
                return 0;
            }
            if (!(for_device_step && one_rank)) CHK(launch_finish_backsub(h, np));
            CHK(exchange_tail(h));
            return 0;
        };
        CHK(tail(true));

        Mailbox trial_post{};
        bool trial_post_pending = false;
        auto enqueue_trial = [&](const double* coef_dev, double c1, double c2) -> int {
            const int bc = (int)((C + 255) / 256);
            hipLaunchKernelGGL(k_step_table, dim3(bc + grid_1d(3 * P, 256, 2048)), dim3(256), 0, h->stream, h->x,
                               h->sg.as<double>(), h->p.as<double>(), c1, c2, coef_dev, (int)C, n, bc, h->x_new,
                               h->tab_new, h->rec_new, h->skip);
            LAUNCHED(h);
            if (h->mirror_on) {
                const int w = h->x_new == h->xa.as<double>() ? 0 : 1;
                HIPCHK(h, hipEventRecord(h->ev_written, h->stream));
                HIPCHK(h, hipStreamWaitEvent(h->copy_stream, h->ev_written, 0));
                HIPCHK(h, hipMemcpyAsync(h->mirror[w].p, h->x_new, sizeof(double) * n, hipMemcpyDeviceToHost, h->copy_stream));
                HIPCHK(h, hipEventRecord(h->ev_copied[w], h->copy_stream));
                h->mirror_tag[w] = ++h->copy_count;
            }
            const Mailbox mb{h->mbox_dev, sc, h->ctrl.as<PcgCtrl>() + (h->pcg_L & 1), ++h->mbox_seq, p2p_error_word(h)};
            const bool ranks = multi_rank(h);
            if (ranks && h->p2p.ready) {
                CHK(eval_jac(h->x_new, h->tab_new, true, false));
                Piggyback pb{h->part.as<double>(), sc, FinishJob{}, 1, 1, 0};
                pb.job.row0[0] = 0; pb.job.nrows[0] = np_cost;
                for (int k = 0; k < kNQ; ++k) { pb.job.slot[0][k] = k; pb.job.slot[1][k] = -1; }
                CHK(p2p_allreduce(h, sc, 1, 0, nullptr, 0, &pb, &mb, h->skip));
                ++h->n_collectives;
                return 0;
            }
            if (!ranks && h->dbg.cost_rider == 0) {
                h->post = mb;
                const int rc = eval_jac(h->x_new, h->tab_new, true);
                h->post = Mailbox{};
                return rc;
            }
            if (!ranks) {
                CHK(eval_jac(h->x_new, h->tab_new, true, false));
                trial_post = mb;
                trial_post_pending = true;
                return 0;
            }
            CHK(eval_jac(h->x_new, h->tab_new, true));
            CHK(exchange(h, sc, 1, 0));
            hipLaunchKernelGGL(k_post, dim3(1), dim3(64), 0, h->stream, mb);
            LAUNCHED(h);
            return 0;
        };
        auto handoff = [&](bool with_ctrl) -> int {
            if (trial_post_pending) CHK(launch_normal_blocks(h, h->x_new, h->tab_new, h->rec_new, np_cost, trial_post));
            else CHK(launch_normal_blocks(h, h->x_new, h->tab_new, h->rec_new));
            trial_post_pending = false;
            nb_valid = false;
            CHK(wait_mailbox(h, h->mbox_seq));
            memcpy(h->h_scal, h->mbox, sizeof(double) * kScalSlots);
            if (with_ctrl) memcpy(&hc, h->mbox + kMboxCtrl, sizeof hc);
            return 0;
        };
        const bool speculated = pcg_guess > 0 || dense;
        const int pcg_enqueued = pcg_guess > 0 ? pcg_guess + (h->pcg_fused ? 1 : 0) + (guess_exact ? 0 : 1) : 0;
        bool missed = false;
        for (bool speculative = speculated;;) {
            hipLaunchKernelGGL(k_tr_step, dim3(1), dim3(one_rank ? 1024 : 64), 0, h->stream, sc, Delta,
                               speculative ? (const PcgCtrl*)(h->ctrl.as<PcgCtrl>() + (h->pcg_L & 1)) : (const PcgCtrl*)nullptr,
                               one_rank ? backsub_rider(h, np_tail) : Piggyback{});
            LAUNCHED(h);
            h->skip = sc + 30;
            int rc_trial = enqueue_trial(sc + 25, 0.0, 0.0);
            if (rc_trial == 0) rc_trial = handoff(speculative);
            h->skip = nullptr;
            CHK(rc_trial);
            if (!(speculative && hc.done == 0)) break;
            missed = true;
            nb_valid = true;
            if (opt.profile && !evs.empty()) {
                (void)hipEventDestroy(evs.back().first);
                (void)hipEventDestroy(evs.back().second);
                evs.pop_back();
            }
            CHK(pcg_finish_polling(h, opt, &hc));
            CHK(tail(true));
            speculative = false;
        }
        bool first_trial_ready = true;
        if (hc.done == 3) ++pcg_breakdowns;

        g_norm = std::max(h->h_scal[kMaxSlot], h->h_scal[kCamSlot + 0]);
        if (g_norm < opt.gtol) status = 1;
        if (opt.verbose >= 2) print_iter(h, iteration, nfev, cost, have_red, actual_reduction, step_norm, g_norm);
        if (status != -1 || nfev >= max_nfev || (opt.max_iter > 0 && iteration >= opt.max_iter)) break;
        pcg_total += hc.iters;
        if (pcg_debug && dense)
            fprintf(stderr, "sfmba: iteration %lld: PCG in LDS, %d iterations, outcome %d, reg %.3e\n", (long long)iteration,
                    hc.iters, hc.done, h->h_scal[kRegSlot]);
        else if (pcg_debug)
            fprintf(stderr, "sfmba: iteration %lld: PCG enqueued %d, needed %d%s\n", (long long)iteration,
                    pcg_enqueued, hc.iters, missed ? " (miss)" : "");
        h->pcg_hint = std::max(hc.iters, h->pcg_hint - 1);
        pcg_hist_new.push_back(hc.iters);
        {
            const int rec = (iteration + 1 < (int64_t)h->pcg_hist.size()) ? h->pcg_hist[iteration + 1] : 0;
            guess_exact = rec > 0 && pcg_bias == 0 && hist_same;
            pcg_guess = std::max(1, (guess_exact ? rec : h->pcg_hint) + pcg_bias);
        }
        reg_term = h->h_scal[kRegSlot];

        const double x_norm = std::sqrt(qsum(h, 3));
        const TrModel model = tr_build_model(h->h_scal[1], h->h_scal[2], h->h_scal[3], qsum(h, 1), qsum(h, 5),
                                             qsum(h, 6), qsum(h, 4), qsum(h, 7), qsum(h, 8));

        actual_reduction = -1.0;
        double cost_new = cost;
        while (actual_reduction <= 0.0 && nfev < max_nfev) {
            TrStep st;
            if (first_trial_ready) {
                st.c1 = h->h_scal[25]; st.c2 = h->h_scal[26]; st.predicted = h->h_scal[27];
                st.step_h_norm = h->h_scal[28]; st.step_norm = h->h_scal[29];
                first_trial_ready = false;
            } else {
                st = tr_solve_step(model, Delta);
                CHK(enqueue_trial(nullptr, st.c1, st.c2));
                CHK(handoff(false));
            }
            ++nfev;
            cost_new = 0.5 * h->h_scal[0];
            if (!std::isfinite(cost_new)) {
                Delta = 0.25 * st.step_h_norm;
                continue;
            }
            actual_reduction = cost - cost_new;
            double ratio;
            const double Delta_new = update_tr_radius(Delta, actual_reduction, st.predicted, st.step_h_norm,
                                                      st.step_h_norm > 0.95 * Delta, &ratio);
            step_norm = st.step_norm;
            const int term = check_termination(actual_reduction, cost, step_norm, x_norm, ratio, opt.ftol, opt.xtol);
            if (term != 0) { status = term; break; }
            Delta = Delta_new;
        }
        have_red = true;
        if (actual_reduction > 0.0) {
            std::swap(h->x, h->x_new);
            std::swap(h->tab, h->tab_new);
            std::swap(h->rec, h->rec_new);
            h->x_tag = h->mirror_tag[h->x == h->xa.as<double>() ? 0 : 1];
            nb_valid = true;
            cost = cost_new;
            ++njev;
            CHK(launch_update_scale(h, 0, true));
        } else {
            step_norm = 0.0;
            actual_reduction = 0.0;
        }
        ++iteration;
        if (status != -1) {
            if (h->pending_scale_sums) {
                CHK(flush_scale_sums(h));
                CHK(exchange_linearise(h));
            }
            CHK(fetch_scalars(h));
            g_norm = std::max(h->h_scal[kMaxSlot], h->h_scal[kCamSlot + 0]);
            if (opt.verbose >= 2) print_iter(h, iteration, nfev, cost, have_red, actual_reduction, step_norm, g_norm);
            break;
        }
    }
    if (status == -1) status = 0;
    if (!nb_valid) {
        int np = 0;
        CHK((launch_resjac<false, true>(h, h->x, h->tab, &np)));
    }

    CHK(ensure_h_x(h));
    const double t_dl0 = now_s();
    const int xw = h->x == h->xa.as<double>() ? 0 : 1;
    const bool mirrored = h->mirror_on && h->x_tag != 0 && h->mirror_tag[xw] == h->x_tag;
    const size_t xbytes = sizeof(double) * (size_t)n;
    if (!mirrored) HIPCHK(h, hipMemcpyAsync(h->h_x, h->x, xbytes, hipMemcpyDeviceToHost, h->stream));
    if (h->p2p.ready)
        HIPCHK(h, hipMemcpyAsync(h->h_scal + 62, h->p2p.words + 1, sizeof(unsigned), hipMemcpyDeviceToHost, h->stream));
    CHK(wait_stream(h));
    if (mirrored) HIPCHK(h, hipEventSynchronize(h->ev_copied[xw]));
    const double t_dl1 = now_s();
    if (h->p2p.ready) {
        unsigned err = 0;
        memcpy(&err, h->h_scal + 62, sizeof err);
        if (err != 0) return p2p_timed_out(h, err);
    }
    staging_copy(h, x_inout, mirrored ? h->mirror[xw].p : (const void*)h->h_x, xbytes);
    if (h->mirror_on) HIPCHK(h, hipStreamSynchronize(h->copy_stream));
    const double t_end = now_s();
    if (h->dbg.trace_timing)
        fprintf(stderr, "sfmba: solve  %.3f ms total, upload %.1f us, result: copy + wait %.1f us, staging copy %.1f us\n", 1e3 * (t_end - t_begin),
                1e6 * (t_dev0 - t_begin), 1e6 * (t_dl1 - t_dl0), 1e6 * (t_end - t_dl1));
    if (!evs.empty()) {
        double tot = 0.0;
        for (auto& pr : evs) {
            float ms = 0.f;
            if (hipEventElapsedTime(&ms, pr.first, pr.second) == hipSuccess) tot += ms;
        }
        out->resjac_avg_us = 1e3 * tot / (double)evs.size();
        out->resjac_launches = (int64_t)evs.size();
    }
    h->pcg_hist.swap(pcg_hist_new);
    h->hist_C = C; h->hist_P = P; h->hist_N = h->N; h->hist_sig = sig;
    out->cost = cost;
    out->optimality = g_norm;
    out->rmse = std::sqrt(2.0 * cost / m_total);
    out->nfev = nfev; out->njev = njev; out->iterations = iteration; out->pcg_iterations = pcg_total;
    out->status = status;
    out->seconds_total = t_end - t_begin;
    out->seconds_device = t_end - t_dev0;
    out->last_step_norm = step_norm;
    out->last_reg = reg_term;
    out->reserved = (int32_t)pcg_breakdowns;
    h->solved = true;
    return 0;
}

int sfmba_get_fun_grad(sfmba_handle* h, double* fun_out, double* grad_out) {
    CHK(enter(h));
    if (!h->have_problem || !h->solved) return fail(h, -1, "no completed sfmba_solve on this handle");
    if (fun_out) CHK(download_residuals(h, fun_out));
    if (grad_out) {
        CHK(ensure_h_x(h));
        HIPCHK(h, hipMemcpyAsync(h->h_x, h->g.p, sizeof(double) * h->n, hipMemcpyDeviceToHost, h->stream));
        CHK(wait_stream(h));
        memcpy(grad_out, h->h_x, sizeof(double) * h->n);
    }
    return 0;
}

int sfmba_tr2d_solve(const double* B3, const double* g2, double Delta, double* p2) {
    return solve_trust_region_2d(B3, g2, Delta, p2) ? 1 : 0;
}

}
```

Measured before the change: 2645.

## Speculate scale update, defer initial host sync, and overlap result download

Adds three host-side schedule changes, each behind a flag that defaults to -1, which counts as on. First, the scale update runs speculatively into double-buffered g/si/sg arrays right after the trial normal blocks, and the buffers are swapped if the step is accepted. Second, the initial cost and trust radius no longer wait on a host sync: the radius is computed on device from the scalars, and the start values are read back through the mailbox after the first jdot launch. Third, the final x download starts early on a separate copy stream once convergence is known. Together these aim to remove host round-trips and serialised launches per solve, at the cost of extra buffers and wasted scale work when a step is rejected.

```diff
diff --git a/sfm-python_amd/csrc/ba_kernels.hpp b/sfm-python_amd/csrc/ba_kernels.hpp
--- a/sfm-python_amd/csrc/ba_kernels.hpp
+++ b/sfm-python_amd/csrc/ba_kernels.hpp
@@ -244,6 +244,12 @@
     cam_table_row(prm, tab, C, c);
 }
 
+__device__ __forceinline__ double start_radius(const double* __restrict__ sc, double Delta) {
+    if (Delta >= 0.0) return Delta;
+    const double d = sqrt(sc[9] + sc[16 + 2]);
+    return d == 0.0 ? 1.0 : d;
+}
+
 __global__ void k_tr_step(double* __restrict__ sc, double Delta, const PcgCtrl* __restrict__ ctrl,
                           Piggyback pb) {
     if (pb.part != nullptr) {
@@ -254,6 +260,7 @@
     if (ctrl != nullptr && ctrl->done == 0) { sc[30] = 1.0; return; }
     auto q = [&](int point_slot, int k) { return sc[point_slot] + sc[16 + k]; };
     const TrModel m = tr_build_model(sc[1], sc[2], sc[3], q(8, 1), q(4, 5), q(5, 6), q(11, 4), q(6, 7), q(7, 8));
+    Delta = start_radius(sc, Delta);
     const TrStep st = tr_solve_step(m, Delta);
     sc[25] = st.c1; sc[26] = st.c2; sc[27] = st.predicted; sc[28] = st.step_h_norm; sc[29] = st.step_norm;
     sc[30] = 0.0; sc[31] = Delta;
@@ -296,6 +303,23 @@
     if (q >= 3 * P) return;
     const int p = q / 3;
     rec[(size_t)kRec * p + (q - 3 * p)] = pts[q];
+}
+
+__global__ __launch_bounds__(256) void k_cam_table_rec(const double* __restrict__ x, int C, int P, int bc,
+                                                       double* __restrict__ tab, double* __restrict__ rec) {
+    if ((int)blockIdx.x < bc) {
+        const int c = blockIdx.x * blockDim.x + threadIdx.x;
+        if (c >= C) return;
+        double prm[6];
+#pragma unroll
+        for (int k = 0; k < 6; ++k) prm[k] = x[6 * (size_t)c + k];
+        cam_table_row(prm, tab, C, c);
+        return;
+    }
+    const int q = ((int)blockIdx.x - bc) * blockDim.x + threadIdx.x;
+    if (q >= 3 * P) return;
+    const int p = q / 3;
+    rec[(size_t)kRec * p + (q - 3 * p)] = x[6 * (size_t)C + q];
 }
 
 template <bool JAC>
@@ -979,9 +1003,10 @@
                                                       const double* __restrict__ V,
                                                       const double* __restrict__ gp,
                                                       const double* __restrict__ x, int C, int P,
-                                                      int first, int bc, double* __restrict__ si,
+                                                      int first, int bc, const double* si_old, double* si,
                                                       double* __restrict__ g, double* __restrict__ sg,
-                                                      double* __restrict__ part) {
+                                                      double* __restrict__ part, const double* __restrict__ skip) {
+    if (skip != nullptr && *skip != 0.0) return;
     const int n6 = 6 * C;
     double q[kNQ];
 #pragma unroll
@@ -1002,13 +1027,14 @@
             const int c = e / 6, k = e - 6 * c;
             const double d = Ugc[(size_t)c * 27 + diagU[k]], ge = Ugc[(size_t)c * 27 + 21 + k];
             double s, sge;
-            element(d, ge, first ? 0.0 : si[e], x[e], s, sge);
+            element(d, ge, first ? 0.0 : si_old[e], x[e], s, sge);
             si[e] = s; g[e] = ge; sg[e] = sge;
         }
     } else {
         const int nb = (int)gridDim.x - bc, b = (int)blockIdx.x - bc;
         const double* __restrict__ xp = x + n6;
-        double* __restrict__ sip = si + n6;
+        const double* sio = si_old + n6;
+        double* sip = si + n6;
         double* __restrict__ gpo = g + n6;
         double* __restrict__ sgp = sg + n6;
         for (int p0 = (b * kScalePts) * (int)blockDim.x + (int)threadIdx.x; p0 < P; p0 += nb * kScalePts * (int)blockDim.x) {
@@ -1022,7 +1048,7 @@
                 for (int k = 0; k < 3; ++k) {
                     ge[u][k] = gp[pp * 3 + k];
                     xe[u][k] = xp[pp * 3 + k];
-                    so[u][k] = first ? 0.0 : sip[pp * 3 + k];
+                    so[u][k] = first ? 0.0 : sio[pp * 3 + k];
                 }
             }
 #pragma unroll
@@ -1353,7 +1379,7 @@
     } else {
         G11 = sc[1];
     }
-    const double reg = reg_from_scalars(sc, G11, Delta, reg_min);
+    const double reg = reg_from_scalars(sc, G11, start_radius(sc, Delta), reg_min);
     if (blockIdx.x == 0 && threadIdx.x == 0) {
         sc[13] = reg;
         const double a11 = sc[8] + sc[16 + 1], prev = sc[14];
diff --git a/sfm-python_amd/csrc/sfmba.hip b/sfm-python_amd/csrc/sfmba.hip
--- a/sfm-python_amd/csrc/sfmba.hip
+++ b/sfm-python_amd/csrc/sfmba.hip
@@ -230,6 +230,9 @@
         int pcg_mixed_b = -1;
         int pcg_mixed = -1;
         int pcg_split = -1;
+        int spec_scale = -1;
+        int start_handoff = -1;
+        int early_download = -1;
         int cam_chunk = 0;
         int pcg_guess_bias = 0;
         int trace_pcg = 0, trace_stalls = 0, trace_timing = 0;
@@ -257,6 +260,7 @@
     DevBuf V, Vinv, gp, e, recA, recB;
     DevBuf edge;
     DevBuf g, si, sg, p;
+    DevBuf g2, si2, sg2;
     DevBuf Dc, Minv, vecs, vtmp, vcm;
     DevBuf part, ctrl;
     DevBuf arena_own;
@@ -300,6 +304,7 @@
     size_t h_x_doubles = 0;
     hipStream_t copy_stream = nullptr;
     hipEvent_t ev_written = nullptr, ev_copied[2] = {nullptr, nullptr};
+    bool result_in_flight = false;
     PinnedBuf mirror[2];
     unsigned long long mirror_tag[2] = {0, 0}, copy_count = 0, x_tag = 0;
     bool mirror_on = false;
@@ -330,6 +335,12 @@
     double* tab_new = nullptr;
     double* rec = nullptr;
     double* rec_new = nullptr;
+    double* g_cur = nullptr;
+    double* si_cur = nullptr;
+    double* sg_cur = nullptr;
+    double* g_new = nullptr;
+    double* si_new = nullptr;
+    double* sg_new = nullptr;
 
     double* acc() const { return arena; }
     double* sd() const { return arena + 6 * C; }
@@ -502,6 +513,19 @@
     if (h->dbg.trace_stalls && seconds > 2e-3) fprintf(stderr, "sfmba: waited %.2f ms in %s\n", 1e3 * seconds, where);
 }
 
+int wait_event(sfmba_handle* h, hipEvent_t ev) {
+    const double t0 = now_s();
+    for (;;) {
+        const hipError_t e = hipEventQuery(ev);
+        if (e == hipSuccess) { report_stall(h, "wait_event", now_s() - t0); return 0; }
+        if (e != hipErrorNotReady) return fail(h, -3, "hipEventQuery failed: %s", hipGetErrorString(e));
+        if (now_s() - t0 > 0.05) break;
+    }
+    HIPCHK(h, hipEventSynchronize(ev));
+    report_stall(h, "wait_event (blocking)", now_s() - t0);
+    return 0;
+}
+
 int wait_stream(sfmba_handle* h) {
     const double t0 = now_s();
     for (;;) {
@@ -553,7 +577,14 @@
 }
 
 
-int launch_cam_table(sfmba_handle* h, const double* x, double* tab, double* rec) {
+int launch_cam_table(sfmba_handle* h, const double* x, double* tab, double* rec, bool one_launch = false) {
+    if (one_launch) {
+        const int bc = (int)((h->C + 255) / 256);
+        hipLaunchKernelGGL(k_cam_table_rec, dim3((unsigned)(bc + (3 * h->P + 255) / 256)), dim3(256), 0, h->stream, x,
+                           (int)h->C, (int)h->P, bc, tab, rec);
+        LAUNCHED(h);
+        return 0;
+    }
     hipLaunchKernelGGL(k_cam_table, dim3((h->C + 255) / 256), dim3(256), 0, h->stream, x, (int)h->C, tab);
     LAUNCHED(h);
     hipLaunchKernelGGL(k_fill_rec, dim3((unsigned)((3 * h->P + 255) / 256)), dim3(256), 0, h->stream, x + 6 * h->C, (int)h->P, rec);
@@ -939,7 +970,7 @@
 
 int launch_jdot(sfmba_handle* h, int* nparts) {
     const int grid = grid_1d(h->N, kSweepThreads, h->n_cu);
-    const double* sgc = h->sg.as<double>();
+    const double* sgc = h->sg_cur;
     const double* sgp = sgc + 6 * h->C;
     Piggyback pb{};
     if (h->pending_scale_sums) pb = slices_rider(h, 0, 4);
@@ -982,7 +1013,7 @@
         CHK(set_lds(h, kern, lds));
         hipLaunchKernelGGL(kern, dim3(grid), dim3(kSweepThreads), lds, h->stream, h->ranges.as<int2>(), h->n_ranges, obs_arrays(h),
                            h->vecs.as<double>(), dc, vinv_ptr(h), h->gp.as<double>(), h->t1.as<double>(), dp, h->partB(),
-                           (int)h->C, (const PcgCtrl*)nullptr, 0, h->g.as<double>(), h->si.as<double>(), h->sg.as<double>(), rc, FinalUpdate{});
+                           (int)h->C, (const PcgCtrl*)nullptr, 0, h->g_cur, h->si_cur, h->sg_cur, rc, FinalUpdate{});
     } else if (h->lds_vec) {
         const size_t lds = sizeof(double) * 6 * h->C;
         auto kern = k_backsub<true>;
@@ -990,7 +1021,7 @@
         hipLaunchKernelGGL(kern, dim3(grid), dim3(kSweepThreads), lds, h->stream, h->ranges.as<int2>(),
                            h->n_ranges, obs_arrays(h), h->vecs.as<double>(), dc, vinv_ptr(h),
                            h->gp.as<double>(), h->t1.as<double>(), dp, h->partB(), (int)h->C,
-                           ctrl2, h->pcg_L, h->g.as<double>(), h->si.as<double>(), h->sg.as<double>(), rc,
+                           ctrl2, h->pcg_L, h->g_cur, h->si_cur, h->sg_cur, rc,
                            h->pcg_a_owed ? FinalUpdate{h->pcg_part.as<double>(), h->vecs.as<double>(), h->ctrl.as<PcgCtrl>(), h->pcg_L - 1}
                                          : FinalUpdate{});
     } else {
@@ -1000,24 +1031,30 @@
         hipLaunchKernelGGL(k_backsub<false>, dim3(grid), dim3(kSweepThreads), 0, h->stream,
                            h->ranges.as<int2>(), h->n_ranges, obs_arrays(h), h->vecs.as<double>(), dc,
                            vinv_ptr(h), h->gp.as<double>(), h->t1.as<double>(), dp,
-                           h->partB(), (int)h->C, (const PcgCtrl*)nullptr, 0, h->g.as<double>(),
-                           h->si.as<double>(), h->sg.as<double>(), rc, FinalUpdate{});
+                           h->partB(), (int)h->C, (const PcgCtrl*)nullptr, 0, h->g_cur,
+                           h->si_cur, h->sg_cur, rc, FinalUpdate{});
     }
     LAUNCHED(h);
     *nparts = grid;
     return 0;
 }
 
-int launch_update_scale(sfmba_handle* h, int first, bool defer = false) {
+int launch_update_scale(sfmba_handle* h, int first, bool defer = false, bool speculative = false) {
+    const double* x = speculative ? h->x_new : h->x;
+    double* si = speculative ? h->si_new : h->si_cur;
+    double* g = speculative ? h->g_new : h->g_cur;
+    double* sg = speculative ? h->sg_new : h->sg_cur;
+    const double* skip = speculative ? h->skip : (const double*)nullptr;
     if (h->scale_pts == 2)
         hipLaunchKernelGGL(k_update_scale<2>, dim3(h->red_grid), dim3(256), 0, h->stream, h->Ugc(), h->V.as<double>(),
-                           h->gp.as<double>(), h->x, (int)h->C, (int)h->P, first, h->red_bc, h->si.as<double>(),
-                           h->g.as<double>(), h->sg.as<double>(), h->part.as<double>());
+                           h->gp.as<double>(), x, (int)h->C, (int)h->P, first, h->red_bc, (const double*)h->si_cur, si,
+                           g, sg, h->part.as<double>(), skip);
     else
         hipLaunchKernelGGL(k_update_scale<1>, dim3(h->red_grid), dim3(256), 0, h->stream, h->Ugc(), h->V.as<double>(),
-                           h->gp.as<double>(), h->x, (int)h->C, (int)h->P, first, h->red_bc, h->si.as<double>(),
-                           h->g.as<double>(), h->sg.as<double>(), h->part.as<double>());
+                           h->gp.as<double>(), x, (int)h->C, (int)h->P, first, h->red_bc, (const double*)h->si_cur, si,
+                           g, sg, h->part.as<double>(), skip);
     LAUNCHED(h);
+    if (speculative) return 0;
     if (defer) { h->pending_scale_sums = true; return 0; }
     return launch_finish_slices(h, 0, 4);
 }
@@ -1107,6 +1144,8 @@
         if (!std::isfinite(h->origin.x + h->origin.y + h->origin.z)) h->origin = Origin{0.0, 0.0, 0.0};
     }
     HIPCHK(h, hipStreamSynchronize(h->stream));
+    if (h->result_in_flight && h->copy_stream) HIPCHK(h, hipStreamSynchronize(h->copy_stream));
+    h->result_in_flight = false;
     const double t0 = now_s();
     hipError_t err = hipSuccess;
     staging_copy(h, h->h_x, x_host, sizeof(double) * h->n, [&](int, size_t off, size_t bytes) {
@@ -1407,6 +1446,9 @@
     else if (n == "packed_upload") h->dbg.packed_upload = v;
     else if (n == "pcg_mixed_b") h->dbg.pcg_mixed_b = v;
     else if (n == "cost_rider") h->dbg.cost_rider = v;
+    else if (n == "spec_scale") h->dbg.spec_scale = v;
+    else if (n == "start_handoff") h->dbg.start_handoff = v;
+    else if (n == "early_download") h->dbg.early_download = v;
     else if (n == "rhsrec") h->dbg.rhsrec = v;
     else if (n == "xcd_chunks") h->dbg.xcd_chunks = v;
     else if (n == "tab_lds") h->dbg.tab_lds = v;
@@ -2036,6 +2078,11 @@
     HIPCHK(h, h->g.ensure(sizeof(double) * h->n));
     HIPCHK(h, h->si.ensure(sizeof(double) * h->n));
     HIPCHK(h, h->sg.ensure(sizeof(double) * h->n));
+    HIPCHK(h, h->g2.ensure(sizeof(double) * h->n));
+    HIPCHK(h, h->si2.ensure(sizeof(double) * h->n));
+    HIPCHK(h, h->sg2.ensure(sizeof(double) * h->n));
+    h->g_cur = static_cast<double*>(h->g.p); h->si_cur = static_cast<double*>(h->si.p); h->sg_cur = static_cast<double*>(h->sg.p);
+    h->g_new = h->g2.as<double>(); h->si_new = h->si2.as<double>(); h->sg_new = h->sg2.as<double>();
     HIPCHK(h, h->p.ensure(sizeof(double) * h->n + 16));
     HIPCHK(h, h->Dc.ensure(sizeof(double) * 6 * C));
     HIPCHK(h, h->Minv.ensure(sizeof(double) * 21 * C));
@@ -2318,14 +2365,14 @@
         CHK(launch_normal_blocks(h, h->x, h->tab, h->rec));
         CHK(launch_update_scale(h, 1));
         hipLaunchKernelGGL(k_point_prep, dim3((h->P + 255) / 256), dim3(256), 0, h->stream, h->V.as<double>(),
-                           h->gp.as<double>(), h->si.as<double>() + 6 * h->C, (const double*)nullptr, (int)h->P,
+                           h->gp.as<double>(), h->si_cur + 6 * h->C, (const double*)nullptr, (int)h->P,
                            1e-6, vinv_ptr(h), h->rec + 3, (const double*)(h->x + 6 * h->C),
                            h->use_rhsrec ? h->rhsrec.as<double>() : (double*)nullptr);
         LAUNCHED(h);
         CHK(launch_mixed_prep(h, h->x, h->tab));
         hipLaunchKernelGGL(k_transpose, dim3((unsigned)((6 * h->C + 255) / 256)), dim3(256), 0, h->stream,
-                           (const double*)h->g.as<double>(), (int)h->C, 6, h->vtmp.as<double>(), (const PcgCtrl*)nullptr, 0);
-        HIPCHK(h, hipMemcpyAsync(h->vcm.p, h->g.p, sizeof(double) * 6 * h->C, hipMemcpyDeviceToDevice, h->stream));
+                           (const double*)h->g_cur, (int)h->C, 6, h->vtmp.as<double>(), (const PcgCtrl*)nullptr, 0);
+        HIPCHK(h, hipMemcpyAsync(h->vcm.p, h->g_cur, sizeof(double) * 6 * h->C, hipMemcpyDeviceToDevice, h->stream));
         CHK(schur_product_standalone(h, h->vtmp.as<double>()));
     }
     struct EventPair {
@@ -2429,8 +2476,13 @@
         ~EventList() { for (auto& pr : *this) { (void)hipEventDestroy(pr.first); (void)hipEventDestroy(pr.second); } }
     } evs;
     int np_cost = 0;
+    const bool quick_start = !multi_rank(h) && h->dbg.start_handoff != 0 && h->dbg.cost_rider != 0;
+    const bool spec_scale = !multi_rank(h) && h->dbg.spec_scale != 0;
+    const bool early_download = h->copy_stream != nullptr && h->dbg.early_download != 0;
+    bool result_sent = false;
+    double t_sent0 = 0.0, t_sent1 = 0.0, t_ws = 0.0;
     auto eval_jac = [&](const double* x, double* tab, bool table_ready, bool finish = true) -> int {
-        if (!table_ready) CHK(launch_cam_table(h, x, tab, h->rec));
+        if (!table_ready) CHK(launch_cam_table(h, x, tab, h->rec, quick_start));
         int& np = np_cost;
         if (opt.profile) {
             hipEvent_t a, b;
@@ -2454,17 +2506,31 @@
         return 0;
     };
 
-    CHK(eval_jac(h->x, h->tab, false));
-    CHK(exchange(h, sc, 1, 0));
-    CHK(linearise(1));
-    CHK(fetch_scalars(h));
-    double cost = 0.5 * h->h_scal[0];
-    if (!std::isfinite(cost)) return fail(h, -2, "Residuals are not finite in the initial point.");
-    out->cost0 = cost;
-    out->rmse0 = std::sqrt(2.0 * cost / m_total);
+    double cost = 0.0, Delta = -1.0;
+    unsigned long long start_seq = 0;
+    auto start_values = [&]() -> int {
+        cost = 0.5 * h->h_scal[0];
+        if (!std::isfinite(cost)) return fail(h, -2, "Residuals are not finite in the initial point.");
+        out->cost0 = cost;
+        out->rmse0 = std::sqrt(2.0 * cost / m_total);
+        return 0;
+    };
+    if (quick_start) {
+        CHK(eval_jac(h->x, h->tab, false, false));
+        start_seq = ++h->mbox_seq;
+        CHK(launch_normal_blocks(h, h->x, h->tab, h->rec, np_cost,
+                                 Mailbox{h->mbox_dev, sc, nullptr, start_seq, p2p_error_word(h)}));
+        CHK(launch_update_scale(h, 1, true));
+    } else {
+        CHK(eval_jac(h->x, h->tab, false));
+        CHK(exchange(h, sc, 1, 0));
+        CHK(linearise(1));
+        CHK(fetch_scalars(h));
+        CHK(start_values());
+        Delta = std::sqrt(qsum(h, 2));
+        if (Delta == 0.0) Delta = 1.0;
+    }
     int64_t nfev = 1, njev = 1, iteration = 0, pcg_total = 0;
-    double Delta = std::sqrt(qsum(h, 2));
-    if (Delta == 0.0) Delta = 1.0;
     int status = -1;
     double step_norm = 0.0, actual_reduction = 0.0, g_norm = 0.0, reg_term = 0.0;
     bool have_red = false;
@@ -2500,6 +2566,12 @@
         int np = 0;
         const bool scale_sums_rode = h->pending_scale_sums;
         CHK(launch_jdot(h, &np));
+        if (start_seq != 0) {
+            CHK(wait_mailbox(h, start_seq));
+            memcpy(h->h_scal, h->mbox, sizeof(double) * kScalSlots);
+            start_seq = 0;
+            CHK(start_values());
+        }
         if (!one_rank && h->p2p.ready) {
             Piggyback pb{h->partB(), sc, FinishJob{}, 1, 1, 0};
             pb.job.row0[0] = 0; pb.job.nrows[0] = np;
@@ -2516,7 +2588,7 @@
         {
             const int bc = (int)((C + 63) / 64), bp = (int)((P + 63) / 64);
             hipLaunchKernelGGL(k_prep, dim3(bc + bp), dim3(64), 0, h->stream, sc, Delta, opt.reg_min, h->Ugc(),
-                               h->V.as<double>(), h->gp.as<double>(), h->si.as<double>(), (int)C, (int)P, bc,
+                               h->V.as<double>(), h->gp.as<double>(), h->si_cur, (int)C, (int)P, bc,
                                h->Dc.as<double>(), (h->dbg.precond == 0 ? h->Minv.as<double>() : (double*)nullptr),
                                vinv_ptr(h), h->rec + 3,
                                one_rank ? (const double*)h->partB() : (const double*)nullptr, np, opt.pcg_tol,
@@ -2557,7 +2629,7 @@
         auto enqueue_trial = [&](const double* coef_dev, double c1, double c2) -> int {
             const int bc = (int)((C + 255) / 256);
             hipLaunchKernelGGL(k_step_table, dim3(bc + grid_1d(3 * P, 256, 2048)), dim3(256), 0, h->stream, h->x,
-                               h->sg.as<double>(), h->p.as<double>(), c1, c2, coef_dev, (int)C, n, bc, h->x_new,
+                               h->sg_cur, h->p.as<double>(), c1, c2, coef_dev, (int)C, n, bc, h->x_new,
                                h->tab_new, h->rec_new, h->skip);
             LAUNCHED(h);
             if (h->mirror_on) {
@@ -2602,6 +2674,7 @@
             else CHK(launch_normal_blocks(h, h->x_new, h->tab_new, h->rec_new));
             trial_post_pending = false;
             nb_valid = false;
+            if (spec_scale) CHK(launch_update_scale(h, 0, true, true));
             CHK(wait_mailbox(h, h->mbox_seq));
             memcpy(h->h_scal, h->mbox, sizeof(double) * kScalSlots);
             if (with_ctrl) memcpy(&hc, h->mbox + kMboxCtrl, sizeof hc);
@@ -2634,6 +2707,7 @@
         }
         bool first_trial_ready = true;
         if (hc.done == 3) ++pcg_breakdowns;
+        if (Delta < 0.0) Delta = h->h_scal[31];
 
         g_norm = std::max(h->h_scal[kMaxSlot], h->h_scal[kCamSlot + 0]);
         if (g_norm < opt.gtol) status = 1;
@@ -2696,7 +2770,23 @@
             nb_valid = true;
             cost = cost_new;
             ++njev;
-            CHK(launch_update_scale(h, 0, true));
+            if (status != -1 && early_download && !h->mirror_on) {
+                CHK(ensure_h_x(h));
+                t_sent0 = now_s();
+                HIPCHK(h, hipMemcpyAsync(h->h_x, h->x, sizeof(double) * (size_t)n, hipMemcpyDeviceToHost, h->copy_stream));
+                HIPCHK(h, hipEventRecord(h->ev_copied[0], h->copy_stream));
+                h->result_in_flight = true;
+                result_sent = true;
+                t_sent1 = now_s();
+            }
+            if (spec_scale) {
+                std::swap(h->g_cur, h->g_new);
+                std::swap(h->si_cur, h->si_new);
+                std::swap(h->sg_cur, h->sg_new);
+                h->pending_scale_sums = true;
+            } else {
+                CHK(launch_update_scale(h, 0, true));
+            }
         } else {
             step_norm = 0.0;
             actual_reduction = 0.0;
@@ -2724,10 +2814,17 @@
     const int xw = h->x == h->xa.as<double>() ? 0 : 1;
     const bool mirrored = h->mirror_on && h->x_tag != 0 && h->mirror_tag[xw] == h->x_tag;
     const size_t xbytes = sizeof(double) * (size_t)n;
-    if (!mirrored) HIPCHK(h, hipMemcpyAsync(h->h_x, h->x, xbytes, hipMemcpyDeviceToHost, h->stream));
+    if (!mirrored && !result_sent) {
+        HIPCHK(h, hipMemcpyAsync(h->h_x, h->x, xbytes, hipMemcpyDeviceToHost, h->stream));
+    }
     if (h->p2p.ready)
         HIPCHK(h, hipMemcpyAsync(h->h_scal + 62, h->p2p.words + 1, sizeof(unsigned), hipMemcpyDeviceToHost, h->stream));
     CHK(wait_stream(h));
+    t_ws = now_s();
+    if (result_sent) {
+        CHK(wait_event(h, h->ev_copied[0]));
+        h->result_in_flight = false;
+    }
     if (mirrored) HIPCHK(h, hipEventSynchronize(h->ev_copied[xw]));
     const double t_dl1 = now_s();
     if (h->p2p.ready) {
@@ -2738,6 +2835,9 @@
     staging_copy(h, x_inout, mirrored ? h->mirror[xw].p : (const void*)h->h_x, xbytes);
     if (h->mirror_on) HIPCHK(h, hipStreamSynchronize(h->copy_stream));
     const double t_end = now_s();
+    if (h->dbg.trace_timing && result_sent)
+        fprintf(stderr, "sfmba: early result copy: enqueue %.1f us, then %.1f us to the last post, stream query %.1f us, copy event %.1f us\n",
+                1e6 * (t_sent1 - t_sent0), 1e6 * (t_dl0 - t_sent1), 1e6 * (t_ws - t_dl0), 1e6 * (t_dl1 - t_ws));
     if (h->dbg.trace_timing)
         fprintf(stderr, "sfmba: solve  %.3f ms total, upload %.1f us, result: copy + wait %.1f us, staging copy %.1f us\n", 1e3 * (t_end - t_begin),
                 1e6 * (t_dev0 - t_begin), 1e6 * (t_dl1 - t_dl0), 1e6 * (t_end - t_dl1));
@@ -2772,7 +2872,7 @@
     if (fun_out) CHK(download_residuals(h, fun_out));
     if (grad_out) {
         CHK(ensure_h_x(h));
-        HIPCHK(h, hipMemcpyAsync(h->h_x, h->g.p, sizeof(double) * h->n, hipMemcpyDeviceToHost, h->stream));
+        HIPCHK(h, hipMemcpyAsync(h->h_x, h->g_cur, sizeof(double) * h->n, hipMemcpyDeviceToHost, h->stream));
         CHK(wait_stream(h));
         memcpy(grad_out, h->h_x, sizeof(double) * h->n);
     }
```

After: 2763 (median of 6 runs). 4.5% higher.
